# Chuanming-Liu/DAzimSurfTomo

Measured on AMD Instinct MI355X. Metric: FMM traveltime fields/sec (256^2 grid, 16 periods) + LSQR SpMV HBM GB/s, higher is better.
Workload: dtype f32

## Files before the change

dazimsurftomo_amd/csrc/assemble.hip:

```cpp
#include "sparse_internal.h"

#include <rocprim/device/device_scan.hpp>

namespace {

__device__ __forceinline__ bool tikh_face(int cell, int nvx, int nvz, int nzm1, int &i, int &j, int &k) {
  k = cell / (nvx * nvz);
  const int r = cell - k * nvx * nvz;
  j = r / nvx;
  i = r - j * nvx;
  return i == 0 || i == nvx - 1 || j == 0 || j == nvz - 1 || k == 0 || k == nzm1 - 1;
}
__global__ void k_tikh_count(int64_t r0, int64_t nrow, int maxvp, int nvx, int nvz, int nzm1, long *cnt) {
  const int64_t r = (int64_t)blockIdx.x * VB + threadIdx.x;
  if (r > nrow) return;
  int i, j, k;
  cnt[r] = r == nrow ? 0 : (tikh_face((int)((r0 + r) % maxvp), nvx, nvz, nzm1, i, j, k) ? 1 : 7);
}
__global__ void k_tikh_fill(int64_t r0, int64_t nrow, int maxvp, int nvx, int nvz, int nzm1, const long *off, int64_t nnz0,
                            const float *__restrict__ w, int64_t *__restrict__ rowptr, int *__restrict__ col,
                            float *__restrict__ val) {
  const int64_t r = (int64_t)blockIdx.x * VB + threadIdx.x;
  if (r > nrow) return;
  rowptr[r] = nnz0 + off[r];
  if (r == nrow) return;
  const int blk = (int)((r0 + r) / maxvp), cell = (int)((r0 + r) - (int64_t)blk * maxvp);
  int i, j, k;
  const bool face = tikh_face(cell, nvx, nvz, nzm1, i, j, k);
  const float wt = w[blk];
  const int c = blk * maxvp + cell;
  const int64_t p = nnz0 + off[r];
  if (face) {
    col[p] = c;
    val[p] = 2.0f * wt;
  } else {
    const int d[7] = {-nvz * nvx, -nvx, -1, 0, 1, nvx, nvz * nvx};
#pragma unroll
    for (int q = 0; q < 7; q++) {
      col[p + q] = c + d[q];
      val[p + q] = q == 3 ? 6.0f * wt : -1.0f * wt;
    }
  }
}
__device__ __forceinline__ bool lap2d_edge(int cell, int nvx, int nvz) {
  const int j = cell / nvx, i = cell - j * nvx;
  return i == 0 || i == nvx - 1 || j == 0 || j == nvz - 1;
}
__global__ void k_lap2d_count(int64_t nrow, int ncell, int nvx, int nvz, long *cnt) {
  const int64_t r = (int64_t)blockIdx.x * VB + threadIdx.x;
  if (r > nrow) return;
  cnt[r] = r == nrow ? 0 : (lap2d_edge((int)(r % ncell), nvx, nvz) ? 1 : 5);
}
__global__ void k_lap2d_fill(int64_t nrow, int ncell, int nvx, int nvz, const long *off, int64_t nnz0, const float *__restrict__ w,
                             int64_t *__restrict__ rowptr, int *__restrict__ col, float *__restrict__ val) {
  const int64_t r = (int64_t)blockIdx.x * VB + threadIdx.x;
  if (r > nrow) return;
  rowptr[r] = nnz0 + off[r];
  if (r == nrow) return;
  const int b = (int)(r / ncell), cell = (int)(r - (int64_t)b * ncell);
  const float wt = w[b];
  const int c = b * ncell + cell;
  const int64_t p = nnz0 + off[r];
  if (lap2d_edge(cell, nvx, nvz)) {
    col[p] = c;
    val[p] = 2.0f * wt;
  } else {
    const int d[5] = {-nvx, -1, 0, 1, nvx};
#pragma unroll
    for (int q = 0; q < 5; q++) {
      col[p + q] = c + d[q];
      val[p + q] = q == 2 ? 4.0f * wt : -1.0f * wt;
    }
  }
}
__global__ void k_residual(int64_t n, const float *obst, const float *dsyn, float *res, float *rel) {
  for (int64_t i = (int64_t)blockIdx.x * VB + threadIdx.x; i < n; i += (int64_t)gridDim.x * VB) {
    const float r = obst[i] - dsyn[i];
    res[i] = r;
    rel[i] = fabsf(r / obst[i]);
  }
}
__global__ void k_sigma_stats(int64_t n, const float *rel, float *out) {
  constexpr int CH = 8192;
  __shared__ float s_c[CH];
  __shared__ float s_mean;
  float acc = 0.0f;
  for (int pass = 0; pass < 2; pass++) {
    acc = 0.0f;
    const float mean = pass ? s_mean : 0.0f;
    for (int64_t base = 0; base < n; base += CH) {
      const int len = (int)((n - base) < CH ? (n - base) : CH);
      __syncthreads();
      for (int i = threadIdx.x; i < len; i += blockDim.x) s_c[i] = rel[base + i];
      __syncthreads();
      if (threadIdx.x == 0) {
        if (pass == 0)
          for (int i = 0; i < len; i++) acc = acc + s_c[i];
        else
          for (int i = 0; i < len; i++) acc = acc + (s_c[i] - mean) * (s_c[i] - mean);
      }
    }
    if (threadIdx.x == 0) {
      if (pass == 0) {
        s_mean = acc / (float)n;
        out[0] = s_mean;
      } else {
        out[1] = sqrtf(acc / (float)n);
      }
    }
    __syncthreads();
  }
}
__global__ void k_sigma_weights(int64_t n, const float *obst, const float *res, const float *rel, const float *ms, float *wgt,
                                float *rhs) {
  const float sd = ms[1];
  for (int64_t i = (int64_t)blockIdx.x * VB + threadIdx.x; i < n; i += (int64_t)gridDim.x * VB) {
    const float ratio = fabsf(rel[i] / (1.5f * sd));
    float sigma = sd * obst[i];
    if (ratio > 1.0f) sigma = sigma * (float)exp((double)(ratio - 1.0f));
    const float wt = 1.0f / sigma;
    wgt[i] = wt;
    rhs[i] = res[i] * wt;
  }
}
__global__ void k_weight_sums(int64_t n, const float *res, const float *wgt, const float *rhs, double *part) {
  double a[5] = {0, 0, 0, 0, 0};
  for (int64_t i = (int64_t)blockIdx.x * VB + threadIdx.x; i < n; i += (int64_t)gridDim.x * VB) {
    const double r = res[i];
    a[0] += r; a[1] += fabs(r); a[2] += r * r; a[3] += wgt[i]; a[4] += fabsf(rhs[i]);
  }
  __shared__ double s[5][VB / 64];
#pragma unroll
  for (int q = 0; q < 5; q++) {
    const double t = wave_sum(a[q]);
    if ((threadIdx.x & 63) == 0) s[q][threadIdx.x >> 6] = t;
  }
  __syncthreads();
  if (threadIdx.x < 5) {
    double t = 0.0;
    for (int i = 0; i < VB / 64; i++) t += s[threadIdx.x][i];
    part[blockIdx.x * 5 + threadIdx.x] = t;
  }
}
__global__ void k_model_update(int nx, int ny, int nzm1, int joint, float *vs, float *dv, float minvel, float maxvel, float *gc,
                               float *gs) {
  const int nvx = nx - 2, nvz = ny - 2, maxvp = nvx * nvz * nzm1;
  const int ii = blockIdx.x * VB + threadIdx.x;
  if (ii >= maxvp) return;
  const int k = ii / (nvx * nvz), r = ii - k * nvx * nvz, j = r / nvx, i = r - j * nvx;
  float p = dv[ii];
  if (p >= 0.500f) p = 0.500f;
  if (p <= -0.500f) p = -0.500f;
  if (fabsf(p) < 1e-5f) p = 0.0f;
  dv[ii] = p;
  const size_t iv = ((size_t)k * ny + (j + 1)) * nx + (i + 1);
  float v = vs[iv] + p;
  if (v < minvel) v = minvel;
  if (v > maxvel) v = maxvel;
  vs[iv] = v;
  if (joint) {
    if (gc) gc[ii] = dv[maxvp + ii];
    if (gs) gs[ii] = dv[2 * maxvp + ii];
  }
}
__global__ void k_map_update(int nx, int ny, int kmax, int azim, double *pv, float *dm, float minc, float maxc, float *a1, float *a2) {
  const int nvx = nx - 2, nvz = ny - 2, nmap = nvx * nvz * kmax;
  const int ii = blockIdx.x * VB + threadIdx.x;
  if (ii >= nmap) return;
  const int k = ii / (nvx * nvz), r = ii - k * nvx * nvz, j = r / nvx, i = r - j * nvx;
  float p = dm[ii];
  if (p >= 0.500f) p = 0.500f;
  if (p <= -0.500f) p = -0.500f;
  if (fabsf(p) < 1e-5f) p = 0.0f;
  dm[ii] = p;
  const size_t iv = ((size_t)k * ny + (j + 1)) * nx + (i + 1);
  float v = (float)pv[iv] + p;
  if (v < minc) v = minc;
  if (v > maxc) v = maxc;
  pv[iv] = (double)v;
  if (azim) {
    if (a1) a1[ii] = dm[nmap + ii];
    if (a2) a2[ii] = dm[2 * nmap + ii];
  }
}
__global__ void k_update_stats(int ncell, const float *dv, float *out) {
  const float *x = dv + (size_t)blockIdx.x * ncell;
  float mn = INFINITY, mx = -INFINITY;
  double sa = 0.0;
  for (int i = threadIdx.x; i < ncell; i += VB) {
    const float v = x[i];
    mn = fminf(mn, v);
    mx = fmaxf(mx, v);
    sa += fabsf(v);
  }
#pragma unroll
  for (int o = 32; o > 0; o >>= 1) {
    mn = fminf(mn, __shfl_xor(mn, o));
    mx = fmaxf(mx, __shfl_xor(mx, o));
  }
  sa = wave_sum(sa);
  __shared__ float s_mn[VB / 64], s_mx[VB / 64];
  __shared__ double s_sa[VB / 64];
  if ((threadIdx.x & 63) == 0) { s_mn[threadIdx.x >> 6] = mn; s_mx[threadIdx.x >> 6] = mx; s_sa[threadIdx.x >> 6] = sa; }
  __syncthreads();
  if (threadIdx.x == 0) {
    for (int i = 1; i < VB / 64; i++) { mn = fminf(mn, s_mn[i]); mx = fmaxf(mx, s_mx[i]); sa += s_sa[i]; }
    out[blockIdx.x * 3 + 0] = mn; out[blockIdx.x * 3 + 1] = mx; out[blockIdx.x * 3 + 2] = (float)sa;
  }
}

}

extern "C" {

static int append_stencil_rows(dazim_ctx *ctx, dazim_csr *A, bool lap2d, int nvx, int nvz, int nzm1, int64_t maxvp, int64_t row_lo,
                               int64_t nrow, int nblock, const float *w_host, float *dw, long *cnt, long *off);

int dazim_csr_append_tikhonov(dazim_ctx *ctx, dazim_csr *A, int nx, int ny, int nz, int nblock, const float *w_host) {
  if (nblock < 1 || nx < 3 || ny < 3 || nz < 2) return dz_fail(ctx, DAZIM_E_BAD_ARG, "bad arguments to dazim_csr_append_tikhonov");
  return dazim_csr_append_tikhonov_rows(ctx, A, nx, ny, nz, nblock, w_host, 0, (int64_t)(nx - 2) * (ny - 2) * (nz - 1) * nblock);
}
int dazim_csr_append_tikhonov_rows(dazim_ctx *ctx, dazim_csr *A, int nx, int ny, int nz, int nblock, const float *w_host,
                                   int64_t row_lo, int64_t row_hi) {
  if (!ctx || !A || !w_host || nblock < 1 || nx < 3 || ny < 3 || nz < 2) return dz_fail(ctx, DAZIM_E_BAD_ARG, "bad arguments to dazim_csr_append_tikhonov");
  const int nvx = nx - 2, nvz = ny - 2, nzm1 = nz - 1;
  const int64_t maxvp = (int64_t)nvx * nvz * nzm1, nrow = row_hi - row_lo;
  if (row_lo < 0 || row_hi < row_lo || row_hi > maxvp * nblock) return dz_fail(ctx, DAZIM_E_BAD_ARG, "bad row range of the regularisation block");
  if (maxvp * nblock > A->n || maxvp > 0x7ffffff0) return dz_fail(ctx, DAZIM_E_BAD_ARG, "regularisation blocks do not fit the %lld columns", (long long)A->n);
  DZ_HIP(hipSetDevice(ctx->device));
  int rc;
  long *cnt, *off;
  float *dw;
  if ((rc = dz_scratch(ctx, "tikh.cnt", (size_t)(nrow + 1), &cnt)) || (rc = dz_scratch(ctx, "tikh.off", (size_t)(nrow + 1), &off)) ||
      (rc = dz_scratch(ctx, "tikh.w", 64, &dw)))
    return rc;
  if (nblock > 64) return dz_fail(ctx, DAZIM_E_BAD_ARG, "too many regularisation blocks");
  return append_stencil_rows(ctx, A, false, nvx, nvz, nzm1, maxvp, row_lo, nrow, nblock, w_host, dw, cnt, off);
}

static int append_stencil_rows(dazim_ctx *ctx, dazim_csr *A, bool lap2d, int nvx, int nvz, int nzm1, int64_t maxvp, int64_t row_lo,
                               int64_t nrow, int nblock, const float *w_host, float *dw, long *cnt, long *off) {
  int rc;
  void *p;
  DZ_HIP(hipMemcpyAsync(dw, w_host, (size_t)nblock * 4, hipMemcpyHostToDevice, ctx->stream));
  const unsigned nb = (unsigned)((nrow + 1 + VB - 1) / VB);
  if (lap2d)
    hipLaunchKernelGGL(k_lap2d_count, dim3(nb), dim3(VB), 0, ctx->stream, nrow, (int)maxvp, nvx, nvz, cnt);
  else
    hipLaunchKernelGGL(k_tikh_count, dim3(nb), dim3(VB), 0, ctx->stream, row_lo, nrow, (int)maxvp, nvx, nvz, nzm1, cnt);
  auto fill = [&](int64_t *rowptr, int *col, float *val) {
    if (lap2d)
      hipLaunchKernelGGL(k_lap2d_fill, dim3(nb), dim3(VB), 0, ctx->stream, nrow, (int)maxvp, nvx, nvz, off, A->nnz, dw, rowptr, col, val);
    else
      hipLaunchKernelGGL(k_tikh_fill, dim3(nb), dim3(VB), 0, ctx->stream, row_lo, nrow, (int)maxvp, nvx, nvz, nzm1, off, A->nnz, dw,
                         rowptr, col, val);
  };
  size_t tb = 0;
  DZ_HIP(rocprim::exclusive_scan(nullptr, tb, cnt, off, 0l, (size_t)(nrow + 1), rocprim::plus<long>(), ctx->stream));
  if ((rc = dz_scratch(ctx, "tikh.scan", tb + 256, &p))) return rc;
  DZ_HIP(rocprim::exclusive_scan(p, tb, cnt, off, 0l, (size_t)(nrow + 1), rocprim::plus<long>(), ctx->stream));
  long nnz2 = 0;
  DZ_HIP(hipMemcpyAsync(&nnz2, off + nrow, 8, hipMemcpyDeviceToHost, ctx->stream));
  DZ_HIP(hipStreamSynchronize(ctx->stream));
  const int64_t m2 = A->m + nrow, nz2 = A->nnz + nnz2;
  if (nz2 > 0xfffffff0ll) return dz_fail(ctx, DAZIM_E_NNZ_OVERFLOW, "too many stored entries");
  if (A->cap_m >= m2 && A->cap_nnz >= nz2) {
    const int64_t nnz1 = A->nnz;
    fill(A->rowptr + A->m, A->col, A->val);
    DZ_HIP(hipGetLastError());
    A->m = m2;
    A->nnz = nz2;
    if ((rc = dz_build_colblocks(ctx, A, nnz1 > 0 ? nnz1 : 0))) return rc;
    if ((rc = dz_invalidate_transpose(A))) return rc;
    DZ_HIP(hipStreamSynchronize(ctx->stream));
    return 0;
  }
  int64_t *rowptr;
  int *col;
  float *val;
  if ((rc = dz_big_get(ctx, (size_t)(m2 + 1), &rowptr)) || (rc = dz_big_get(ctx, (size_t)(nz2 > 0 ? nz2 : 1), &col)) ||
      (rc = dz_big_get(ctx, (size_t)(nz2 > 0 ? nz2 : 1), &val)))
    return rc;
  DZ_HIP(hipMemcpyAsync(rowptr, A->rowptr, (size_t)A->m * 8, hipMemcpyDeviceToDevice, ctx->stream));
  DZ_HIP(hipMemcpyAsync(col, A->col, (size_t)A->nnz * 4, hipMemcpyDeviceToDevice, ctx->stream));
  DZ_HIP(hipMemcpyAsync(val, A->val, (size_t)A->nnz * 4, hipMemcpyDeviceToDevice, ctx->stream));
  fill(rowptr + A->m, col, val);
  DZ_HIP(hipGetLastError());
  DZ_HIP(hipStreamSynchronize(ctx->stream));
  dz_big_put(ctx, A->rowptr);
  dz_big_put(ctx, A->col);
  dz_big_put(ctx, A->val);
  A->rowptr = rowptr; A->col = col; A->val = val;
  A->m = m2; A->nnz = nz2;
  A->cap_m = A->cap_nnz = 0;
  if ((rc = dz_build_colblocks(ctx, A))) return rc;
  if ((rc = dz_invalidate_transpose(A))) return rc;
  DZ_HIP(hipStreamSynchronize(ctx->stream));
  return 0;
}

int dazim_csr_append_laplacian2d(dazim_ctx *ctx, dazim_csr *A, int nx, int ny, int nmap, const float *w_host) {
  if (!ctx || !A || !w_host || nmap < 1 || nx < 3 || ny < 3) return dz_fail(ctx, DAZIM_E_BAD_ARG, "bad arguments to dazim_csr_append_laplacian2d");
  const int nvx = nx - 2, nvz = ny - 2;
  const int64_t ncell = (int64_t)nvx * nvz, nrow = ncell * nmap;
  if (nrow > A->n || nrow > 0x7ffffff0) return dz_fail(ctx, DAZIM_E_BAD_ARG, "regularisation maps do not fit the %lld columns", (long long)A->n);
  DZ_HIP(hipSetDevice(ctx->device));
  int rc;
  long *cnt, *off;
  float *dw;
  if ((rc = dz_scratch(ctx, "tikh.cnt", (size_t)(nrow + 1), &cnt)) || (rc = dz_scratch(ctx, "tikh.off", (size_t)(nrow + 1), &off)) ||
      (rc = dz_scratch(ctx, "lap2d.w", (size_t)nmap, &dw)))
    return rc;
  return append_stencil_rows(ctx, A, true, nvx, nvz, 1, ncell, 0, nrow, nmap, w_host, dw, cnt, off);
}

int dazim_weight_data(dazim_ctx *ctx, dazim_csr *G, int64_t dall, const float *obst_u, const float *dsyn_u, float *res_u,
                      float *wgt_u, float *rhs_u, float *stats) {
  return dazim_weight_data_sharded(ctx, G, dall, 0, dall, obst_u, dsyn_u, res_u, wgt_u, rhs_u, stats);
}
int dazim_weight_data_sharded(dazim_ctx *ctx, dazim_csr *G, int64_t dall, int64_t row0, int64_t dall_glob, const float *obst_u,
                              const float *dsyn_u, float *res_u, float *wgt_u, float *rhs_u, float *stats) {
  if (!ctx || dall < 1 || !obst_u || !dsyn_u || !res_u || !wgt_u || !rhs_u || (G && G->m < dall) || row0 < 0 || row0 + dall > dall_glob)
    return dz_fail(ctx, DAZIM_E_BAD_ARG, "bad arguments to dazim_weight_data");
  const bool sharded = ctx->comm && dall_glob > dall;
  DZ_HIP(hipSetDevice(ctx->device));
  DzBuf<float> obst, dsyn, res, wgt, rhs;
  int rc;
  if ((rc = obst.init(ctx, obst_u, dall, true, false)) || (rc = dsyn.init(ctx, dsyn_u, dall, true, false)) ||
      (rc = res.init(ctx, res_u, dall, false, true)) || (rc = wgt.init(ctx, wgt_u, dall, false, true)) ||
      (rc = rhs.init(ctx, rhs_u, dall, false, true)))
    return rc;
  float *rel, *ms;
  double *part;
  if ((rc = dz_scratch(ctx, "wd.rel", (size_t)dall, &rel)) || (rc = dz_scratch(ctx, "wd.ms", 16, &ms)) ||
      (rc = dz_scratch(ctx, "wd.part", (size_t)NPART * 5, &part)))
    return rc;
  const int nb = nblk(dall, NPART);
  hipLaunchKernelGGL(k_residual, dim3(nb), dim3(VB), 0, ctx->stream, dall, obst.dev, dsyn.dev, res.dev, rel);
  if (sharded) {
    float *relg;
    if ((rc = dz_scratch(ctx, "wd.relg", (size_t)dall_glob, &relg))) return rc;
    DZ_HIP(hipMemsetAsync(relg, 0, (size_t)dall_glob * 4, ctx->stream));
    DZ_HIP(hipMemcpyAsync(relg + row0, rel, (size_t)dall * 4, hipMemcpyDeviceToDevice, ctx->stream));
    if ((rc = dz_allreduce(ctx, (DzComm *)ctx->comm, relg, (size_t)dall_glob, DZ_F32, DZ_SUM))) return rc;
    hipLaunchKernelGGL(k_sigma_stats, dim3(1), dim3(VB), 0, ctx->stream, dall_glob, relg, ms);
  } else {
    hipLaunchKernelGGL(k_sigma_stats, dim3(1), dim3(VB), 0, ctx->stream, dall, rel, ms);
  }
  hipLaunchKernelGGL(k_sigma_weights, dim3(nb), dim3(VB), 0, ctx->stream, dall, obst.dev, res.dev, rel, ms, wgt.dev, rhs.dev);
  hipLaunchKernelGGL(k_weight_sums, dim3(nb), dim3(VB), 0, ctx->stream, dall, res.dev, wgt.dev, rhs.dev, part);
  DZ_HIP(hipGetLastError());
  std::vector<double> hp((size_t)nb * 5);
  float hms[2];
  DZ_HIP(hipMemcpyAsync(hp.data(), part, hp.size() * 8, hipMemcpyDeviceToHost, ctx->stream));
  DZ_HIP(hipMemcpyAsync(hms, ms, 8, hipMemcpyDeviceToHost, ctx->stream));
  if (G && (rc = dz_scale_rows(ctx, G, dall, wgt.dev))) return rc;
  DZ_HIP(hipStreamSynchronize(ctx->stream));
  if (stats) {
    double a[5] = {0, 0, 0, 0, 0};
    for (int b = 0; b < nb; b++)
      for (int q = 0; q < 5; q++) a[q] += hp[(size_t)b * 5 + q];
    if (sharded && (rc = dazim_comm_allreduce(ctx, a, 5, DZ_F64, DZ_SUM))) return rc;
    const double n = (double)dall_glob, mean = a[0] / n;
    stats[0] = (float)mean;
    stats[1] = (float)sqrt(fmax(a[2] / n - mean * mean, 0.0));
    stats[2] = (float)(a[1] / n);
    stats[3] = (float)sqrt(a[2] / n);
    stats[4] = hms[0];
    stats[5] = hms[1];
    stats[6] = (float)(a[3] / n);
    stats[7] = (float)(a[4] / n);
  }
  if ((rc = res.finish()) || (rc = wgt.finish()) || (rc = rhs.finish())) return rc;
  DZ_HIP(hipStreamSynchronize(ctx->stream));
  return 0;
}

int dazim_model_update(dazim_ctx *ctx, int nx, int ny, int nz, int joint, float *vs_u, float *dv_u, float minvel, float maxvel,
                       float *gc_u, float *gs_u, float *stats) {
  if (!ctx || !vs_u || !dv_u || nx < 3 || ny < 3 || nz < 2) return dz_fail(ctx, DAZIM_E_BAD_ARG, "bad arguments to dazim_model_update");
  DZ_HIP(hipSetDevice(ctx->device));
  const int nzm1 = nz - 1, ncell = (nx - 2) * (ny - 2), maxvp = ncell * nzm1, nblock = joint ? 3 : 1;
  DzBuf<float> vs, dv, gc, gs;
  int rc;
  if ((rc = vs.init(ctx, vs_u, (size_t)nx * ny * nz, true, true)) || (rc = dv.init(ctx, dv_u, (size_t)maxvp * nblock, true, true)) ||
      (rc = gc.init(ctx, gc_u, joint ? maxvp : 0, false, true)) || (rc = gs.init(ctx, gs_u, joint ? maxvp : 0, false, true)))
    return rc;
  hipLaunchKernelGGL(k_model_update, dim3((maxvp + VB - 1) / VB), dim3(VB), 0, ctx->stream, nx, ny, nzm1, joint, vs.dev, dv.dev,
                     minvel, maxvel, joint ? gc.dev : nullptr, joint ? gs.dev : nullptr);
  DZ_HIP(hipGetLastError());
  if (stats) {
    float *p;
    if ((rc = dz_scratch(ctx, "mu.stats", (size_t)nblock * nzm1 * 3, &p))) return rc;
    hipLaunchKernelGGL(k_update_stats, dim3(nblock * nzm1), dim3(VB), 0, ctx->stream, ncell, dv.dev, p);
    DZ_HIP(hipGetLastError());
    DZ_HIP(hipMemcpyAsync(stats, p, (size_t)nblock * nzm1 * 3 * 4, hipMemcpyDeviceToHost, ctx->stream));
  }
  if ((rc = vs.finish()) || (rc = dv.finish()) || (rc = gc.finish()) || (rc = gs.finish())) return rc;
  DZ_HIP(hipStreamSynchronize(ctx->stream));
  return 0;
}

int dazim_phase_map_update(dazim_ctx *ctx, int nx, int ny, int kmax, int azim, double *pv_u, float *dm_u, float minc, float maxc,
                           float *a1_u, float *a2_u, float *stats) {
  if (!ctx || !pv_u || !dm_u || nx < 3 || ny < 3 || kmax < 1) return dz_fail(ctx, DAZIM_E_BAD_ARG, "bad arguments to dazim_phase_map_update");
  DZ_HIP(hipSetDevice(ctx->device));
  const int ncell = (nx - 2) * (ny - 2), nmap = ncell * kmax, nblock = azim ? 3 : 1;
  DzBuf<double> pv;
  DzBuf<float> dm, a1, a2;
  int rc;
  if ((rc = pv.init(ctx, pv_u, (size_t)nx * ny * kmax, true, true)) || (rc = dm.init(ctx, dm_u, (size_t)nmap * nblock, true, true)) ||
      (rc = a1.init(ctx, a1_u, azim ? nmap : 0, false, true)) || (rc = a2.init(ctx, a2_u, azim ? nmap : 0, false, true)))
    return rc;
  hipLaunchKernelGGL(k_map_update, dim3((nmap + VB - 1) / VB), dim3(VB), 0, ctx->stream, nx, ny, kmax, azim ? 1 : 0, pv.dev, dm.dev,
                     minc, maxc, azim ? a1.dev : nullptr, azim ? a2.dev : nullptr);
  DZ_HIP(hipGetLastError());
  if (stats) {
    float *p;
    if ((rc = dz_scratch(ctx, "mu.stats", (size_t)nblock * kmax * 3, &p))) return rc;
    hipLaunchKernelGGL(k_update_stats, dim3(nblock * kmax), dim3(VB), 0, ctx->stream, ncell, dm.dev, p);
    DZ_HIP(hipGetLastError());
    DZ_HIP(hipMemcpyAsync(stats, p, (size_t)nblock * kmax * 3 * 4, hipMemcpyDeviceToHost, ctx->stream));
  }
  if ((rc = pv.finish()) || (rc = dm.finish()) || (rc = a1.finish()) || (rc = a2.finish())) return rc;
  DZ_HIP(hipStreamSynchronize(ctx->stream));
  return 0;
}

}
```

dazimsurftomo_amd/csrc/rays.hip:

```cpp
#include <cmath>
#include <chrono>
#include <unistd.h>

#include "dazim_internal.h"

#include <rocprim/device/device_scan.hpp>
#include <rocprim/device/device_radix_sort.hpp>

namespace {

#ifdef DZ_RAYS_MARK
#define RAYS_MARK(i) asm volatile("; MARK " #i ::: "memory")
#else
#define RAYS_MARK(i)
#endif

constexpr int GDX = 5, GDZ = 5;
constexpr int RM = DAZIM_RMAX;
constexpr float EARTH = 6371.0f;
constexpr float FTOL = 1e-4f;

struct RayArgs {
  dazim_geom g;
  int nx, ny, nz, kmax;
  long nray;
  const int *field;
  const float *rcx, *rcz;
  const float *scx, *scz;
  const int *period;
  const int *kidx;
  const float *veln;
  const float *ttn;
  const int *tslot;
  int tsh;
  long fstride;
  const int *fdone;
  int *defer_mark;
  int max_quads;
  int sweeps;
  const float *ttnr;
  const int *nstsr;
  const dazim_refbox *boxes;
  const float *vels;
  const double *svs, *svp, *srho;
  unsigned nvx_magic;
  const double *skern;
  const float *lsen;
  double r_dnx, r_dnz, r_dnxr, r_dnzr, r_dvx, r_dvz, r_e2dnx, r_e2dnxr;
  float dplh;
  float *dsurf;
  int *status;
  int *rbflag;
  long *count;
  int *nlist;
  unsigned short *lcell;
  float *lval;
  float *fdm_scratch;
  int LK;
  int lcap;
  const unsigned *perm;
  unsigned *qcount;
  float2 *pts;
  int *npts;
  int pcap;
  int dense;
  long *countd;
  int plain_step;
  int keep_small;
  const long *rowptr;
  float *val;
  int *col;
};

__device__ __forceinline__ float dz_sinf(float x) {
  if (!(x > 0.0f && x < 3.1415927f)) return (float)sin((double)x);
  const double y = (double)x - 1.5707963267948966192;
  const double y2 = y * y;
  double p = -1.5619206968586226e-16;
  p = fma(p, y2, 4.7794773323873853e-14);
  p = fma(p, y2, -1.1470745597729725e-11);
  p = fma(p, y2, 2.0876756987868099e-09);
  p = fma(p, y2, -2.7557319223985891e-07);
  p = fma(p, y2, 2.4801587301587302e-05);
  p = fma(p, y2, -1.3888888888888889e-03);
  p = fma(p, y2, 4.1666666666666664e-02);
  p = fma(p, y2, -0.5);
  p = fma(p, y2, 1.0);
  return (float)p;
}

__device__ __forceinline__ void step_azimuth(float x0, float z0, float x1, float z1, float &c2psi, float &s2psi) {
  const float PI_F = 3.1415926535898f;
  const float evtlat = (PI_F / 2 - x0) * 180.0f / PI_F, evtlon = z0 * 180.0f / PI_F;
  const float stalat = (PI_F / 2 - x1) * 180.0f / PI_F, stalon = z1 * 180.0f / PI_F;
  const double pi = (double)3.1415926535898f;
  const float piby2 = (float)(pi / (double)2.f);
  const double rad = (double)2.f * pi / (double)360.f;
  const double sph = (double)(1.0f / 298.257f);
  const double scolat = (double)piby2 - atan((1. - sph) * (1. - sph) * tan((double)stalat * rad));
  const double ecolat = (double)piby2 - atan((1. - sph) * (1. - sph) * tan((double)evtlat * rad));
  const double slon = (double)stalon * rad, elon = (double)evtlon * rad;
  const double a = sin(scolat) * cos(slon), b = sin(scolat) * sin(slon), c = cos(scolat);
  const double dd = sin(elon), ee = -cos(elon), cc = cos(ecolat);
  const double gg = -cc * ee, hh = cc * dd, kk = -sin(ecolat);
  const double rhs1 = (a - dd) * (a - dd) + (b - ee) * (b - ee) + c * c - (double)2.f;
  const double rhs2 = (a - gg) * (a - gg) + (b - hh) * (b - hh) + (c - kk) * (c - kk) - (double)2.f;
  double daz = atan2(rhs1, rhs2);
  if (daz < 0.0) daz = daz + 2 * pi;
  float az = (float)(daz / rad);
  if (fabsf(az - 360.f) < .00001f) az = 0.0f;
  const float rgpsi = az / 180 * PI_F;
  c2psi = (float)cos((double)(2.0f * rgpsi));
  s2psi = (float)sin((double)(2.0f * rgpsi));
}

__device__ __forceinline__ float divr(float x, double rd) { return (float)((double)x * rd); }

__device__ __forceinline__ void basis(float v, float b[4]) {
  const float om = 1.0f - v;
  b[0] = om * om * om / 6.0f;
  b[1] = (4.0f - 6.0f * (v * v) + 3.0f * (v * v * v)) / 6.0f;
  b[2] = (1.0f + 3.0f * v + 3.0f * (v * v) - 3.0f * (v * v * v)) / 6.0f;
  b[3] = v * v * v / 6.0f;
}

__device__ __forceinline__ float div6(float x) { return divr(x, 1.0 / 6.0); }
__device__ __forceinline__ float basis1(float v, int i) {
  const float w = i == 0 ? 1.0f - v : v;
  const float t2 = w * w, t3 = t2 * w;
  const float p = i == 1 ? 4.0f : 1.0f + 3.0f * v;
  const float c = i == 1 ? -6.0f : 3.0f, d = i == 1 ? 3.0f : -3.0f;
  const float n = (p + c * t2) + d * t3;
  return div6((i == 0 || i == 3) ? t3 : n);
}

__device__ __forceinline__ float vel_at(const dazim_geom &g, const float *veln, int ipx, int ipz, float drx, float drz,
                                        double rdnx, double rdnz) {
  float vel = 0.0f;
#pragma unroll
  for (int l = 1; l <= 2; l++)
#pragma unroll
    for (int m = 1; m <= 2; m++) {
      float produ = (1.0f - fabsf(divr((float)(m - 1) * g.dnz - drz, rdnz)));
      produ = produ * (1.0f - fabsf(divr((float)(l - 1) * g.dnx - drx, rdnx)));
      if (ipz - 1 + m <= g.nnz && ipx - 1 + l <= g.nnx && ipz - 1 + m >= 1 && ipx - 1 + l >= 1)
        vel = vel + veln[(size_t)(ipx - 2 + l) * g.nnz + (ipz - 2 + m)] * produ;
    }
  return vel;
}
__device__ __forceinline__ float vel_at_interior(const dazim_geom &g, const float *veln, int ipx, int ipz, float drx, float drz,
                                                 double rdnx, double rdnz) {
  float vel = 0.0f;
#pragma unroll
  for (int l = 1; l <= 2; l++)
#pragma unroll
    for (int m = 1; m <= 2; m++) {
      float produ = (1.0f - fabsf(divr((float)(m - 1) * g.dnz - drz, rdnz)));
      produ = produ * (1.0f - fabsf(divr((float)(l - 1) * g.dnx - drx, rdnx)));
      vel = vel + veln[(size_t)(ipx - 2 + l) * g.nnz + (ipz - 2 + m)] * produ;
    }
  return vel;
}

__device__ __forceinline__ float bilin_cell(const dazim_geom &g, const float *veln, int cx, int cz, float px, float pz,
                                            double rdnx, double rdnz) {
  const float drx = (px - g.gox) - (float)(cx - 1) * g.dnx;
  const float drz = (pz - g.goz) - (float)(cz - 1) * g.dnz;
  float biv = 0.0f;
#pragma unroll
  for (int i = 1; i <= 2; i++)
#pragma unroll
    for (int j = 1; j <= 2; j++) {
      const float produ = (1.0f - fabsf(divr((float)(i - 1) * g.dnx - drx, rdnx))) *
                          (1.0f - fabsf(divr((float)(j - 1) * g.dnz - drz, rdnz)));
      biv = biv + veln[(size_t)(cx - 2 + i) * g.nnz + (cz - 2 + j)] * produ;
    }
  return biv;
}

__global__ void k_row_kernels(long n, int kmax, long ncol, const float *__restrict__ vels, const double *__restrict__ svs,
                              const double *__restrict__ svp, const double *__restrict__ srho, double *__restrict__ out) {
  const long i = (long)blockIdx.x * blockDim.x + threadIdx.x;
  if (i >= n) return;
  const long k = i / (kmax * ncol), c = i % ncol;
  out[i] = dz_row_kernel(vels[k * ncol + c], svs[i], svp[i], srho[i]);
}

__global__ void k_ray_keys(long nray, const int *__restrict__ field, const float *__restrict__ scx, const float *__restrict__ scz,
                           const float *__restrict__ rcx, const float *__restrict__ rcz, float inv_dmax, int dbits,
                           unsigned *__restrict__ keys, unsigned *__restrict__ iota, const int *__restrict__ order) {
  const long i = (long)blockIdx.x * blockDim.x + threadIdx.x;
  if (i >= nray) return;
  const int f = field[i];
  const float dx = scx[f] - rcx[i], dz = (scz[f] - rcz[i]) * __sinf(rcx[i]);
  const float d = sqrtf(dx * dx + dz * dz) * inv_dmax;
  const unsigned dmaxq = (1u << dbits) - 1u;
  unsigned q = d >= 1.0f ? dmaxq : (unsigned)(d * (float)dmaxq);
  keys[i] = ((unsigned)(order ? order[f] : f) << dbits) | (dmaxq - q);
  iota[i] = (unsigned)i;
}

constexpr int GP_COUNT = 8, GP_EMIT = 16;
constexpr int RAYS_MINW = 4;
constexpr int RPW_MAX = 64 / GP_COUNT;
__device__ __forceinline__ void cbar() { asm volatile("" ::: "memory"); }

template <bool EMIT, bool AZIM, bool TILED, bool MAP>
__global__ __launch_bounds__(64, AZIM ? 2 : RAYS_MINW) void rays_kernel(RayArgs A_) {
  using ArgP = const __attribute__((address_space(4))) RayArgs *;
  auto launder = [](ArgP p) {
    int z;
    asm volatile("v_mov_b32 %0, 0" : "=v"(z));
    return (ArgP)((const __attribute__((address_space(4))) char *)p + __builtin_amdgcn_readfirstlane(z));
  };
  ArgP Ap = launder((ArgP)__builtin_amdgcn_kernarg_segment_ptr());
#define A (*Ap)
#define RAYS_ARGS_FRESH Ap = launder(Ap)
  constexpr int GP = EMIT ? GP_EMIT : GP_COUNT;
  constexpr int RPW = 64 / GP;
  constexpr int LPR = 16 / GP;
  constexpr int LSTEP = 4 / LPR;
  constexpr unsigned GMASK = (1u << GP) - 1u;
  extern __shared__ __attribute__((aligned(16))) unsigned short s_lists[];
  dazim_geom g;
  g.nvx = A.g.nvx; g.nvz = A.g.nvz; g.nnx = A.g.nnx; g.nnz = A.g.nnz;
  g.gox = A.g.gox; g.goz = A.g.goz; g.dnx = A.g.dnx; g.dnz = A.g.dnz; g.dvx = A.g.dvx; g.dvz = A.g.dvz;
  const int lane = threadIdx.x, grp = lane / GP, gl = lane & (GP - 1);
  const int lm = gl & 3, l0 = gl >> 2;
  const int nnx = g.nnx, nnz = g.nnz, nvx = g.nvx, nvz = g.nvz;
  const int ldf = nvx + 2, nf = ldf * (nvz + 2);
  constexpr int NG = AZIM ? 3 : 1;
  const unsigned nvx_magic = A.nvx_magic;
  const int LC = A.lcap;
  unsigned short *s_list = s_lists + (size_t)grp * LC;
  float *gfdm = A.fdm_scratch + ((size_t)blockIdx.x * RPW + grp) * nf * NG;
  float *gfdmc = gfdm + nf, *gfdms = gfdm + 2 * nf;
  __shared__ int s_rngs[RPW][4];
  int *s_rng = s_rngs[grp];
  constexpr int RC = 8;
  const float gox = g.gox, goz = g.goz, dnx = g.dnx, dnz = g.dnz, dvx = g.dvx, dvz = g.dvz;
  const double rdnx = A.r_dnx, rdnz = A.r_dnz, rdnxr = A.r_dnxr, rdnzr = A.r_dnzr, rdvx = A.r_dvx, rdvz = A.r_dvz;
  const unsigned gmask_shift = grp * GP;
  const long nquad = (A.nray + RPW - 1) / RPW;
  const int nxcd = (gridDim.x % 8 == 0) ? 8 : 1;
  unsigned *qcnt = A.qcount + (EMIT ? 8 : 0);
  int chunk = (int)(blockIdx.x % nxcd);
  int traced = 0;
  for (;;) {
    RAYS_ARGS_FRESH;
    long quad = -1;
    if (lane == 0) {
      for (int tried = 0; tried < nxcd; tried++) {
        const long lo = nquad * chunk / nxcd, hi = nquad * (chunk + 1) / nxcd;
        const long b = lo < hi ? (long)atomicAdd(&qcnt[chunk], 1u) : hi;
        if (lo + b < hi) {
          quad = lo + b;
          break;
        }
        if (!EMIT && A.sweeps > 1 && lo < hi && b < (hi - lo) * A.sweeps) {
          quad = lo + b % (hi - lo);
          break;
        }
        chunk = (chunk + 1) % nxcd;
      }
    }
    quad = ((long)__shfl((int)(quad >> 32), 0) << 32) | (unsigned)__shfl((int)quad, 0);
    chunk = __shfl(chunk, 0);
    if (quad < 0) break;
    const long slot = quad * RPW + grp;
    if (!EMIT && A.defer_mark) {
      if (!A.defer_mark[quad]) continue;
      if (A.fdone) {
        const int fq = slot < A.nray ? A.field[A.perm ? (long)A.perm[slot] : slot] : -1;
        const int st = fq >= 0 ? __hip_atomic_load(A.fdone + fq, __ATOMIC_ACQUIRE, __HIP_MEMORY_SCOPE_AGENT) : 1;
        if (__ballot(st != 1) != 0) continue;
        __builtin_amdgcn_fence(__ATOMIC_ACQUIRE, "agent");
      }
      if (A.max_quads > 0 && traced >= A.max_quads) break;
      int mine = 0;
      if (lane == 0) mine = __hip_atomic_exchange(A.defer_mark + quad, 0, __ATOMIC_RELAXED, __HIP_MEMORY_SCOPE_AGENT);
      mine = __shfl(mine, 0);
      if (!mine) continue;
      traced++;
      if (lane == 0) atomicAdd(&A.qcount[18], 1u);
    }
    if (slot >= A.nray) continue;
    const long ray = A.perm ? (long)A.perm[slot] : slot;
    const int f = A.field[ray];
    const float scx = A.scx[f], scz = A.scz[f], rcx = A.rcx[ray], rcz = A.rcz[ray];
    const float *veln = A.veln + (size_t)(A.period[f] - 1) * nnx * nnz;
    const float *ttn = TILED ? A.ttn + (size_t)(A.tslot ? A.tslot[f] : f) * A.fstride : A.ttn + (size_t)f * nnx * nnz;
    const int tsh = TILED ? A.tsh : 0;
    auto tnode = [&](int x0, int z0) -> float {
      return TILED ? ttn[dz_tile_x(x0, tsh) + dz_tile_z(z0)] : ttn[(size_t)x0 * nnz + z0];
    };
    const float *ttnr = A.ttnr + (size_t)f * RM * RM;
    const int *nstsr = A.nstsr + (size_t)f * RM * RM;
    const dazim_refbox bx = A.boxes[f];
    const int saved = EMIT ? A.nlist[ray] : -1;
    if (saved < 0 && gl < 4) s_rng[gl] = gl < 2 ? 0x7fffffff : -1;
    cbar();
    int status = 0, rb = 0;
    if (!EMIT) {
      int irx = (int)divr(rcx - gox, rdnx) + 1, irz = (int)divr(rcz - goz, rdnz) + 1;
      if (irx < 1 || irx > nnx || irz < 1 || irz > nnz) status = DAZIM_E_RECEIVER_OUTSIDE;
      if (!status) {
        if (irx == nnx) irx--;
        if (irz == nnz) irz--;
        const int isx = (int)divr(scx - gox, rdnx) + 1, isz = (int)divr(scz - goz, rdnz) + 1;
        float sred = ((scx - rcx) * EARTH) * ((scx - rcx) * EARTH);
        const float e2 = (scz - rcz) * EARTH * dz_sinf(rcx);
        sred = sqrtf(sred + e2 * e2);
        bool sw = sred < A.dplh;
        if (isx == irx && isz == irz) sw = true;
        float trr;
        if (sw) {
          const float vs = bilin_cell(g, veln, isx, isz, scx, scz, rdnx, rdnz);
          const float vr = bilin_cell(g, veln, irx, irz, rcx, rcz, rdnx, rdnz);
          trr = 2.0f * sred / (vs + vr);
        } else {
          const float drx = (rcx - gox) - (float)(irx - 1) * dnx;
          const float drz = (rcz - goz) - (float)(irz - 1) * dnz;
          trr = 0.0f;
#pragma unroll
          for (int k = 1; k <= 2; k++)
#pragma unroll
            for (int l = 1; l <= 2; l++) {
              const float produ = (1.0f - fabsf(divr((float)(l - 1) * dnz - drz, rdnz))) *
                                  (1.0f - fabsf(divr((float)(k - 1) * dnx - drx, rdnx)));
              trr = trr + tnode(irx - 2 + k, irz - 2 + l) * produ;
            }
        }
        if (gl == 0) A.dsurf[ray] = trr;
      }
    }
    const float goxr = bx.goxr, gozr = bx.gozr, dnxr = bx.dnxr, dnzr = bx.dnzr;
    const int nnxr = bx.nnxr, nnzr = bx.nnzr;
    const int isx = (int)divr(scx - goxr, rdnxr) + 1, isz = (int)divr(scz - gozr, rdnzr) + 1;
    const float dpl = 0.5f * A.dplh;
    int ipx = (int)divr(rcx - gox, rdnx) + 1, ipz = (int)divr(rcz - goz, rdnz) + 1;
    if (ipx < 1 || ipx >= nnx || ipz < 1 || ipz >= nnz) status = DAZIM_E_RECEIVER_OUTSIDE;
    if (!status && saved < 0) {
      float x0 = rcx, z0 = rcz;
      float sinx0 = dz_sinf(x0);
      int sw = 0;
      float sred = ((scx - x0) * EARTH) * ((scx - x0) * EARTH);
      float e2 = (scz - z0) * EARTH * sinx0;
      sred = sqrtf(sred + e2 * e2);
      if (sred < 2.0f * dpl) sw = 1;
      int ipxr = (int)divr(rcx - goxr, rdnxr) + 1, ipzr = (int)divr(rcz - gozr, rdnzr) + 1;
      auto in_refined = [&](int px, int pz) -> int {
        if (px < 1 || px >= nnxr || pz < 1 || pz >= nnzr) return 0;
        const int *sp = nstsr + (size_t)(px - 1) * RM + (pz - 1);
        if (sp[0] != 0 || sp[1] != 0) return 0;
        if (sp[RM] != 0 || sp[RM + 1] != 0) return 0;
        return 1;
      };
      int igref = in_refined(ipxr, ipzr);
      if (sw == 0 && igref == 1 && ipxr == isx && ipzr == isz) sw = 1;
      const bool keep_pts = !EMIT && A.pts != nullptr && gl == 0;
      float2 *rp = A.pts ? A.pts + (size_t)ray * A.pcap : nullptr;
      int np = 1;
      if (keep_pts) {
        rp[0] = make_float2(rcx, rcz);
        if (sw == 1) { if (A.pcap > 1) rp[1] = make_float2(scx, scz); np = 2; }
      }
      int cbx = -100, cbz = -100;
      float acc[LPR], accc[LPR], accs[LPR];
#pragma unroll
      for (int q = 0; q < LPR; q++) acc[q] = accc[q] = accs[q] = 0.0f;
      auto flush = [&]() {
        if (cbx > -100) {
#pragma unroll
          for (int q = 0; q < LPR; q++) {
            const int fi = (cbz + l0 + q * LSTEP) * ldf + (cbx + lm);
            gfdm[fi] = acc[q];
            if (AZIM) { gfdmc[fi] = accc[q]; gfdms[fi] = accs[q]; }
          }
        }
      };
      float tc00, tc01, tc10, tc11, tr00 = 0.0f, tr01 = 0.0f, tr10 = 0.0f, tr11 = 0.0f;
      auto load_corner_times = [&]() {
        if (TILED) {
          const int x0 = dz_tile_x(ipx - 1, tsh), x1 = dz_tile_x(ipx, tsh), z0 = dz_tile_z(ipz - 1), z1 = dz_tile_z(ipz);
          tc00 = ttn[x0 + z0]; tc01 = ttn[x0 + z1]; tc10 = ttn[x1 + z0]; tc11 = ttn[x1 + z1];
        } else {
          const float *t = ttn + (size_t)(ipx - 1) * nnz + (ipz - 1);
          tc00 = t[0]; tc01 = t[1]; tc10 = t[nnz]; tc11 = t[nnz + 1];
        }
      };
      auto load_refined_corner_times = [&]() {
        if (ipxr >= 1 && ipxr < nnxr && ipzr >= 1 && ipzr < nnzr) {
          const float *u = ttnr + (size_t)(ipxr - 1) * RM + (ipzr - 1);
          tr00 = u[0]; tr01 = u[1]; tr10 = u[RM]; tr11 = u[RM + 1];
        }
      };
      load_corner_times();
      load_refined_corner_times();
      bool carry = false;
      float rdc[LPR];
#pragma unroll
      for (int q = 0; q < LPR; q++) rdc[q] = 0.0f;
      float fart = __builtin_inff();
      int nnx_in = 0, nnz_in = 0;
      const long maxrp = (long)nnx * nnz;
      for (long j = 1; j <= maxrp; j++) {
        if (sw == 1) break;
        RAYS_MARK(0);
        float dtx, dtz;
        if (igref == 1) {
          dtx = tr10 - tr00;
          dtx = dtx + tr11 - tr01;
          dtx = divr(dtx, A.r_e2dnxr);
          dtz = tr01 - tr00;
          dtz = dtz + tr11 - tr10;
          dtz = dtz / (2.0f * EARTH * sinx0 * dnzr);
        } else {
          dtx = tc10 - tc00;
          dtx = dtx + tc11 - tc01;
          dtx = divr(dtx, A.r_e2dnx);
          dtz = tc01 - tc00;
          dtz = dtz + tc11 - tc10;
          dtz = dtz / (2.0f * EARTH * sinx0 * dnz);
        }
        const float rd1 = sqrtf(dtx * dtx + dtz * dtz);
        float x1 = x0 - dpl * dtx / (EARTH * rd1);
        float z1 = z0 - dpl * dtz / (EARTH * sinx0 * rd1);
        RAYS_MARK(1);
        const int ipxo = ipx, ipzo = ipz;
        const float sdx = scx - x1, sdz = scz - z1;
        bool srcell = false;
        if (__ballot(!(fabsf(sdx) > fart || fabsf(sdz) > fart)) != 0) {
          ipxr = (int)divr(x1 - goxr, rdnxr) + 1;
          ipzr = (int)divr(z1 - gozr, rdnzr) + 1;
          igref = in_refined(ipxr, ipzr);
          srcell = igref == 1 && ipxr == isx && ipzr == isz;
          load_refined_corner_times();
        } else {
          igref = 0;
        }
        ipx = (int)divr(x1 - gox, rdnx) + 1;
        ipz = (int)divr(z1 - goz, rdnz) + 1;
        RAYS_MARK(2);
        float sinx1 = dz_sinf(x1);
        sred = (sdx * EARTH) * (sdx * EARTH);
        e2 = sdz * EARTH * sinx1;
        sred = sqrtf(sred + e2 * e2);
        sw = 0;
        if (sred < 2.0f * dpl) sw = 1;
        if (srcell) sw = 1;
        RAYS_MARK(3);
        bool clipx = false;
        if (ipx < 1) { x1 = gox; ipx = 1; rb = 1; clipx = true; }
        if (ipx >= nnx) { x1 = gox + (float)(nnx - 1) * dnx; ipx = nnx - 1; rb = 1; clipx = true; }
        if (ipz < 1) { z1 = goz; ipz = 1; rb = 1; }
        if (ipz >= nnz) { z1 = goz + (float)(nnz - 1) * dnz; ipz = nnz - 1; rb = 1; }
        RAYS_MARK(4);
        load_corner_times();
        if (keep_pts) {
          if (np < A.pcap) rp[np] = make_float2(x1, z1);
          np++;
          if (sw == 1) {
            if (np < A.pcap) rp[np] = make_float2(scx, scz);
            np++;
          }
        }
        if (clipx) sinx1 = dz_sinf(x1);
        float c2psi = 0.0f, s2psi = 0.0f;
        if (AZIM) step_azimuth(x0, z0, x1, z1, c2psi, s2psi);
        RAYS_MARK(5);
        const int ivx = (ipx - 1) / GDX + 1, ivz = (ipz - 1) / GDZ + 1;
        const int ivxo = (ipxo - 1) / GDX + 1, ivzo = (ipzo - 1) / GDZ + 1;
        int nhp = 0, chp0 = 0, chp1 = 0;
        float vr0 = 1.0f, vr1 = 1.0f, vr2 = 1.0f;
        if (ivx != ivxo) {
          nhp = 1;
          const float xi = (ivx > ivxo) ? gox + (float)(ivx - 1) * dvx : gox + (float)ivx * dvx;
          vr0 = (xi - x0) / (x1 - x0);
          chp0 = 1;
        }
        if (ivz != ivzo) {
          const float zi = (ivz > ivzo) ? goz + (float)(ivz - 1) * dvz : goz + (float)ivz * dvz;
          const float r = (zi - z0) / (z1 - z0);
          if (nhp == 0) {
            vr0 = r;
            chp0 = 2;
          } else if (r >= vr0) {
            vr1 = r;
            chp1 = 2;
          } else {
            vr1 = vr0;
            chp1 = chp0;
            vr0 = r;
            chp0 = 2;
          }
          nhp++;
        }
        nhp++;
        if (nhp == 1) vr0 = 1.0f;
        if (nhp == 2) vr1 = 1.0f;
        RAYS_MARK(6);
        float drx, drz;
        if (__builtin_expect(__ballot(!carry) != 0, 0)) {
          drx = (x0 - gox) - (float)(ipxo - 1) * dnx;
          drz = (z0 - goz) - (float)(ipzo - 1) * dnz;
          const float vel = vel_at(g, veln, ipxo, ipzo, drx, drz, rdnx, rdnz);
          drx = (x0 - gox) - (float)(ivxo - 1) * dvx;
          drz = (z0 - goz) - (float)(ivzo - 1) * dvz;
          const float vi = basis1(divr(drx, rdvx), lm);
#pragma unroll
          for (int q = 0; q < LPR; q++) rdc[q] = vi * basis1(divr(drz, rdvz), l0 + q * LSTEP) / (vel * vel);
          if (A.plain_step == 0) {
            fart = (float)((RM - 1) / 8 + 1) * fmaxf(dnx, dnz);
            nnx_in = nnx;
            nnz_in = nnz;
          }
        }
        RAYS_MARK(7);
        int ivxt = ivxo, ivzt = ivzo;
        bool endsame = false;
        for (int k = 1; k <= nhp; k++) {
          if (k > 1) {
            const int cp = (k == 2) ? chp0 : chp1;
            if (cp == 1) ivxt = ivx;
            else if (cp == 2) ivzt = ivz;
          }
          const float vrk = (k == 1) ? vr0 : (k == 2 ? vr1 : vr2);
          const float vrp = (k == 2) ? vr0 : vr1;
          const float rigz = z0 + vrk * (z1 - z0);
          const float rigx = x0 + vrk * (x1 - x0);
          const int ipxt = (int)divr(rigx - gox, rdnx) + 1, ipzt = (int)divr(rigz - goz, rdnz) + 1;
          endsame = rigx == x1 && rigz == z1 && ipxt == ipx && ipzt == ipz && ivxt == ivx && ivzt == ivz;
          drx = (rigx - gox) - (float)(ipxt - 1) * dnx;
          drz = (rigz - goz) - (float)(ipzt - 1) * dnz;
          const bool inner = ipxt >= 1 && ipxt < nnx_in && ipzt >= 1 && ipzt < nnz_in;
          endsame = endsame && inner;
          float vel;
          if (__builtin_expect(__ballot(!inner) == 0, 1)) vel = vel_at_interior(g, veln, ipxt, ipzt, drx, drz, rdnx, rdnz);
          else vel = vel_at(g, veln, ipxt, ipzt, drx, drz, rdnx, rdnz);
          drx = (rigx - gox) - (float)(ivxt - 1) * dvx;
          drz = (rigz - goz) - (float)(ivzt - 1) * dvz;
          const float vi = basis1(divr(drx, rdvx), lm);
          float wi[LPR];
#pragma unroll
          for (int q = 0; q < LPR; q++) wi[q] = basis1(divr(drz, rdvz), l0 + q * LSTEP);
          const float dinc = (k == 1) ? vrk * dpl : (vrk - vrp) * dpl;
          const int nbx = ivxt - 1, nbz = ivzt - 1;
          RAYS_MARK(8);
          if (nbx != cbx || nbz != cbz) {
            flush();
            cbar();
            cbx = nbx;
            cbz = nbz;
            __hip_atomic_fetch_min(s_rng + 0, nbx, __ATOMIC_RELAXED, __HIP_MEMORY_SCOPE_WORKGROUP);
            __hip_atomic_fetch_min(s_rng + 1, nbz, __ATOMIC_RELAXED, __HIP_MEMORY_SCOPE_WORKGROUP);
            __hip_atomic_fetch_max(s_rng + 2, nbx, __ATOMIC_RELAXED, __HIP_MEMORY_SCOPE_WORKGROUP);
            __hip_atomic_fetch_max(s_rng + 3, nbz, __ATOMIC_RELAXED, __HIP_MEMORY_SCOPE_WORKGROUP);
#pragma unroll
            for (int q = 0; q < LPR; q++) {
              const int fi = (cbz + l0 + q * LSTEP) * ldf + (cbx + lm);
              acc[q] = gfdm[fi];
              if (AZIM) { accc[q] = gfdmc[fi]; accs[q] = gfdms[fi]; }
            }
          }
          RAYS_MARK(9);
#pragma unroll
          for (int q = 0; q < LPR; q++) {
            const float rdc1 = vi * wi[q] / (vel * vel);
            const float rdc2 = rdc[q];
            rdc[q] = rdc1;
            float r1 = -(rdc1 + rdc2) * dinc / 2.0f;
            acc[q] = r1 + acc[q];
            if (AZIM) {
              r1 = -(rdc1 * c2psi + rdc2 * c2psi) * dinc / 2.0f;
              accc[q] = r1 + accc[q];
              r1 = -(rdc1 * s2psi + rdc2 * s2psi) * dinc / 2.0f;
              accs[q] = r1 + accs[q];
            }
          }
        }
        RAYS_MARK(10);
        carry = endsame;
        x0 = x1;
        z0 = z1;
        sinx0 = sinx1;
      RAYS_MARK(11);
      }
      flush();
      if (keep_pts) A.npts[ray] = np <= A.pcap ? np : -1;
    }
    cbar();
    if (!EMIT && gl == 0) {
      if (A.pts && status) A.npts[ray] = 0;
      A.status[ray] = status;
      A.rbflag[ray] = rb;
    }
    auto usual = [&](int n) { return n <= LC && n <= RC * GP && (MAP || A.skern != nullptr) && !A.dense; };
    int nlist = 0;
    if (saved >= 0) {
      nlist = saved;
      const size_t o = (size_t)ray * A.LK, ov = o * NG;
      const bool viaslot = !usual(saved);
      for (int i = gl; i < nlist; i += GP) {
        const int c = A.lcell[o + i];
        s_list[i] = (unsigned short)c;
        if (viaslot) {
          const int jj = (int)__umulhi((unsigned)c, nvx_magic) + 1, kk = c - (jj - 1) * nvx + 1;
          gfdm[jj * ldf + kk] = A.lval[ov + i];
          if (AZIM) {
            gfdmc[jj * ldf + kk] = A.lval[ov + A.LK + i];
            gfdms[jj * ldf + kk] = A.lval[ov + 2 * A.LK + i];
          }
        }
      }
    } else if (!status) {
      const int kk0 = max(s_rng[0], 1), kk1 = min(s_rng[2] + 3, nvx), jj0 = max(s_rng[1], 1), jj1 = min(s_rng[3] + 3, nvz);
      for (int jj = jj0; jj <= jj1; jj++)
        for (int kb = kk0; kb <= kk1; kb += GP) {
          const int kk = kb + gl;
          const bool keep = kk <= kk1 && fabsf(gfdm[jj * ldf + kk]) >= FTOL;
          const unsigned m = (unsigned)((__ballot(keep) >> gmask_shift) & GMASK);
          const int pos = nlist + __popc(m & ((1u << gl) - 1u));
          if (keep && pos < LC) s_list[pos] = (unsigned short)((jj - 1) * nvx + kk - 1);
          nlist += __popc(m);
        }
    }
    cbar();
    if (!EMIT) {
      const size_t o = (size_t)ray * A.LK, ov = o * NG;
      if (nlist <= A.LK)
        for (int i = gl; i < nlist; i += GP) {
          const int c = s_list[i];
          const int jj = (int)__umulhi((unsigned)c, nvx_magic) + 1, kk = c - (jj - 1) * nvx + 1;
          A.lcell[o + i] = (unsigned short)c;
          A.lval[ov + i] = gfdm[jj * ldf + kk];
          if (AZIM) {
            A.lval[ov + A.LK + i] = gfdmc[jj * ldf + kk];
            A.lval[ov + 2 * A.LK + i] = gfdms[jj * ldf + kk];
          }
        }
      if (gl == 0) A.nlist[ray] = (status || nlist <= A.LK) ? (status ? 0 : nlist) : -1;
    }
    const size_t ncol = (size_t)A.nx * A.ny;
    const int kslot = A.kidx[f] - 1;
    long cnt = 0;
    const long rstart = EMIT ? A.rowptr[ray] : 0;
    const int nparpi = nvx * nvz * (A.nz - 1);
    const int nlay = MAP ? 1 : A.nz - 1;
    const int bstride = MAP ? A.kmax * nvx * nvz : nparpi;
    const int poff = MAP ? (A.period[f] - 1) * nvx * nvz : 0;
    const bool lovf = nlist > LC;
    const int ntot = lovf ? nvz * nvx : nlist;
    long cntd = 0;
    int jjL = 1, kkL = 1;
    if (A.dense) {
      int clast = -1;
      if (!lovf) {
        if (nlist > 0) clast = s_list[nlist - 1];
      } else {
        for (int base = ((nvz * nvx - 1) / GP) * GP; base >= 0 && clast < 0; base -= GP) {
          const int c = base + gl;
          bool k2 = false;
          if (c < nvz * nvx) {
            const int jj = (int)__umulhi((unsigned)c, nvx_magic) + 1, kk = c - (jj - 1) * nvx + 1;
            k2 = fabsf(gfdm[jj * ldf + kk]) >= FTOL;
          }
          const unsigned m2 = (unsigned)((__ballot(k2) >> gmask_shift) & GMASK);
          if (m2) clast = base + (31 - __clz(m2));
        }
      }
      if (clast >= 0) { jjL = (int)__umulhi((unsigned)clast, nvx_magic) + 1; kkL = clast - (jjL - 1) * nvx + 1; }
    }
    const bool rowcache = usual(nlist);
    if (rowcache) {
      int sidx[RC], cbase[RC], fidx[RC];
#pragma unroll
      for (int i = 0; i < RC; i++) {
        const int li = i * GP + gl;
        const int c = li < ntot ? (int)s_list[li] : 0;
        const int jj = (int)__umulhi((unsigned)c, nvx_magic) + 1, kk = c - (jj - 1) * nvx + 1;
        sidx[i] = jj * (nvx + 2) + kk;
        cbase[i] = (jj - 1) * nvx + kk;
        fidx[i] = jj * ldf + kk;
      }
      for (int blk = 0; blk < NG; blk++) {
        float fdv[RC];
        const float *fsrc = blk == 0 ? gfdm : (blk == 1 ? gfdmc : gfdms);
        const float *lsrc = A.lval + ((size_t)ray * NG + blk) * A.LK;
#pragma unroll
        for (int i = 0; i < RC; i++) fdv[i] = (i * GP + gl < ntot) ? (saved >= 0 ? lsrc[i * GP + gl] : fsrc[fidx[i]]) : 0.0f;
        for (int k = 1; k <= nlay; k++) {
          const size_t sk = ((size_t)(k - 1) * A.kmax + kslot) * ncol;
          const int nk = blk * bstride + poff + (k - 1) * nvz * nvx;
#pragma unroll
          for (int i = 0; i < RC; i++) {
            if (i * GP >= ntot) break;
            const bool cell = i * GP + gl < ntot;
            float rowv = 0.0f;
            bool keep = false;
            if (cell) {
              if (MAP) rowv = fdv[i];
              else if (blk == 0) rowv = (float)(A.skern[sk + sidx[i]] * (double)fdv[i]);
              else rowv = A.lsen[sk + sidx[i]] * fdv[i];
              keep = A.keep_small ? (rowv != 0.0f) : (fabsf(rowv) > FTOL);
            }
            const unsigned m = (unsigned)((__ballot(keep) >> gmask_shift) & GMASK);
            if (EMIT && keep) {
              const long pos = rstart + cnt + __popc(m & ((1u << gl) - 1u));
              A.val[pos] = rowv;
              A.col[pos] = nk + cbase[i] - 1;
            }
            cnt += __popc(m);
          }
        }
      }
    } else
    for (int blk = 0; blk < NG; blk++)
      for (int k = 1; k <= nlay; k++) {
        for (int base = 0; base < ntot; base += GP) {
          const int li = base + gl;
          bool keep = false, keepd = false;
          float rowv = 0.0f;
          int nn = 0;
          bool cell = li < ntot;
          int c = 0;
          if (cell) c = lovf ? li : s_list[li];
          const int jj = (int)__umulhi((unsigned)c, nvx_magic) + 1, kk = c - (jj - 1) * nvx + 1;
          if (cell && lovf) cell = fabsf(gfdm[jj * ldf + kk]) >= FTOL;
          if (cell && MAP) {
            rowv = (blk == 0 ? gfdm : (blk == 1 ? gfdmc : gfdms))[jj * ldf + kk];
            keep = A.keep_small ? (rowv != 0.0f) : (fabsf(rowv) > FTOL);
            nn = blk * bstride + poff + (jj - 1) * nvx + kk;
          } else if (cell) {
            const size_t si = ((size_t)(k - 1) * A.kmax + kslot) * ncol + (size_t)jj * (nvx + 2) + kk;
            if (blk == 0) {
              const float fd = gfdm[jj * ldf + kk];
              double r;
              if (A.skern) {
                r = A.skern[si] * (double)fd;
              } else {
                const float v = A.vels[((size_t)(k - 1) * A.ny + jj) * A.nx + kk];
                const float coe_a = (2.0947f - 0.8206f * 2 * v + 0.2683f * 3 * (v * v) - 0.0251f * 4 * (v * v * v));
                const float vpft = 0.9409f + 2.0947f * v - 0.8206f * (v * v) + 0.2683f * (v * v * v) - 0.0251f * (v * v * v * v);
                const float coe_rho = coe_a * (1.6612f - 0.4721f * 2 * vpft + 0.0671f * 3 * (vpft * vpft) -
                                               0.0043f * 4 * (vpft * vpft * vpft) + 0.000106f * 5 * (vpft * vpft * vpft * vpft));
                r = (A.svp[si] * (double)coe_a + A.srho[si] * (double)coe_rho + A.svs[si]) * (double)fd;
              }
              rowv = (float)r;
              if (A.dense) {
                const float vL = A.vels[((size_t)(k - 1) * A.ny + jjL) * A.nx + kkL];
                const float caL = (2.0947f - 0.8206f * 2 * vL + 0.2683f * 3 * (vL * vL) - 0.0251f * 4 * (vL * vL * vL));
                const float vpL = 0.9409f + 2.0947f * vL - 0.8206f * (vL * vL) + 0.2683f * (vL * vL * vL) - 0.0251f * (vL * vL * vL * vL);
                const float crL = caL * (1.6612f - 0.4721f * 2 * vpL + 0.0671f * 3 * (vpL * vpL) -
                                         0.0043f * 4 * (vpL * vpL * vpL) + 0.000106f * 5 * (vpL * vpL * vpL * vpL));
                const double rd = (A.svp[si] * (double)caL + A.srho[si] * (double)crL + A.svs[si]) * (double)fd;
                keepd = (float)rd != 0.0f;
                if (EMIT && A.dense == 1) rowv = (float)rd;
              }
            } else {
              rowv = A.lsen[si] * (blk == 1 ? gfdmc : gfdms)[jj * ldf + kk];
              keepd = rowv != 0.0f;
            }
            keep = A.keep_small ? (rowv != 0.0f) : (fabsf(rowv) > FTOL);
            if (EMIT && A.dense == 1) keep = keepd;
            nn = blk * bstride + (k - 1) * nvz * nvx + (jj - 1) * nvx + kk;
          }
          if (!EMIT && A.dense == 2) cntd += __popc((unsigned)((__ballot(keepd) >> gmask_shift) & GMASK));
          const unsigned m = (unsigned)((__ballot(keep) >> gmask_shift) & GMASK);
          if (EMIT && keep) {
            const long pos = rstart + cnt + __popc(m & ((1u << gl) - 1u));
            A.val[pos] = rowv;
            A.col[pos] = nn - 1;
          }
          cnt += __popc(m);
        }
      }
    cbar();
    if (saved < 0) {
      const int x0 = max(s_rng[0], 0), x1 = min(s_rng[2] + 3, nvx + 1), z0 = max(s_rng[1], 0), z1 = min(s_rng[3] + 3, nvz + 1);
      for (int z = z0; z <= z1; z++)
        for (int x = x0 + gl; x <= x1; x += GP) {
          gfdm[z * ldf + x] = 0.0f;
          if (AZIM) { gfdmc[z * ldf + x] = 0.0f; gfdms[z * ldf + x] = 0.0f; }
        }
    } else if (!rowcache) {
      for (int i = gl; i < nlist; i += GP) {
        const int c = s_list[i];
        const int jj = (int)__umulhi((unsigned)c, nvx_magic) + 1, kk = c - (jj - 1) * nvx + 1;
        gfdm[jj * ldf + kk] = 0.0f;
        if (AZIM) { gfdmc[jj * ldf + kk] = 0.0f; gfdms[jj * ldf + kk] = 0.0f; }
      }
    }
    cbar();
    if (!EMIT && gl == 0) {
      A.count[ray] = cnt;
      if (A.dense == 2) A.countd[ray] = cntd;
      if (lovf) atomicAdd(&A.qcount[16], 1u);
      if (!status && nlist > A.LK) atomicAdd(&A.qcount[17], 1u);
    }
  }
}
#undef A
#undef RAYS_ARGS_FRESH

struct RayBuild {
  dazim_ctx *ctx;
  int nx = 0, ny = 0, nz = 0, kmax = 0, nfield = 0;
  float goxd = 0, gozd = 0, dvxd = 0, dvzd = 0;
  const float *vels = nullptr, *scx = nullptr, *scz = nullptr, *veln = nullptr, *ttn = nullptr, *ttnr = nullptr, *rcx = nullptr, *rcz = nullptr;
  const float *lsen = nullptr;
  const int *period = nullptr, *kidx = nullptr, *nstsr = nullptr, *field = nullptr;
  const dazim_refbox *boxes = nullptr;
  const double *svs = nullptr, *svp = nullptr, *srho = nullptr;
  int64_t nray = 0;
  float *dsurf = nullptr;
  dazim_csr **G = nullptr;
  int64_t *nnz_out = nullptr;
  int *n_boundary = nullptr;
  bool map = false, azim = false;
  struct StreamSwap {
    dazim_ctx *c; hipStream_t main; bool on = false;
    void restore() { if (on) { c->stream = main; on = false; } }
    ~StreamSwap() {
      if (on) (void)hipStreamSynchronize(c->stream);
      restore();
    }
  } swap;
  struct {
    DzBuf<float> vels, scx, scz, veln, ttn, ttnr, rcx, rcz, dsurf, lsen;
    DzBuf<int> period, kidx, nstsr, field;
    DzBuf<dazim_refbox> boxes;
    DzBuf<double> svs, svp, srho;
  } d;
  struct Arrays {
    dazim_ctx *c; int64_t *rp = nullptr; float *v = nullptr; int *cl = nullptr; int64_t nnz = 0, cap_nnz = 0; bool keep = false;
    ~Arrays() { if (!keep) { dz_big_put(c, rp); dz_big_put(c, v); dz_big_put(c, cl); } }
  } arrays, arrays_d;
  dazim_geom g;
  bool joint = false, tiled = false, overlap = false, twin = false;
  size_t nn = 0, nr = 0, ncol = 0, nk = 0, nr1 = 0, lds = 0;
  int64_t res_rows = 0, res_nnz = 0;
  long nwg = 0;
  double overlap_tail_s = 0.0;
  RayArgs A;
  explicit RayBuild(dazim_ctx *c) : ctx(c), swap{c, c ? c->stream : nullptr}, arrays{c}, arrays_d{c} {}
  int check() {
    if (!ctx || !G) return DAZIM_E_BAD_ARG;
    joint = map ? azim : lsen != nullptr;
    if (map) nz = 2;
    if (map && dz_opt(ctx, "rays.dense_twin", 0) != 0)
      return dz_fail(ctx, DAZIM_E_BAD_ARG, "dazim_rays_build_G_maps: option rays.dense_twin serves the 3-D program's diagnostics only");
    if (dazim_geometry(nx, ny, goxd, gozd, dvxd, dvzd, &g)) return dz_fail(ctx, DAZIM_E_BAD_ARG, "bad grid");
    if (nray < 0 || nfield < 1 || nz < 2 || kmax < 1 || (size_t)g.nvx * g.nvz > 65535u) return dz_fail(ctx, DAZIM_E_BAD_ARG, "bad arguments to dazim_rays_build_G");
    tiled = ttn == nullptr;
    if (tiled && (!ctx->fields.tiled || ctx->fields.nfield != nfield || ctx->fields.nnx != g.nnx || ctx->fields.nnz != g.nnz))
      return dz_fail(ctx, DAZIM_E_BAD_ARG, "dazim_rays_build_G: ttn is NULL and the last dazim_fmm_batch call did not keep %d fields of this grid inside the library (call it with ttn = NULL)", nfield);
    if (!scx || !scz || !period || !veln || !ttnr || !nstsr || !boxes || !dsurf ||
        (!map && (!vels || !svs || !svp || !srho)) || (nray > 0 && (!field || !rcx || !rcz)))
      return dz_fail(ctx, DAZIM_E_BAD_ARG, "dazim_rays_build_G: NULL array (the refined fields ttnr, nstsr and boxes of dazim_fmm_batch are required)");
    DZ_HIP(hipSetDevice(ctx->device));
    return 0;
  }
  int decide_overlap() {
    overlap = (bool)ctx->fmm_finish && tiled && ctx->fields.fdone && nray > 0;
    if (overlap && ctx->aux_epilogue && ctx->comm && ((DzComm *)ctx->comm)->nccl) overlap = false;
    if (overlap)
      for (const void *q : {(const void *)vels, (const void *)scx, (const void *)scz, (const void *)period, (const void *)veln,
                            (const void *)ttnr, (const void *)nstsr, (const void *)boxes, (const void *)field, (const void *)rcx,
                            (const void *)rcz, (const void *)svs, (const void *)svp, (const void *)srho, (const void *)dsurf,
                            (const void *)kidx, (const void *)lsen})
        if (q && !dz_is_device_ptr(q)) overlap = false;
    if (!overlap) { const int rcf = dz_fmm_finish(ctx); if (rcf) return rcf; }
    if (overlap) {
      DZ_HIP(hipStreamWaitEvent(ctx->stream3, ctx->ev_pre, 0));
      ctx->stream = ctx->stream3;
      swap.on = true;
    }
    return dz_join_aux(ctx);
  }
  int stage_inputs() {
    nn = (size_t)g.nnx * g.nnz; nr = (size_t)RM * RM; ncol = (size_t)nx * ny;
    int rc;
    if (!map && (rc = d.vels.init(ctx, vels, (size_t)nz * ncol, true, false))) return rc;
    if ((rc = d.scx.init(ctx, scx, nfield, true, false)) || (rc = d.scz.init(ctx, scz, nfield, true, false)) ||
        (rc = d.period.init(ctx, period, nfield, true, false)) || (rc = d.kidx.init(ctx, kidx ? kidx : period, nfield, true, false)) ||
        (rc = d.veln.init(ctx, veln, nn * kmax, true, false)) || (!tiled && (rc = d.ttn.init(ctx, ttn, nn * nfield, true, false))) ||
        (rc = d.ttnr.init(ctx, ttnr, nr * nfield, true, false)) || (rc = d.nstsr.init(ctx, nstsr, nr * nfield, true, false)) ||
        (rc = d.boxes.init(ctx, boxes, nfield, true, false)) || (rc = d.field.init(ctx, field, nray, true, false)) ||
        (rc = d.rcx.init(ctx, rcx, nray, true, false)) || (rc = d.rcz.init(ctx, rcz, nray, true, false)))
      return rc;
    nk = (size_t)nz * kmax * ncol;
    if (!map && ((rc = d.svs.init(ctx, svs, nk, true, false)) || (rc = d.svp.init(ctx, svp, nk, true, false)) ||
                  (rc = d.srho.init(ctx, srho, nk, true, false))))
      return rc;
    if ((rc = d.dsurf.init(ctx, dsurf, nray, false, true))) return rc;
    if (joint && !map && (rc = d.lsen.init(ctx, lsen, (size_t)(nz - 1) * kmax * ncol, true, false))) return rc;
    if ((rc = dz_check_range(ctx, d.period.dev, nfield, 1, kmax, "period_idx"))) return rc;
    if ((rc = dz_check_range(ctx, d.kidx.dev, nfield, 1, kmax, "kernel_idx"))) return rc;
    return dz_check_range(ctx, d.field.dev, nray, 0, nfield - 1, "field_of_ray");
  }
  int kernel_constants() {
    int rc;
    A.g = g;
    A.nx = nx; A.ny = ny; A.nz = nz; A.kmax = kmax;
    A.nray = nray;
    A.field = d.field.dev; A.rcx = d.rcx.dev; A.rcz = d.rcz.dev; A.scx = d.scx.dev; A.scz = d.scz.dev;
    A.period = d.period.dev; A.kidx = d.kidx.dev; A.veln = d.veln.dev; A.ttn = d.ttn.dev; A.ttnr = d.ttnr.dev;
    A.tslot = nullptr; A.tsh = 0; A.fstride = (long)nn;
    if (tiled) {
      A.ttn = reinterpret_cast<const float *>(ctx->fields.tiled);
      A.tslot = ctx->fields.tslot; A.tsh = ctx->fields.tsh; A.fstride = ctx->fields.stride;
    }
    ctx->ksec["rays.tiled_fields"] = tiled ? 1.0 : 0.0;
    ctx->ksec["rays.map"] = map ? 1.0 : 0.0;
    ctx->ksec["rays.overlap"] = overlap ? 1.0 : 0.0;
    A.fdone = overlap ? ctx->fields.fdone : nullptr;
    A.defer_mark = nullptr; A.max_quads = 0; A.sweeps = 1;
    A.nstsr = d.nstsr.dev; A.boxes = d.boxes.dev; A.vels = d.vels.dev; A.svs = d.svs.dev; A.svp = d.svp.dev; A.srho = d.srho.dev;
    A.lsen = joint && !map ? d.lsen.dev : nullptr;
    A.skern = nullptr;
    {
      const unsigned dv = (unsigned)g.nvx;
      A.nvx_magic = (unsigned)((0x100000000ull + dv - 1) / dv);
      for (unsigned c = 0; c < 65536u; c++)
        if ((unsigned)(((unsigned long long)c * A.nvx_magic) >> 32) != c / dv) return dz_fail(ctx, DAZIM_E_BAD_ARG, "internal: reciprocal of nvx");
    }
    if (!map && dz_opt(ctx, "rays.skern", 1) != 0) {
      double *pk;
      if ((rc = dz_scratch(ctx, "rays.skern", nk, &pk))) return rc;
      hipLaunchKernelGGL(k_row_kernels, dim3((unsigned)((nk + 255) / 256)), dim3(256), 0, ctx->stream, (long)nk, kmax, (long)ncol,
                         d.vels.dev, d.svs.dev, d.svp.dev, d.srho.dev, pk);
      DZ_HIP(hipGetLastError());
      A.skern = pk;
    }
    {
      float dpl = g.dnx * EARTH;
      float rd1 = g.dnz * EARTH * sinf(g.gox);
      if (rd1 < dpl) dpl = rd1;
      rd1 = g.dnz * EARTH * sinf(g.gox + (float)(g.nnx - 1) * g.dnx);
      if (rd1 < dpl) dpl = rd1;
      A.dplh = dpl;
    }
    {
      const float dnxr = g.dvx / (float)(GDX * 8), dnzr = g.dvz / (float)(GDZ * 8);
      const float e2dnx = 2.0f * EARTH * g.dnx, e2dnxr = 2.0f * EARTH * dnxr;
      A.r_dnx = 1.0 / (double)g.dnx;   A.r_dnz = 1.0 / (double)g.dnz;
      A.r_dnxr = 1.0 / (double)dnxr;   A.r_dnzr = 1.0 / (double)dnzr;
      A.r_dvx = 1.0 / (double)g.dvx;   A.r_dvz = 1.0 / (double)g.dvz;
      A.r_e2dnx = 1.0 / (double)e2dnx; A.r_e2dnxr = 1.0 / (double)e2dnxr;
    }
    return 0;
  }
  int scratch() {
    int rc;
    nr1 = (size_t)(nray > 0 ? nray : 1);
    if ((rc = dz_scratch(ctx, "rays.status", nr1, &A.status))) return rc;
    if ((rc = dz_scratch(ctx, "rays.rb", nr1, &A.rbflag))) return rc;
    if ((rc = dz_scratch(ctx, "rays.count", (size_t)(nray + 1), &A.count))) return rc;
    A.lcap = g.nvx * g.nvz <= 4096 ? 512 : 1024;
    if (dz_opt(ctx, "rays.lcap", 0) >= 16 && dz_opt(ctx, "rays.lcap", 0) <= 8192) A.lcap = dz_opt(ctx, "rays.lcap", 0);
    if (A.lcap > g.nvx * g.nvz) A.lcap = g.nvx * g.nvz;
    A.LK = A.lcap;
    A.keep_small = dz_opt(ctx, "rays.keep_small", 0) != 0 ? 1 : 0;
    A.plain_step = dz_opt(ctx, "rays.plain_step", 0) != 0 ? 1 : 0;
    A.pts = nullptr; A.npts = nullptr; A.pcap = 0;
    if (dz_opt(ctx, "rays.keep_paths", 0) != 0) {
      A.pcap = 4 * (g.nnx + g.nnz) + 16;
      if ((rc = dz_scratch(ctx, "rays.pts", nr1 * (size_t)A.pcap, &A.pts))) return rc;
      if ((rc = dz_scratch(ctx, "rays.npts", nr1, &A.npts))) return rc;
      DZ_HIP(hipMemsetAsync(A.npts, 0, nr1 * 4, ctx->stream));
    }
    ctx->ksec["rays.path_cap"] = A.pcap;
    ctx->ksec["rays.path_rays"] = A.pts ? (double)nray : 0.0;
    twin = dz_opt(ctx, "rays.dense_twin", 0) != 0 && !A.keep_small;
    A.dense = twin ? 2 : 0;
    A.countd = nullptr;
    if (twin) {
      if ((rc = dz_scratch(ctx, "rays.countd", (size_t)(nray + 1), &A.countd))) return rc;
      DZ_HIP(hipMemsetAsync(A.countd, 0, (size_t)(nray + 1) * 8, ctx->stream));
    }
    if ((rc = dz_scratch(ctx, "rays.nlist", nr1, &A.nlist))) return rc;
    if ((rc = dz_scratch(ctx, "rays.lcell", nr1 * A.LK, &A.lcell))) return rc;
    if ((rc = dz_scratch(ctx, "rays.lval", nr1 * A.LK * (joint ? 3 : 1), &A.lval))) return rc;
    res_rows = (int64_t)g.nvx * g.nvz * (map ? kmax : nz - 1) * (joint ? 3 : 1);
    res_nnz = (map ? 5 : 7) * res_rows;
    if (dz_opt(ctx, "csr.reserve_rows", 0) > res_rows) res_rows = dz_opt(ctx, "csr.reserve_rows", 0);
    if (dz_opt(ctx, "csr.reserve_nnz", 0) > res_nnz) res_nnz = dz_opt(ctx, "csr.reserve_nnz", 0);
    if ((rc = dz_big_get(ctx, (size_t)(nray + res_rows + 1), &arrays.rp))) return rc;
    A.dsurf = d.dsurf.dev;
    A.rowptr = (const long *)arrays.rp; A.val = nullptr; A.col = nullptr;
    return 0;
  }
  template <int I> static const void *kernel_no() { return (const void *)rays_kernel<(I & 8) != 0, (I & 4) != 0, (I & 2) != 0, (I & 1) != 0>; }
  const void *kern(bool emit) const {
    static const void *const tab[16] = {kernel_no<0>(),  kernel_no<1>(),  kernel_no<2>(),  kernel_no<3>(), kernel_no<4>(),  kernel_no<5>(),
                                        kernel_no<6>(),  kernel_no<7>(),  kernel_no<8>(),  kernel_no<9>(), kernel_no<10>(), kernel_no<11>(),
                                        kernel_no<12>(), kernel_no<13>(), kernel_no<14>(), kernel_no<15>()};
    return tab[(emit ? 8 : 0) + (joint ? 4 : 0) + (tiled ? 2 : 0) + (map ? 1 : 0)];
  }
  int launch(bool emit, const RayArgs &R, long nwg_) {
    RayArgs args = R;
    void *params[] = {&args};
    DZ_HIP(hipLaunchKernel(kern(emit), dim3((unsigned)nwg_), dim3(64), params, lds, ctx->stream));
    return 0;
  }
  int launch_shape() {
    lds = (size_t)A.lcap * 2 * RPW_MAX + 16;
    DZ_HIP(hipFuncSetAttribute(kern(false), hipFuncAttributeMaxDynamicSharedMemorySize, (int)lds));
    DZ_HIP(hipFuncSetAttribute(kern(true), hipFuncAttributeMaxDynamicSharedMemorySize, (int)lds));
    int per_cu = (int)(160 * 1024 / (lds + 256));
    {
      int occ = 0;
      const void *kf = kern(false);
      if (hipOccupancyMaxActiveBlocksPerMultiprocessor(&occ, kf, 64, lds) == hipSuccess && occ > 0 && occ < per_cu) per_cu = occ;
    }
    if (per_cu > 16) per_cu = 16;
    if (per_cu < 1) return dz_fail(ctx, DAZIM_E_BAD_ARG, "inversion grid too large for the LDS cell lists");
    if (dz_opt(ctx, "rays.wg_per_cu", 0) > 0 && dz_opt(ctx, "rays.wg_per_cu", 0) < per_cu) per_cu = dz_opt(ctx, "rays.wg_per_cu", 0);
    nwg = (long)ctx->num_cu * per_cu;
    if (nwg > (nray + RPW_MAX - 1) / RPW_MAX) nwg = (nray + RPW_MAX - 1) / RPW_MAX;
    if (dz_opt(ctx, "rays.nwg", 0) > 0 && dz_opt(ctx, "rays.nwg", 0) < nwg) nwg = dz_opt(ctx, "rays.nwg", 0);
    if (nwg >= 8) nwg -= nwg % 8;
    if (nwg < 1) nwg = 1;
    const size_t nslot = (size_t)nwg * RPW_MAX * (g.nvx + 2) * (g.nvz + 2) * (joint ? 3 : 1);
    int rc;
    if ((rc = dz_scratch(ctx, "rays.fdm", nslot, &A.fdm_scratch))) return rc;
    DZ_HIP(hipMemsetAsync(A.fdm_scratch, 0, nslot * sizeof(float), ctx->stream));
    ctx->ksec["rays.nwg"] = (double)nwg;
    return 0;
  }
  int sort_rays() {
    int rc;
    A.perm = nullptr;
    if (nray >= 64 && nray < (1ll << 32) && dz_opt(ctx, "rays.sort", 1) != 0) {
      int fbits = 1;
      while ((1ll << fbits) < nfield) fbits++;
      const int dbits = 32 - fbits > 12 ? 12 : 32 - fbits;
      if (dbits >= 4) {
        unsigned *k0, *k1, *v0, *v1;
        if ((rc = dz_scratch(ctx, "rays.sortbuf", (size_t)nray * 4 + 16, &k0))) return rc;
        k1 = k0 + nray; v0 = k1 + nray; v1 = v0 + nray;
        const float ex = (float)g.nnx * g.dnx, ez = (float)g.nnz * g.dnz;
        const float inv_dmax = 1.0f / sqrtf(ex * ex + ez * ez);
        hipLaunchKernelGGL(k_ray_keys, dim3((unsigned)((nray + 255) / 256)), dim3(256), 0, ctx->stream, (long)nray, d.field.dev, d.scx.dev,
                           d.scz.dev, d.rcx.dev, d.rcz.dev, inv_dmax, dbits, k0, v0, overlap ? A.tslot : (const int *)nullptr);
        size_t tb = 0;
        DZ_HIP(rocprim::radix_sort_pairs(nullptr, tb, k0, k1, v0, v1, (size_t)nray, 0, fbits + dbits, ctx->stream));
        void *tmp;
        if ((rc = dz_scratch(ctx, "rays.sorttmp", tb + 256, &tmp))) return rc;
        DZ_HIP(rocprim::radix_sort_pairs(tmp, tb, k0, k1, v0, v1, (size_t)nray, 0, fbits + dbits, ctx->stream));
        A.perm = v1;
      }
    }
    if ((rc = dz_scratch(ctx, "rays.qcount", 32, &A.qcount))) return rc;
    DZ_HIP(hipMemsetAsync(A.qcount, 0, 128, ctx->stream));
    if (overlap) {
      const size_t nq = (size_t)((nray + RPW_MAX - 1) / RPW_MAX) + 8;
      if ((rc = dz_scratch(ctx, "rays.defer", nq, &A.defer_mark))) return rc;
      DZ_HIP(hipMemsetAsync(A.defer_mark, 0, nq * 4, ctx->stream));
    }
    return 0;
  }
  int count_pass() { return nray > 0 ? launch(false, A, nwg) : 0; }
  int count_passes_beside_eikonal() {
    int rc;
    const auto t_poll0 = std::chrono::steady_clock::now();
    auto fmm_over = [&]() {
      const bool over = hipEventQuery(ctx->ev_f1) == hipSuccess;
      if (!over) (void)hipGetLastError();
      return over;
    };
    if (ctx->fields.hprog && ctx->fields.total_tasks > 0) {
      const unsigned slack = ctx->fields.nwg / 4 + 8 * 16;
      const unsigned total = ctx->fields.total_tasks;
      const unsigned want = total > slack ? total - slack : 0;
      for (;;) {
        unsigned have = 0;
        for (int c = 0; c < 8; c++) have += ctx->fields.hprog[c];
        if (have >= want || fmm_over()) break;
        if (std::chrono::steady_clock::now() - t_poll0 > std::chrono::seconds(120)) break;
        usleep(50);
      }
    }
    const unsigned nquad_all = (unsigned)((nray + RPW_MAX - 1) / RPW_MAX);
    unsigned pending = nquad_all, *h_traced = nullptr;
    { void *hp; if ((rc = dz_pinned(ctx, "rays.host_pending", 64, &hp))) return rc; h_traced = (unsigned *)hp; }
    DZ_HIP(hipMemsetAsync(A.defer_mark, 1, (size_t)nquad_all * 4, ctx->stream));
    int npass = 0;
    bool collected = false, ev0_set = false;
    unsigned left_by_first = 0;
    int rcf = 0;
    while (pending > 0) {
      const bool last = fmm_over();
      if (last && !collected) {
        swap.restore();
        DZ_HIP(hipStreamSynchronize(ctx->stream3));
        rcf = dz_fmm_finish(ctx);
        collected = true;
        if (rcf) break;
        if (npass == 0) (void)hipEventRecord(ctx->ev_r1, ctx->stream);
        (void)hipEventRecord(ctx->ev0, ctx->stream);
        ev0_set = true;
      }
      long nwg_pass = nwg;
      A.max_quads = 0;
      A.sweeps = collected ? 1 : 3;
      if (collected) A.fdone = nullptr;
      DZ_HIP(hipMemsetAsync(A.qcount, 0, 32, ctx->stream));
      if ((rc = launch(false, A, nwg_pass))) return rc;
      if (!collected) DZ_HIP(hipEventRecord(ctx->ev_r1, ctx->stream));
      DZ_HIP(hipMemcpyAsync(h_traced, A.qcount + 18, 4, hipMemcpyDeviceToHost, ctx->stream));
      DZ_HIP(hipStreamSynchronize(ctx->stream));
      const unsigned before = pending;
      pending = collected ? 0u : nquad_all - *h_traced;
      if (npass == 0) left_by_first = pending;
      npass++;
      if (pending > 0 && pending == before) usleep(100);
    }
    swap.restore();
    if (!collected) rcf = dz_fmm_finish(ctx);
    DZ_HIP(hipStreamSynchronize(ctx->stream3));
    if (rcf) return rcf;
    ctx->ksec["rays.passes"] = npass;
    ctx->ksec["rays.deferred_quads"] = left_by_first;
    A.fdone = nullptr; A.defer_mark = nullptr; A.max_quads = 0; A.sweeps = 1;
    float ms_tail = 0;
    if (hipEventElapsedTime(&ms_tail, ctx->ev_f1, ctx->ev_r1) == hipSuccess && ms_tail > 0) overlap_tail_s = ms_tail * 1e-3;
    if (!ev0_set) (void)hipEventRecord(ctx->ev0, ctx->stream);
    return 0;
  }
  int scan_and_emit(Arrays &M, long *count, int64_t slack, bool dense_twin) {
    int rc; void *p; size_t tb = 0;
    DZ_HIP(rocprim::exclusive_scan(nullptr, tb, count, (long *)M.rp, 0l, (size_t)(nray + 1), rocprim::plus<long>(), ctx->stream));
    if ((rc = dz_scratch(ctx, "rays.scan", tb + 256, &p))) return rc;
    DZ_HIP(rocprim::exclusive_scan(p, tb, count, (long *)M.rp, 0l, (size_t)(nray + 1), rocprim::plus<long>(), ctx->stream));
    DZ_HIP(hipMemcpyAsync(&M.nnz, M.rp + nray, 8, hipMemcpyDeviceToHost, ctx->stream));
    DZ_HIP(hipStreamSynchronize(ctx->stream));
    M.cap_nnz = M.nnz + slack;
    const size_t cap = (size_t)(M.cap_nnz > 0 ? M.cap_nnz : 1);
    if ((rc = dz_big_get(ctx, cap, &M.v)) || (rc = dz_big_get(ctx, cap, &M.cl))) return rc;
    RayArgs R = A;
    R.rowptr = (const long *)M.rp; R.val = M.v; R.col = M.cl;
    if (dense_twin) {
      R.dense = 1;
      DZ_HIP(hipMemsetAsync(A.qcount + 8, 0, 32, ctx->stream));
    }
    return nray > 0 ? launch(true, R, nwg) : 0;
  }
  int statuses() {
    int rc;
    std::vector<int> hs(nr1), hb(nr1);
    unsigned hq[2] = {0, 0};
    if (nray > 0) {
      DZ_HIP(hipMemcpyAsync(hq, A.qcount + 16, 8, hipMemcpyDeviceToHost, ctx->stream));
      DZ_HIP(hipMemcpyAsync(hs.data(), A.status, nray * 4, hipMemcpyDeviceToHost, ctx->stream));
      DZ_HIP(hipMemcpyAsync(hb.data(), A.rbflag, nray * 4, hipMemcpyDeviceToHost, ctx->stream));
      DZ_HIP(hipStreamSynchronize(ctx->stream));
    }
    int nb = 0, err = 0;
    for (int64_t i = 0; i < nray; i++) {
      nb += hb[i];
      if (hs[i] && !err) err = dz_fail(ctx, hs[i], "ray %ld: receiver lies outside model", (long)i);
    }
    if (n_boundary) *n_boundary = nb;
    if (nnz_out) *nnz_out = arrays.nnz;
    ctx->ksec["rays.list_sweeps"] = hq[0];
    ctx->ksec["rays.list_retraced"] = hq[1];
    ctx->ksec["rays.lcap"] = A.lcap;
    if ((rc = d.dsurf.finish())) return rc;
    DZ_HIP(hipStreamSynchronize(ctx->stream));
    return err;
  }
  int adopt() {
    int rc;
    const int64_t n = (int64_t)g.nvx * g.nvz * (map ? kmax : nz - 1) * (joint ? 3 : 1);
    arrays.keep = true;
    if ((rc = dz_csr_adopt_cap(ctx, nray, n, arrays.nnz, arrays.rp, arrays.cl, arrays.v, nray + res_rows, arrays.cap_nnz, G))) return rc;
    if (twin) {
      dazim_csr *Gd = nullptr;
      arrays_d.keep = true;
      if ((rc = dz_csr_adopt_cap(ctx, nray, n, arrays_d.nnz, arrays_d.rp, arrays_d.cl, arrays_d.v, 0, 0, &Gd)) || (rc = dz_csr_set_twin(ctx, *G, Gd))) {
        dazim_csr_free(ctx, *G);
        *G = nullptr;
        return rc;
      }
    }
    return 0;
  }
  int run() {
    int rc;
    if ((rc = check()) || (rc = decide_overlap()) || (rc = stage_inputs()) || (rc = kernel_constants()) || (rc = scratch()) ||
        (rc = launch_shape()) || (rc = sort_rays()))
      return rc;
    DzTimer t(ctx, "rays");
    DZ_HIP(hipMemsetAsync(A.count, 0, (size_t)(nray + 1) * 8, ctx->stream));
    if ((rc = overlap ? count_passes_beside_eikonal() : count_pass())) return rc;
    if ((rc = scan_and_emit(arrays, A.count, res_nnz, false))) return rc;
    if (twin && ((rc = dz_big_get(ctx, (size_t)(nray + 1), &arrays_d.rp)) || (rc = scan_and_emit(arrays_d, A.countd, 0, true)))) return rc;
    t.stop();
    if (overlap) {
      ctx->ksec["rays.after_fmm_count"] = overlap_tail_s;
      ctx->ksec["rays"] += overlap_tail_s;
    }
    return (rc = statuses()) ? rc : adopt();
  }
};

}

extern "C" int dazim_rays_build_G(dazim_ctx *ctx, int nx, int ny, int nz, float goxd, float gozd, float dvxd,
                                  float dvzd, int kmax, const float *vels, int nfield, const float *scx,
                                  const float *scz, const int *period, const int *kidx, const float *veln,
                                  const float *ttn, const float *ttnr, const int *nstsr, const dazim_refbox *boxes,
                                  int64_t nray, const int *field, const float *rcx, const float *rcz,
                                  const double *svs, const double *svp, const double *srho, float *dsurf,
                                  dazim_csr **G, int64_t *nnz_out, int *n_boundary) {
  RayBuild b(ctx);
  b.nx = nx; b.ny = ny; b.nz = nz; b.goxd = goxd; b.gozd = gozd; b.dvxd = dvxd; b.dvzd = dvzd;
  b.kmax = kmax; b.vels = vels; b.svs = svs; b.svp = svp; b.srho = srho;
  b.nfield = nfield; b.scx = scx; b.scz = scz; b.period = period; b.kidx = kidx;
  b.veln = veln; b.ttn = ttn; b.ttnr = ttnr; b.nstsr = nstsr; b.boxes = boxes;
  b.nray = nray; b.field = field; b.rcx = rcx; b.rcz = rcz;
  b.dsurf = dsurf; b.G = G; b.nnz_out = nnz_out; b.n_boundary = n_boundary;
  return b.run();
}
extern "C" int dazim_rays_build_G_joint(dazim_ctx *ctx, int nx, int ny, int nz, float goxd, float gozd, float dvxd,
                                        float dvzd, int kmax, const float *vels, int nfield, const float *scx,
                                        const float *scz, const int *period, const int *kidx, const float *veln,
                                        const float *ttn, const float *ttnr, const int *nstsr,
                                        const dazim_refbox *boxes, int64_t nray, const int *field, const float *rcx,
                                        const float *rcz, const double *svs, const double *svp, const double *srho,
                                        const float *lsen, float *dsurf, dazim_csr **G, int64_t *nnz_out,
                                        int *n_boundary) {
  if (!lsen) return dz_fail(ctx, DAZIM_E_BAD_ARG, "joint mode needs Lsen_Gsc");
  RayBuild b(ctx);
  b.nx = nx; b.ny = ny; b.nz = nz; b.goxd = goxd; b.gozd = gozd; b.dvxd = dvxd; b.dvzd = dvzd;
  b.kmax = kmax; b.vels = vels; b.svs = svs; b.svp = svp; b.srho = srho; b.lsen = lsen;
  b.nfield = nfield; b.scx = scx; b.scz = scz; b.period = period; b.kidx = kidx;
  b.veln = veln; b.ttn = ttn; b.ttnr = ttnr; b.nstsr = nstsr; b.boxes = boxes;
  b.nray = nray; b.field = field; b.rcx = rcx; b.rcz = rcz;
  b.dsurf = dsurf; b.G = G; b.nnz_out = nnz_out; b.n_boundary = n_boundary;
  return b.run();
}

extern "C" int dazim_rays_build_G_maps(dazim_ctx *ctx, int nx, int ny, float goxd, float gozd, float dvxd, float dvzd, int kmax,
                                       int azim, int nfield, const float *scx, const float *scz, const int *period,
                                       const float *veln, const float *ttn, const float *ttnr, const int *nstsr,
                                       const dazim_refbox *boxes, int64_t nray, const int *field, const float *rcx,
                                       const float *rcz, float *dsurf, dazim_csr **G, int64_t *nnz_out, int *n_boundary) {
  RayBuild b(ctx);
  b.map = true; b.azim = azim != 0;
  b.nx = nx; b.ny = ny; b.nz = 2; b.goxd = goxd; b.gozd = gozd; b.dvxd = dvxd; b.dvzd = dvzd;
  b.kmax = kmax; b.nfield = nfield; b.scx = scx; b.scz = scz; b.period = period;
  b.veln = veln; b.ttn = ttn; b.ttnr = ttnr; b.nstsr = nstsr; b.boxes = boxes;
  b.nray = nray; b.field = field; b.rcx = rcx; b.rcz = rcz;
  b.dsurf = dsurf; b.G = G; b.nnz_out = nnz_out; b.n_boundary = n_boundary;
  return b.run();
}

extern "C" int dazim_ray_paths_dims(dazim_ctx *ctx, int64_t *nray, int *cap) {
  if (!ctx || !nray || !cap) return DAZIM_E_BAD_ARG;
  *nray = (int64_t)dazim_last_kernel_seconds(ctx, "rays.path_rays");
  *cap = (int)dazim_last_kernel_seconds(ctx, "rays.path_cap");
  if (*nray < 0) *nray = 0;
  if (*cap < 0) *cap = 0;
  return 0;
}
extern "C" int dazim_ray_paths_copy(dazim_ctx *ctx, float *xz, int *nrp) {
  int64_t nray;
  int cap;
  if (!ctx || !xz || !nrp || dazim_ray_paths_dims(ctx, &nray, &cap)) return DAZIM_E_BAD_ARG;
  if (nray == 0 || cap == 0) return dz_fail(ctx, DAZIM_E_BAD_ARG, "no ray paths were kept (option rays.keep_paths)");
  auto a = ctx->scratch.find("rays.pts"), b = ctx->scratch.find("rays.npts");
  if (a == ctx->scratch.end() || b == ctx->scratch.end()) return dz_fail(ctx, DAZIM_E_BAD_ARG, "no ray paths were kept");
  DZ_HIP(hipMemcpyAsync(xz, a->second.first, (size_t)nray * cap * 8, hipMemcpyDefault, ctx->stream));
  DZ_HIP(hipMemcpyAsync(nrp, b->second.first, (size_t)nray * 4, hipMemcpyDefault, ctx->stream));
  DZ_HIP(hipStreamSynchronize(ctx->stream));
  return 0;
}
```

dazimsurftomo_amd/csrc/sparse.hip:

```cpp
#include "sparse_internal.h"

#include <type_traits>

#include <rocprim/device/device_radix_sort.hpp>
#include <rocprim/device/device_scan.hpp>

namespace {

__global__ __launch_bounds__(64 * WPB) void spmv_rows(int64_t nrows, const int64_t *__restrict__ ptr,
                                                        const int *__restrict__ idx,
                                                        const float *__restrict__ val,
                                                        const float *__restrict__ x, float *__restrict__ out,
                                                        const float *__restrict__ beta_p, float beta_sign,
                                                        double *__restrict__ sumsq, const int *__restrict__ guard) {
  if (guard && *guard) return;
  const int lane = threadIdx.x & 63, w = threadIdx.x >> 6;
  const float beta = beta_p ? beta_sign * beta_p[0] : beta_sign;
  double sq = 0.0;
  for (int64_t r = (int64_t)blockIdx.x * WPB + w; r < nrows; r += (int64_t)gridDim.x * WPB) {
    const int64_t s = ptr[r], e = ptr[r + 1];
    float acc = 0.0f;
    int64_t s4 = (s + 3) & ~(int64_t)3;
    if (s4 > e) s4 = e;
    for (int64_t i = s + lane; i < s4; i += 64) acc += val[i] * x[idx[i]];
    const int64_t e4 = s4 + ((e - s4) & ~(int64_t)3);
    for (int64_t i = s4 + 4 * lane; i < e4; i += 256) {
      const float4 v = *reinterpret_cast<const float4 *>(val + i);
      const int4 c = *reinterpret_cast<const int4 *>(idx + i);
      acc += v.x * x[c.x];
      acc += v.y * x[c.y];
      acc += v.z * x[c.z];
      acc += v.w * x[c.w];
    }
    for (int64_t i = e4 + lane; i < e; i += 64) acc += val[i] * x[idx[i]];
    acc = wave_sum(acc);
    if (lane == 0) {
      const float o = beta * out[r] + acc;
      out[r] = o;
      sq += (double)o * (double)o;
    }
  }
  if (sumsq) {
    __shared__ double s_sq[WPB];
    if (lane == 0) s_sq[w] = sq;
    __syncthreads();
    if (threadIdx.x == 0) {
      double t = 0.0;
      for (int i = 0; i < WPB; i++) t += s_sq[i];
      sumsq[blockIdx.x] = t;
    }
  }
}

constexpr int LWPB = 16;
template <class IT> struct Idx4;
template <> struct Idx4<int> { using type = int4; };
template <> struct Idx4<unsigned short> { using type = ushort4; };
template <class IT>
__global__ __launch_bounds__(64 * LWPB) void spmv_rows_ldsx(int64_t nrows, int64_t nx, const int64_t *__restrict__ ptr,
                                                           const IT *__restrict__ idx, const float *__restrict__ val,
                                                           const float *__restrict__ x, float *__restrict__ out,
                                                           const float *__restrict__ beta_p, float beta_sign,
                                                           double *__restrict__ sumsq, const int *__restrict__ guard) {
  extern __shared__ __attribute__((aligned(16))) float xs[];
  if (guard && *guard) return;
  for (int64_t i = threadIdx.x * 4; i < nx; i += 64 * LWPB * 4) {
    if (i + 3 < nx)
      *reinterpret_cast<float4 *>(xs + i) = *reinterpret_cast<const float4 *>(x + i);
    else
      for (int64_t j = i; j < nx; j++) xs[j] = x[j];
  }
  __syncthreads();
  const int lane = threadIdx.x & 63, w = threadIdx.x >> 6;
  const float beta = beta_p ? beta_sign * beta_p[0] : beta_sign;
  double sq = 0.0;
  for (int64_t r = (int64_t)blockIdx.x * LWPB + w; r < nrows; r += (int64_t)gridDim.x * LWPB) {
    const int64_t s = ptr[r], e = ptr[r + 1];
    float acc = 0.0f;
    int64_t s4 = (s + 3) & ~(int64_t)3;
    if (s4 > e) s4 = e;
    for (int64_t i = s + lane; i < s4; i += 64) acc += val[i] * xs[idx[i]];
    const int64_t e4 = s4 + ((e - s4) & ~(int64_t)3);
    int64_t i = s4 + 4 * lane;
    for (; i + 768 < e4; i += 1024) {
      using I4 = typename Idx4<IT>::type;
      float4 v[4];
      I4 c[4];
#pragma unroll
      for (int g = 0; g < 4; g++) {
        v[g] = *reinterpret_cast<const float4 *>(val + i + 256 * g);
        c[g] = *reinterpret_cast<const I4 *>(idx + i + 256 * g);
      }
#pragma unroll
      for (int g = 0; g < 4; g++) {
        acc += v[g].x * xs[c[g].x];
        acc += v[g].y * xs[c[g].y];
        acc += v[g].z * xs[c[g].z];
        acc += v[g].w * xs[c[g].w];
      }
    }
    for (; i + 256 < e4; i += 512) {
      using I4 = typename Idx4<IT>::type;
      const float4 v0 = *reinterpret_cast<const float4 *>(val + i);
      const I4 c0 = *reinterpret_cast<const I4 *>(idx + i);
      const float4 v1 = *reinterpret_cast<const float4 *>(val + i + 256);
      const I4 c1 = *reinterpret_cast<const I4 *>(idx + i + 256);
      acc += v0.x * xs[c0.x];
      acc += v0.y * xs[c0.y];
      acc += v0.z * xs[c0.z];
      acc += v0.w * xs[c0.w];
      acc += v1.x * xs[c1.x];
      acc += v1.y * xs[c1.y];
      acc += v1.z * xs[c1.z];
      acc += v1.w * xs[c1.w];
    }
    for (; i < e4; i += 256) {
      using I4 = typename Idx4<IT>::type;
      const float4 v = *reinterpret_cast<const float4 *>(val + i);
      const I4 c = *reinterpret_cast<const I4 *>(idx + i);
      acc += v.x * xs[c.x];
      acc += v.y * xs[c.y];
      acc += v.z * xs[c.z];
      acc += v.w * xs[c.w];
    }
    for (int64_t k = e4 + lane; k < e; k += 64) acc += val[k] * xs[idx[k]];
    acc = wave_sum(acc);
    if (lane == 0) {
      const float o = beta * out[r] + acc;
      out[r] = o;
      sq += (double)o * (double)o;
    }
  }
  if (sumsq) {
    __shared__ double s_sq[LWPB];
    if (lane == 0) s_sq[w] = sq;
    __syncthreads();
    if (threadIdx.x == 0) {
      double t = 0.0;
      for (int k = 0; k < LWPB; k++) t += s_sq[k];
      sumsq[blockIdx.x] = t;
    }
  }
}
__global__ void k_scale_rows(int64_t nrows, const int64_t *ptr, float *val, const float *w) {
  const int lane = threadIdx.x & 63, wv = threadIdx.x >> 6;
  for (int64_t r = (int64_t)blockIdx.x * WPB + wv; r < nrows; r += (int64_t)gridDim.x * WPB) {
    const float a = w[r];
    for (int64_t i = ptr[r] + lane; i < ptr[r + 1]; i += 64) val[i] *= a;
  }
}
__global__ void k_col_abs_sums(int64_t n, const int *col, const float *val, double scale, unsigned long long *acc) {
  for (int64_t i = (int64_t)blockIdx.x * VB + threadIdx.x; i < n; i += (int64_t)gridDim.x * VB)
    atomicAdd(&acc[col[i]], (unsigned long long)__double2ll_rn((double)fabsf(val[i]) * scale));
}
__global__ void k_fixed_to_float(int64_t n, const unsigned long long *acc, double inv_scale, float *out) {
  for (int64_t i = (int64_t)blockIdx.x * VB + threadIdx.x; i < n; i += (int64_t)gridDim.x * VB) out[i] = (float)((double)acc[i] * inv_scale);
}
__global__ void k_gather_f(int64_t n, const unsigned *perm, const float *src, float *dst) {
  for (int64_t i = (int64_t)blockIdx.x * VB + threadIdx.x; i < n; i += (int64_t)gridDim.x * VB) dst[i] = src[perm[i]];
}
__global__ void k_gather_i(int64_t n, const unsigned *perm, const int *src, int *dst, int add) {
  for (int64_t i = (int64_t)blockIdx.x * VB + threadIdx.x; i < n; i += (int64_t)gridDim.x * VB) dst[i] = src[perm ? perm[i] : (unsigned)i] + add;
}
__global__ void k_iota_keys(int64_t n, const int *one_based, unsigned *keys, unsigned *iota) {
  for (int64_t i = (int64_t)blockIdx.x * VB + threadIdx.x; i < n; i += (int64_t)gridDim.x * VB) {
    if (keys) keys[i] = (unsigned)(one_based[i] - 1);
    iota[i] = (unsigned)i;
  }
}
__global__ void k_lower_bound(int64_t nrows, int64_t nnz, const unsigned *keys, int64_t *ptr) {
  for (int64_t r = (int64_t)blockIdx.x * VB + threadIdx.x; r <= nrows; r += (int64_t)gridDim.x * VB) {
    int64_t lo = 0, hi = nnz;
    while (lo < hi) {
      const int64_t mid = (lo + hi) >> 1;
      if ((int64_t)keys[mid] < r) lo = mid + 1; else hi = mid;
    }
    ptr[r] = lo;
  }
}
__global__ void k_check_range(int64_t n, const int *a, int lo, int hi, int *bad) {
  for (int64_t i = (int64_t)blockIdx.x * VB + threadIdx.x; i < n; i += (int64_t)gridDim.x * VB)
    if (a[i] < lo || a[i] > hi) atomicOr(bad, 1);
}

constexpr int SCW = 16;
constexpr int CBW_MAX = 19 * 1024;

__global__ void k_colblock_ptr(int64_t nrows, int ncb, int cbw, const int64_t *__restrict__ ptr,
                               const int *__restrict__ col, int64_t *__restrict__ cbptr) {
  const int64_t t = (int64_t)blockIdx.x * VB + threadIdx.x;
  if (t >= nrows * (ncb + 1)) return;
  const int64_t r = t / (ncb + 1);
  const int b = (int)(t - r * (ncb + 1));
  int64_t lo = ptr[r], hi = ptr[r + 1];
  const int target = b * cbw;
  while (lo < hi) {
    const int64_t mid = (lo + hi) >> 1;
    if (col[mid] < target) lo = mid + 1; else hi = mid;
  }
  cbptr[t] = lo;
}
constexpr int SPLIT_SHORT = 64;
__global__ void k_last_long_row(int64_t nrows, const int64_t *__restrict__ ptr, int thresh, unsigned long long *res) {
  unsigned long long best = 0;
  for (int64_t r = (int64_t)blockIdx.x * VB + threadIdx.x; r < nrows; r += (int64_t)gridDim.x * VB)
    if (ptr[r + 1] - ptr[r] >= thresh) best = (unsigned long long)(r + 1);
#pragma unroll
  for (int o = 32; o > 0; o >>= 1) {
    const unsigned long long b = __shfl_xor(best, o);
    best = b > best ? b : best;
  }
  if ((threadIdx.x & 63) == 0 && best) atomicMax(res, best);
}
__global__ void k_narrow_cols(int64_t n, const int *__restrict__ col, unsigned short *__restrict__ col16, int mod) {
  for (int64_t i = ((int64_t)blockIdx.x * VB + threadIdx.x) * 4; i < n; i += (int64_t)gridDim.x * VB * 4) {
    if (i + 3 < n) {
      int4 c = *reinterpret_cast<const int4 *>(col + i);
      if (mod > 0) { c.x %= mod; c.y %= mod; c.z %= mod; c.w %= mod; }
      *reinterpret_cast<ushort4 *>(col16 + i) = make_ushort4((unsigned short)c.x, (unsigned short)c.y, (unsigned short)c.z, (unsigned short)c.w);
    } else {
      for (int64_t j = i; j < n; j++) col16[j] = (unsigned short)(mod > 0 ? col[j] % mod : col[j]);
    }
  }
}
__device__ __forceinline__ unsigned abs_bits(float x) { return __float_as_uint(x) & 0x7fffffffu; }
__device__ __forceinline__ unsigned umax2(unsigned a, unsigned b) { return a > b ? a : b; }
__global__ void k_absmax(int64_t n, const float *x, float *part) {
  unsigned v = 0u;
  const int64_t n4 = ((reinterpret_cast<uintptr_t>(x) & 15) == 0) ? n / 4 : 0;
  for (int64_t i = (int64_t)blockIdx.x * VB + threadIdx.x; i < n4; i += (int64_t)gridDim.x * VB) {
    const float4 q = reinterpret_cast<const float4 *>(x)[i];
    v = umax2(umax2(v, umax2(abs_bits(q.x), abs_bits(q.y))), umax2(abs_bits(q.z), abs_bits(q.w)));
  }
  for (int64_t i = n4 * 4 + (int64_t)blockIdx.x * VB + threadIdx.x; i < n; i += (int64_t)gridDim.x * VB) v = umax2(v, abs_bits(x[i]));
#pragma unroll
  for (int o = 32; o > 0; o >>= 1) v = umax2(v, (unsigned)__shfl_xor((int)v, o));
  __shared__ unsigned s[VB / 64];
  if ((threadIdx.x & 63) == 0) s[threadIdx.x >> 6] = v;
  __syncthreads();
  if (threadIdx.x == 0) {
    unsigned t = 0u;
    for (int i = 0; i < VB / 64; i++) t = umax2(t, s[i]);
    part[blockIdx.x] = __uint_as_float(t);
  }
}
__global__ void k_absmax_finish(const float *part, int np, float *res) {
  unsigned v = 0u;
  for (int i = threadIdx.x; i < np; i += 64) v = umax2(v, abs_bits(part[i]));
#pragma unroll
  for (int o = 32; o > 0; o >>= 1) v = umax2(v, (unsigned)__shfl_xor((int)v, o));
  if (threadIdx.x == 0) res[0] = __uint_as_float(v);
}

struct RowPtr { int64_t s, e; float aux; };
template <int GL, int NG, class IT, class PtrF, class ElemF, class EndF>
__device__ __forceinline__ void walk_rows(int64_t r_first, int64_t stride, int64_t nrows, int lane, const IT *__restrict__ col,
                                          const float *__restrict__ val, PtrF ptrf, ElemF elemf, EndF endf) {
  using I4 = typename Idx4<IT>::type;
  struct Ent { int64_t r, s4, e4; float aux; float4 v[NG]; I4 k[NG]; float hv, tv; int hk, tk; bool hh, ht; };
  auto load_ptr = [&](int64_t r) {
    RowPtr p = ptrf(r < nrows ? r : 0);
    if (r >= nrows) p.e = p.s;
    return p;
  };
  auto issue = [&](int64_t r, const RowPtr &p) {
    Ent t;
    t.r = r;
    t.aux = p.aux;
    t.s4 = (p.s + 3) & ~(int64_t)3;
    if (t.s4 > p.e) t.s4 = p.e;
    t.e4 = t.s4 + ((p.e - t.s4) & ~(int64_t)3);
#pragma unroll
    for (int g = 0; g < NG; g++) {
      const int64_t i = t.s4 + 4 * lane + (int64_t)g * 4 * GL;
      const int64_t j = i < t.e4 ? i : 0;
      t.v[g] = *reinterpret_cast<const float4 *>(val + j);
      t.k[g] = *reinterpret_cast<const I4 *>(col + j);
    }
    const int64_t ih = p.s + lane, it = t.e4 + lane;
    t.hh = ih < t.s4;
    t.ht = it < p.e;
    t.hv = val[t.hh ? ih : 0];
    t.hk = (int)col[t.hh ? ih : 0];
    t.tv = val[t.ht ? it : 0];
    t.tk = (int)col[t.ht ? it : 0];
    return t;
  };
  auto consume = [&](const Ent &t) {
    if (t.hh) elemf(t.hk, t.hv, t.aux);
#pragma unroll
    for (int g = 0; g < NG; g++) {
      const int64_t i = t.s4 + 4 * lane + (int64_t)g * 4 * GL;
      if (i < t.e4) {
        elemf((int)t.k[g].x, t.v[g].x, t.aux); elemf((int)t.k[g].y, t.v[g].y, t.aux);
        elemf((int)t.k[g].z, t.v[g].z, t.aux); elemf((int)t.k[g].w, t.v[g].w, t.aux);
      }
    }
    for (int64_t i = t.s4 + 4 * lane + (int64_t)NG * 4 * GL; i < t.e4; i += 4 * GL) {
      const float4 v = *reinterpret_cast<const float4 *>(val + i);
      const I4 k = *reinterpret_cast<const I4 *>(col + i);
      elemf((int)k.x, v.x, t.aux); elemf((int)k.y, v.y, t.aux); elemf((int)k.z, v.z, t.aux); elemf((int)k.w, v.w, t.aux);
    }
    if (t.ht) elemf(t.tk, t.tv, t.aux);
    endf(t.r, t.aux);
  };
  int64_t r = r_first;
  Ent eC = issue(r, load_ptr(r));
  RowPtr pB = load_ptr(r + stride);
  for (; r < nrows; r += stride) {
    const RowPtr pA = load_ptr(r + 2 * stride);
    const Ent eB = issue(r + stride, pB);
    consume(eC);
    eC = eB;
    pB = pA;
  }
}

template <int GL, int NG, class IT>
__global__ __launch_bounds__(64 * SCW) void spmvT_scatter(int64_t nsplit, int64_t nrows, int nchunk, int ncb, int cbw, int64_t ncols,
                                                          const int64_t *__restrict__ cbptr, const IT *__restrict__ col,
                                                          const float *__restrict__ val, const float *__restrict__ y,
                                                          double scale, long long *__restrict__ part, const int *__restrict__ guard,
                                                          int pairlocal) {
  extern __shared__ __attribute__((aligned(16))) long long acc[];
  if (guard && *guard) return;
  const int chunk = blockIdx.x / ncb, cb = blockIdx.x - chunk * ncb;
  const int c0 = cb * cbw;
  const int csub = pairlocal ? (cb & 1) * cbw : c0;
  const int width = (int)((ncols - c0) < cbw ? (ncols - c0) : cbw);
  for (int i = threadIdx.x; i < width; i += 64 * SCW) acc[i] = 0;
  __syncthreads();
  constexpr int RPWV = 64 / GL;
  const int lane = (threadIdx.x & 63) % GL, grp = (threadIdx.x & 63) / GL;
  constexpr double MAGIC = 6755399441055744.0;
  auto ptrf = [&](int64_t r) { return RowPtr{cbptr[r * (ncb + 1) + cb], cbptr[r * (ncb + 1) + cb + 1], y[r]}; };
  auto elemf = [&](int c, float v, float yr) {
    atomicAdd((unsigned long long *)&acc[c - csub],
              (unsigned long long)(__double_as_longlong(fma((double)(v * yr), scale, MAGIC)) - __double_as_longlong(MAGIC)));
  };
  walk_rows<GL, NG, IT>(((int64_t)chunk + (int64_t)nchunk * (threadIdx.x >> 6)) * RPWV + grp, (int64_t)nchunk * SCW * RPWV, nsplit, lane,
                        col, val, ptrf, elemf, [](int64_t, float) {});
  if (nsplit < nrows) {
    constexpr int GS = 16, RS = 64 / GS;
    const int lane_s = (threadIdx.x & 63) % GS, grp_s = (threadIdx.x & 63) / GS;
    walk_rows<GS, 1, IT>(nsplit + ((int64_t)chunk + (int64_t)nchunk * (threadIdx.x >> 6)) * RS + grp_s, (int64_t)nchunk * SCW * RS, nrows,
                         lane_s, col, val, ptrf, elemf, [](int64_t, float) {});
  }
  __syncthreads();
  long long *dst = part + (size_t)chunk * ncols + c0;
  for (int i = threadIdx.x; i < width; i += 64 * SCW) dst[i] = acc[i];
}
__global__ void k_scatter_combine(int64_t ncols, int nchunk, const long long *__restrict__ part, double inv_scale,
                                  float *__restrict__ out, const float *__restrict__ beta_p, float beta_sign,
                                  double *__restrict__ sumsq, const int *__restrict__ guard) {
  if (guard && *guard) return;
  const float beta = beta_p ? beta_sign * beta_p[0] : beta_sign;
  double sq = 0.0;
  for (int64_t c = (int64_t)blockIdx.x * VB + threadIdx.x; c < ncols; c += (int64_t)gridDim.x * VB) {
    long long t8[8] = {0, 0, 0, 0, 0, 0, 0, 0};
    int k = 0;
    for (; k + 8 <= nchunk; k += 8)
#pragma unroll
      for (int j = 0; j < 8; j++) t8[j] += part[(size_t)(k + j) * ncols + c];
    for (; k < nchunk; k++) t8[0] += part[(size_t)k * ncols + c];
    const long long t = ((t8[0] + t8[1]) + (t8[2] + t8[3])) + ((t8[4] + t8[5]) + (t8[6] + t8[7]));
    const float o = beta * out[c] + (float)((double)t * inv_scale);
    out[c] = o;
    sq += (double)o * o;
  }
  if (sumsq) block_partial(sq, sumsq);
}

template <int GL, int NG, class IT>
__global__ __launch_bounds__(64 * SCW) void spmv_rows_blocked(int64_t nsplit, int64_t nrows, int nset, int npair, int ncb, int cbw, int64_t ncols,
                                                              const int64_t *__restrict__ cbptr, const IT *__restrict__ col,
                                                              const float *__restrict__ val, const float *__restrict__ x,
                                                              float *__restrict__ part, const int *__restrict__ guard, int pairlocal) {
  extern __shared__ __attribute__((aligned(16))) float xblk[];
  if (guard && *guard) return;
  const int set = blockIdx.x / npair, pr = blockIdx.x - set * npair;
  const int cb0 = 2 * pr, cb1 = (cb0 + 2 < ncb) ? cb0 + 2 : ncb;
  const int c0 = cb0 * cbw;
  const int csub = pairlocal ? 0 : c0;
  const int width = (int)((ncols - c0) < 2 * (int64_t)cbw ? (ncols - c0) : 2 * (int64_t)cbw);
  for (int i = threadIdx.x; i < width; i += 64 * SCW) xblk[i] = x[c0 + i];
  __syncthreads();
  constexpr int RPWV = 64 / GL;
  const int lane = (threadIdx.x & 63) % GL, grp = (threadIdx.x & 63) / GL;
  float acc = 0.0f;
  float *dst = part + (size_t)pr * nrows;
  auto ptrf = [&](int64_t r) { return RowPtr{cbptr[r * (ncb + 1) + cb0], cbptr[r * (ncb + 1) + cb1], 0.0f}; };
  auto elemf = [&](int c, float v, float) { acc += v * xblk[c - csub]; };
  walk_rows<GL, NG, IT>(((int64_t)set + (int64_t)nset * (threadIdx.x >> 6)) * RPWV + grp, (int64_t)nset * SCW * RPWV, nsplit, lane, col, val,
                        ptrf, elemf, [&](int64_t r, float) {
                          float a = acc;
#pragma unroll
                          for (int o = GL / 2; o > 0; o >>= 1) a += __shfl_xor(a, o);
                          if (lane == 0 && r < nsplit) dst[r] = a;
                          acc = 0.0f;
                        });
  if (nsplit < nrows) {
    constexpr int GS = 16, RS = 64 / GS;
    const int lane_s = (threadIdx.x & 63) % GS, grp_s = (threadIdx.x & 63) / GS;
    acc = 0.0f;
    walk_rows<GS, 1, IT>(nsplit + ((int64_t)set + (int64_t)nset * (threadIdx.x >> 6)) * RS + grp_s, (int64_t)nset * SCW * RS, nrows, lane_s,
                         col, val, ptrf, elemf, [&](int64_t r, float) {
                           float a = acc;
#pragma unroll
                           for (int o = GS / 2; o > 0; o >>= 1) a += __shfl_xor(a, o);
                           if (lane_s == 0 && r < nrows) dst[r] = a;
                           acc = 0.0f;
                         });
  }
}
__global__ void k_rows_combine(int64_t nrows, int npair, const float *__restrict__ part, float *__restrict__ out,
                               const float *__restrict__ beta_p, float beta_sign, double *__restrict__ sumsq,
                               const int *__restrict__ guard) {
  if (guard && *guard) return;
  const float beta = beta_p ? beta_sign * beta_p[0] : beta_sign;
  double sq = 0.0;
  for (int64_t r = (int64_t)blockIdx.x * blockDim.x + threadIdx.x; r < nrows; r += (int64_t)gridDim.x * blockDim.x) {
    float t = part[r];
    for (int k = 1; k < npair; k++) t += part[(size_t)k * nrows + r];
    const float o = beta * out[r] + t;
    out[r] = o;
    sq += (double)o * o;
  }
  if (sumsq) block_partial(sq, sumsq);
}

constexpr int64_t LDSX_MAX = 38 * 1024;
bool use_ldsx(dazim_ctx *ctx, int64_t nrows, int64_t nx) {
  if (dz_opt(ctx, "spmv.ldsx", 1) == 0) return false;
  return nx <= LDSX_MAX && nrows >= (int64_t)ctx->num_cu * LWPB * 4;
}
int launch_spmv(dazim_ctx *ctx, int64_t nrows, int64_t nx, const int64_t *ptr, const int *idx, const float *val,
                const float *x, float *out, const float *beta_p, float beta_sign, double *sumsq,
                int nblocks, const int *guard = nullptr, const unsigned short *idx16 = nullptr) {
  if (use_ldsx(ctx, nrows, nx)) {
    const size_t lds = (size_t)((nx + 3) & ~(int64_t)3) * 4;
    if (idx16) {
      DZ_HIP(hipFuncSetAttribute((const void *)spmv_rows_ldsx<unsigned short>, hipFuncAttributeMaxDynamicSharedMemorySize, (int)lds));
      hipLaunchKernelGGL(spmv_rows_ldsx<unsigned short>, dim3(nblocks), dim3(64 * LWPB), lds, ctx->stream, nrows, nx, ptr, idx16, val,
                         x, out, beta_p, beta_sign, sumsq, guard);
    } else {
      DZ_HIP(hipFuncSetAttribute((const void *)spmv_rows_ldsx<int>, hipFuncAttributeMaxDynamicSharedMemorySize, (int)lds));
      hipLaunchKernelGGL(spmv_rows_ldsx<int>, dim3(nblocks), dim3(64 * LWPB), lds, ctx->stream, nrows, nx, ptr, idx, val, x, out,
                         beta_p, beta_sign, sumsq, guard);
    }
  } else {
    hipLaunchKernelGGL(spmv_rows, dim3(nblocks), dim3(64 * WPB), 0, ctx->stream, nrows, ptr, idx, val, x, out,
                       beta_p, beta_sign, sumsq, guard);
  }
  DZ_HIP(hipGetLastError());
  return 0;
}
__global__ void k_expand_rows(int64_t nrows, const int64_t *ptr, unsigned *rowid) {
  const int lane = threadIdx.x & 63, wv = threadIdx.x >> 6;
  for (int64_t r = (int64_t)blockIdx.x * WPB + wv; r < nrows; r += (int64_t)gridDim.x * WPB)
    for (int64_t i = ptr[r] + lane; i < ptr[r + 1]; i += 64) rowid[i] = (unsigned)r;
}
__global__ void k_offset_ptr(int64_t n, const int64_t *src, int64_t add, int64_t *dst) {
  for (int64_t i = (int64_t)blockIdx.x * VB + threadIdx.x; i < n; i += (int64_t)gridDim.x * VB) dst[i] = src[i] + add;
}
template <bool FILL>
__global__ __launch_bounds__(256) void k_threshold_rows(int64_t m, const int64_t *__restrict__ rowptr, const int *__restrict__ col,
                                                        const float *__restrict__ val, float tol, long *__restrict__ cnt,
                                                        const long *__restrict__ rowptr2, int *__restrict__ col2,
                                                        float *__restrict__ val2) {
  const int lane = threadIdx.x & 63;
  const int64_t r = (int64_t)blockIdx.x * 4 + (threadIdx.x >> 6);
  if (r > m) return;
  if (r == m) {
    if (!FILL && lane == 0) cnt[m] = 0;
    return;
  }
  const int64_t s = rowptr[r], e = rowptr[r + 1];
  long kept = 0;
  const long o = FILL ? rowptr2[r] : 0;
  for (int64_t i = s; i < e; i += 64) {
    const int64_t k = i + lane;
    float v = 0.0f;
    int c = 0;
    if (k < e) { v = val[k]; c = col[k]; }
    const bool keep = k < e && fabsf(v) > tol;
    const unsigned long long b = __ballot(keep);
    if (FILL && keep) {
      const long q = o + kept + __popcll(b & ((1ull << lane) - 1ull));
      val2[q] = v;
      col2[q] = c;
    }
    kept += __popcll(b);
  }
  if (!FILL && lane == 0) cnt[r] = kept;
}

bool use_blocked(dazim_ctx *ctx, const dazim_csr *A) {
  if (dz_opt(ctx, "spmv.blocked", 1) == 0) return false;
  return A->cbptr && A->n > LDSX_MAX && A->nnz >= (1 << 22) && A->m >= (int64_t)ctx->num_cu * SCW;
}
int absmax_to_host(dazim_ctx *ctx, const float *x, int64_t n, float *res) {
  int rc;
  float *pm;
  if ((rc = dz_scratch(ctx, "csr.absmax", (size_t)APART + 4, &pm))) return rc;
  const int nb = nblk((n + 3) / 4, APART);
  hipLaunchKernelGGL(k_absmax, dim3(nb), dim3(VB), 0, ctx->stream, n, x, pm);
  hipLaunchKernelGGL(k_absmax_finish, dim3(1), dim3(64), 0, ctx->stream, pm, nb, pm + APART);
  DZ_HIP(hipMemcpyAsync(res, pm + APART, 4, hipMemcpyDeviceToHost, ctx->stream));
  return 0;
}
double fixed_scale(double pm, int64_t m) {
  int e = 0;
  if (pm > 0) (void)frexp(pm, &e);
  int lgm = 0;
  while (((int64_t)1 << lgm) < m) lgm++;
  const int fb = 62 - lgm < 40 ? 62 - lgm : 40;
  return ldexp(1.0, fb - e);
}
struct RowSplit { int64_t nsplit; bool shortseg; };
RowSplit row_split(dazim_ctx *ctx, const dazim_csr *A, double thresh) {
  const bool split = dz_opt(ctx, "spmv.split", 1) != 0 && A->split_row < A->m;
  return {split ? A->split_row : A->m, (split ? A->long_avg : (double)A->nnz / (double)A->m) < thresh};
}
template <class F>
int dispatch_rows(const dazim_csr *A, bool shortseg, F launch) {
  using GL16 = std::integral_constant<int, 16>; using NG2 = std::integral_constant<int, 2>;
  using GL64 = std::integral_constant<int, 64>; using NG4 = std::integral_constant<int, 4>;
  if (A->col16) return shortseg ? launch(GL16(), NG2(), A->col16) : launch(GL64(), NG4(), A->col16);
  return shortseg ? launch(GL16(), NG2(), A->col) : launch(GL64(), NG4(), A->col);
}

}

int dz_spmv_blocks(dazim_ctx *ctx, int64_t nrows, int64_t nx) {
  if (nx >= 0 && use_ldsx(ctx, nrows, nx)) return ctx->num_cu;
  int64_t b = (nrows + WPB - 1) / WPB;
  const int64_t cap = (int64_t)ctx->num_cu * 8;
  if (b > cap) b = cap;
  if (b < 1) b = 1;
  return (int)b;
}

int dz_invalidate_transpose(dazim_csr *A) {
  for (void **pp : {(void **)&A->colptr, (void **)&A->row, (void **)&A->tval, (void **)&A->tperm})
    if (*pp) { (void)hipFree(*pp); *pp = nullptr; }
  return 0;
}
int dz_build_transpose(dazim_ctx *ctx, dazim_csr *A) {
  const int64_t nnz = A->nnz, n = A->n, m = A->m;
  const size_t nz = (size_t)(nnz > 0 ? nnz : 1);
  (void)dz_invalidate_transpose(A);
  DZ_HIP(dz_malloc_retry(ctx, (void **)&A->colptr, (n + 1) * 8));
  DZ_HIP(dz_malloc_retry(ctx, (void **)&A->row, nz * 4));
  DZ_HIP(dz_malloc_retry(ctx, (void **)&A->tval, nz * 4));
  DZ_HIP(dz_malloc_retry(ctx, (void **)&A->tperm, nz * 4));
  if (nnz == 0) {
    DZ_HIP(hipMemsetAsync(A->colptr, 0, (n + 1) * 8, ctx->stream));
    return 0;
  }
  int rc;
  unsigned *ck, *cks, *iota, *rowid;
  if ((rc = dz_scratch(ctx, "csr.k0", nz, &ck)) || (rc = dz_scratch(ctx, "csr.k1", nz, &cks)) ||
      (rc = dz_scratch(ctx, "csr.v0", nz, &iota)) || (rc = dz_scratch(ctx, "csr.perm", nz, &rowid)))
    return rc;
  const int nb = nblk(nnz);
  int cbits = 1;
  while (((int64_t)1 << cbits) < n) cbits++;
  hipLaunchKernelGGL(k_gather_i, dim3(nb), dim3(VB), 0, ctx->stream, nnz, (const unsigned *)nullptr, A->col, (int *)ck, 0);
  hipLaunchKernelGGL(k_iota_keys, dim3(nb), dim3(VB), 0, ctx->stream, nnz, (const int *)nullptr, (unsigned *)nullptr, iota);
  hipLaunchKernelGGL(k_expand_rows, dim3(dz_spmv_blocks(ctx, m, -1)), dim3(64 * WPB), 0, ctx->stream, m, A->rowptr, rowid);
  size_t tb = 0;
  DZ_HIP(rocprim::radix_sort_pairs(nullptr, tb, ck, cks, iota, A->tperm, (size_t)nnz, 0, cbits, ctx->stream));
  void *tmp;
  if ((rc = dz_scratch(ctx, "csr.tmp", tb + 256, &tmp))) return rc;
  DZ_HIP(rocprim::radix_sort_pairs(tmp, tb, ck, cks, iota, A->tperm, (size_t)nnz, 0, cbits, ctx->stream));
  hipLaunchKernelGGL(k_lower_bound, dim3(nblk(n + 1)), dim3(VB), 0, ctx->stream, n, nnz, cks, A->colptr);
  hipLaunchKernelGGL(k_gather_f, dim3(nb), dim3(VB), 0, ctx->stream, nnz, A->tperm, A->val, A->tval);
  hipLaunchKernelGGL(k_gather_i, dim3(nb), dim3(VB), 0, ctx->stream, nnz, A->tperm, (const int *)rowid, A->row, 0);
  DZ_HIP(hipGetLastError());
  return 0;
}

int dz_build_colblocks(dazim_ctx *ctx, dazim_csr *A, int64_t changed_from) {
  if (A->cbptr) { dz_big_put(ctx, A->cbptr); A->cbptr = nullptr; }
  A->ncb = (int)((A->n + CBW_MAX - 1) / CBW_MAX);
  A->cbw = (int)(((A->n + A->ncb - 1) / A->ncb + 3) & ~3ll);
  const int mod16 = A->n <= 65536 ? 0 : 2 * A->cbw;
  const bool want16 = mod16 <= 65536 && A->nnz > 0 && dz_opt(ctx, "spmv.col16", 1) != 0;
  if (A->col16 && (!want16 || A->col16_cap < A->nnz || changed_from == 0 || A->col16_mod != mod16)) {
    dz_big_put(ctx, A->col16);
    A->col16 = nullptr;
    A->col16_cap = 0;
  }
  if (want16 && (!A->col16 || changed_from >= 0)) {
    int64_t from = 0;
    if (!A->col16) {
      A->col16_cap = ((A->cap_nnz > A->nnz ? A->cap_nnz : A->nnz) + 3) & ~(int64_t)3;
      if (int rcp = dz_big_get(ctx, (size_t)A->col16_cap, &A->col16)) return rcp;
      A->col16_mod = mod16;
    } else {
      from = changed_from & ~(int64_t)3;
    }
    const int64_t cnt = A->nnz - from;
    if (cnt > 0)
      hipLaunchKernelGGL(k_narrow_cols, dim3(nblk((cnt + 3) / 4)), dim3(VB), 0, ctx->stream, cnt, A->col + from, A->col16 + from, mod16);
    DZ_HIP(hipGetLastError());
  }
  const int64_t np = A->m * (A->ncb + 1);
  if (np > 0) {
    if (int rcp = dz_big_get(ctx, (size_t)np, &A->cbptr)) return rcp;
    hipLaunchKernelGGL(k_colblock_ptr, dim3((unsigned)((np + VB - 1) / VB)), dim3(VB), 0, ctx->stream, A->m, A->ncb, A->cbw,
                       A->rowptr, A->col, A->cbptr);
    DZ_HIP(hipGetLastError());
  }
  int rc;
  A->vmax = 0.0f;
  A->split_row = A->m;
  A->long_avg = A->m > 0 ? (double)A->nnz / (double)A->m : 0.0;
  if (A->m > 0 && A->nnz > 0) {
    float *pm;
    if ((rc = dz_scratch(ctx, "csr.absmax", (size_t)APART + 4, &pm))) return rc;
    unsigned long long *d_last = reinterpret_cast<unsigned long long *>(pm + APART + 2), h_last = 0;
    DZ_HIP(hipMemsetAsync(d_last, 0, 8, ctx->stream));
    hipLaunchKernelGGL(k_last_long_row, dim3(nblk(A->m)), dim3(VB), 0, ctx->stream, A->m, A->rowptr, SPLIT_SHORT, d_last);
    DZ_HIP(hipMemcpyAsync(&h_last, d_last, 8, hipMemcpyDeviceToHost, ctx->stream));
    DZ_HIP(hipStreamSynchronize(ctx->stream));
    if ((int64_t)h_last < A->m && (int64_t)h_last > 0) {
      int64_t at = 0;
      DZ_HIP(hipMemcpy(&at, A->rowptr + h_last, 8, hipMemcpyDeviceToHost));
      A->split_row = (int64_t)h_last;
      A->long_avg = (double)at / (double)h_last;
    }
  }
  if (A->nnz > 0 && (rc = absmax_to_host(ctx, A->val, A->nnz, &A->vmax))) return rc;
  DZ_HIP(hipStreamSynchronize(ctx->stream));
  return 0;
}
bool dz_use_scatter(dazim_ctx *ctx, const dazim_csr *A) {
  if (dz_opt(ctx, "spmv.scatter", 1) == 0) return false;
  return A->cbptr && A->nnz >= (1 << 22) && A->m >= (int64_t)ctx->num_cu * SCW;
}
int dz_launch_spmvT(dazim_ctx *ctx, const dazim_csr *A, const float *y, float ymax, float *out, const float *beta_p,
                    float beta_sign, double *sumsq, int *npart, const int *guard) {
  const double pm = (double)A->vmax * (double)ymax;
  ctx->ksec["spmvt.kind"] = (dz_use_scatter(ctx, A) && std::isfinite(pm)) ? 1 : 0;
  ctx->ksec["spmvt.idx_bytes"] = (A->col16 && dz_use_scatter(ctx, A) && std::isfinite(pm)) ? 2 : 4;
  ctx->ksec["spmvt.lanes"] = 0;
  ctx->ksec["spmv.ncb"] = A->ncb;
  ctx->ksec["spmv.cbw"] = A->cbw;
  if (!dz_use_scatter(ctx, A) || !std::isfinite(pm)) {
    if (!A->colptr) {
      int rc0 = dz_build_transpose(ctx, const_cast<dazim_csr *>(A));
      if (rc0) return rc0;
    }
    const int gn = dz_spmv_blocks(ctx, A->n, A->m);
    if (npart) *npart = gn;
    return launch_spmv(ctx, A->n, A->m, A->colptr, A->row, A->tval, y, out, beta_p, beta_sign, sumsq, gn, guard);
  }
  int nchunk = ctx->num_cu / A->ncb;
  if (nchunk < 1) nchunk = 1;
  int rc;
  long long *part;
  if ((rc = dz_scratch(ctx, "spmvt.part", (size_t)nchunk * A->n, &part))) return rc;
  const double scale = fixed_scale(pm, A->m);
  const size_t lds = (size_t)A->cbw * 8;
  const RowSplit rs = row_split(ctx, A, 400.0 * A->ncb);
  ctx->ksec["spmvt.split_row"] = (double)rs.nsplit;
  const dim3 sgrid(nchunk * A->ncb), sblock(64 * SCW);
  rc = dispatch_rows(A, rs.shortseg, [&](auto gl, auto ng, auto *colp) -> int {
    using IT = std::remove_pointer_t<decltype(colp)>;
    const auto kern = spmvT_scatter<decltype(gl)::value, decltype(ng)::value, IT>;
    ctx->ksec["spmvt.lanes"] = decltype(gl)::value;
    DZ_HIP(hipFuncSetAttribute((const void *)kern, hipFuncAttributeMaxDynamicSharedMemorySize, (int)lds));
    hipLaunchKernelGGL(kern, sgrid, sblock, lds, ctx->stream, rs.nsplit, A->m, nchunk, A->ncb, A->cbw, A->n, A->cbptr,
                       (const IT *)colp, A->val, y, scale, part, guard, (sizeof(IT) == 2 && A->col16_mod > 0) ? 1 : 0);
    return 0;
  });
  if (rc) return rc;
  const int nb = nblk(A->n, NPART);
  hipLaunchKernelGGL(k_scatter_combine, dim3(nb), dim3(VB), 0, ctx->stream, A->n, nchunk, part, 1.0 / scale, out, beta_p,
                     beta_sign, sumsq, guard);
  DZ_HIP(hipGetLastError());
  if (npart) *npart = nb;
  return 0;
}

int dz_launch_spmvA(dazim_ctx *ctx, const dazim_csr *A, const float *x, float *out, const float *beta_p, float beta_sign,
                    double *sumsq, int *npart, const int *guard) {
  ctx->ksec["spmv.kind"] = use_blocked(ctx, A) ? 2 : (use_ldsx(ctx, A->m, A->n) ? 1 : 0);
  ctx->ksec["spmv.idx_bytes"] = (A->col16 && (use_blocked(ctx, A) || (use_ldsx(ctx, A->m, A->n) && A->col16_mod == 0))) ? 2 : 4;
  ctx->ksec["spmv.lanes"] = 0;
  ctx->ksec["spmv.ncb"] = A->ncb;
  ctx->ksec["spmv.cbw"] = A->cbw;
  if (!use_blocked(ctx, A)) {
    const int gm = dz_spmv_blocks(ctx, A->m, A->n);
    if (npart) *npart = gm;
    return launch_spmv(ctx, A->m, A->n, A->rowptr, A->col, A->val, x, out, beta_p, beta_sign, sumsq, gm, guard,
                       A->col16_mod == 0 ? A->col16 : nullptr);
  }
  const int npair = (A->ncb + 1) / 2;
  int nset = ctx->num_cu / npair;
  if (nset < 1) nset = 1;
  int rc;
  float *part;
  if ((rc = dz_scratch(ctx, "spmv.part", (size_t)npair * A->m, &part))) return rc;
  const size_t lds = (size_t)A->cbw * 2 * 4;
  const RowSplit rs = row_split(ctx, A, 600.0 * npair);
  ctx->ksec["spmv.split_row"] = (double)rs.nsplit;
  const dim3 bgrid(nset * npair), bblock(64 * SCW);
  rc = dispatch_rows(A, rs.shortseg, [&](auto gl, auto ng, auto *colp) -> int {
    using IT = std::remove_pointer_t<decltype(colp)>;
    const auto kern = spmv_rows_blocked<decltype(gl)::value, decltype(ng)::value, IT>;
    ctx->ksec["spmv.lanes"] = decltype(gl)::value;
    DZ_HIP(hipFuncSetAttribute((const void *)kern, hipFuncAttributeMaxDynamicSharedMemorySize, (int)lds));
    hipLaunchKernelGGL(kern, bgrid, bblock, lds, ctx->stream, rs.nsplit, A->m, nset, npair, A->ncb, A->cbw, A->n, A->cbptr,
                       (const IT *)colp, A->val, x, part, guard, (sizeof(IT) == 2 && A->col16_mod > 0) ? 1 : 0);
    return 0;
  });
  if (rc) return rc;
  const int nb = nblk(A->m, NPART);
  hipLaunchKernelGGL(k_rows_combine, dim3(nb), dim3(VB), 0, ctx->stream, A->m, npair, part, out, beta_p, beta_sign, sumsq, guard);
  DZ_HIP(hipGetLastError());
  if (npart) *npart = nb;
  return 0;
}
int dz_scale_rows(dazim_ctx *ctx, dazim_csr *A, int64_t nrows, const float *w) {
  hipLaunchKernelGGL(k_scale_rows, dim3(dz_spmv_blocks(ctx, nrows, -1)), dim3(64 * WPB), 0, ctx->stream, nrows, A->rowptr, A->val, w);
  if (A->tperm) hipLaunchKernelGGL(k_gather_f, dim3(nblk(A->nnz)), dim3(VB), 0, ctx->stream, A->nnz, A->tperm, A->val, A->tval);
  DZ_HIP(hipGetLastError());
  DZ_HIP(hipStreamSynchronize(ctx->stream));
  return dz_build_colblocks(ctx, A, -1);
}

extern "C" {

int dz_csr_set_twin(dazim_ctx *ctx, dazim_csr *A, dazim_csr *B) {
  if (!A || !B || A->twin) return dz_fail(ctx, DAZIM_E_BAD_ARG, "bad arguments to dz_csr_set_twin");
  A->twin = B;
  return 0;
}
int dazim_csr_take_twin(dazim_ctx *ctx, dazim_csr *A, dazim_csr **twin) {
  if (!A || !twin) return dz_fail(ctx, DAZIM_E_BAD_ARG, "bad arguments to dazim_csr_take_twin");
  *twin = A->twin;
  A->twin = nullptr;
  return 0;
}

int dazim_csr_free(dazim_ctx *ctx, dazim_csr *A) {
  if (!A) return 0;
  if (A->twin) { dazim_csr *t = A->twin; A->twin = nullptr; (void)dazim_csr_free(ctx, t); }
  if (ctx) DZ_HIP(hipStreamSynchronize(ctx->stream));
  else (void)hipDeviceSynchronize();
  void *ps[] = {A->rowptr, A->colptr, A->col, A->row, A->val, A->tval, A->tperm, A->cbptr, A->col16};
  for (void *p : ps)
    if (p) dz_big_put(ctx, p);
  delete A;
  return 0;
}

int dazim_csr_dims(const dazim_csr *A, int64_t *m, int64_t *n, int64_t *nnz) {
  if (!A) return DAZIM_E_BAD_ARG;
  if (m) *m = A->m;
  if (n) *n = A->n;
  if (nnz) *nnz = A->nnz;
  return 0;
}

int dazim_csr_from_coo(dazim_ctx *ctx, int64_t m, int64_t n, int64_t nnz, const int *irow_u,
                       const int *icol_u, const float *rw_u, dazim_csr **out) {
  if (!ctx || !out || m < 1 || n < 1 || nnz < 0 || nnz > 0xfffffff0ll || m > 0x7ffffff0 || n > 0x7ffffff0)
    return dz_fail(ctx, DAZIM_E_BAD_ARG, "bad arguments to dazim_csr_from_coo");
  DZ_HIP(hipSetDevice(ctx->device));
  DzBuf<int> irow, icol;
  DzBuf<float> rw;
  int rc;
  if ((rc = irow.init(ctx, irow_u, nnz, true, false))) return rc;
  if ((rc = icol.init(ctx, icol_u, nnz, true, false))) return rc;
  if ((rc = rw.init(ctx, rw_u, nnz, true, false))) return rc;
  dazim_csr *A = new dazim_csr;
  auto fail = [&](int r) { dazim_csr_free(ctx, A); return r; };
  A->m = m;
  A->n = n;
  A->nnz = nnz;
  const size_t nz = (size_t)(nnz > 0 ? nnz : 1);
  if ((rc = dz_big_get(ctx, (size_t)m + 1, &A->rowptr)) || (rc = dz_big_get(ctx, nz, &A->col)) || (rc = dz_big_get(ctx, nz, &A->val)))
    return fail(rc);
  unsigned *k0, *k1, *v0, *perm;
  int *bad;
  if ((rc = dz_scratch(ctx, "csr.k0", nz, &k0)) || (rc = dz_scratch(ctx, "csr.k1", nz, &k1)) ||
      (rc = dz_scratch(ctx, "csr.v0", nz, &v0)) || (rc = dz_scratch(ctx, "csr.perm", nz, &perm)) ||
      (rc = dz_scratch(ctx, "csr.bad", 4, &bad)))
    return fail(rc);
  DZ_HIP(hipMemsetAsync(bad, 0, 4, ctx->stream));
  const int nb = nblk(nnz);
  if (nnz > 0) {
    hipLaunchKernelGGL(k_check_range, dim3(nb), dim3(VB), 0, ctx->stream, nnz, irow.dev, 1, (int)m, bad);
    hipLaunchKernelGGL(k_check_range, dim3(nb), dim3(VB), 0, ctx->stream, nnz, icol.dev, 1, (int)n, bad);
    int hbad = 0;
    DZ_HIP(hipMemcpyAsync(&hbad, bad, 4, hipMemcpyDeviceToHost, ctx->stream));
    DZ_HIP(hipStreamSynchronize(ctx->stream));
    if (hbad) {
      dazim_csr_free(ctx, A);
      return dz_fail(ctx, DAZIM_E_BAD_ARG, "COO index outside 1..m / 1..n");
    }
    int rbits = 1, cbits = 1;
    while (((int64_t)1 << rbits) < m) rbits++;
    while (((int64_t)1 << cbits) < n) cbits++;
    unsigned *permc;
    if ((rc = dz_scratch(ctx, "csr.permc", nz, &permc))) return fail(rc);
    hipLaunchKernelGGL(k_iota_keys, dim3(nb), dim3(VB), 0, ctx->stream, nnz, icol.dev, k0, v0);
    size_t tb = 0, tb1 = 0;
    DZ_HIP(rocprim::radix_sort_pairs(nullptr, tb, k0, k1, v0, permc, (size_t)nnz, 0, cbits, ctx->stream));
    DZ_HIP(rocprim::radix_sort_pairs(nullptr, tb1, k0, k1, permc, perm, (size_t)nnz, 0, rbits, ctx->stream));
    if (tb1 > tb) tb = tb1;
    void *tmp;
    if ((rc = dz_scratch(ctx, "csr.tmp", tb + 256, &tmp))) return fail(rc);
    DZ_HIP(rocprim::radix_sort_pairs(tmp, tb, k0, k1, v0, permc, (size_t)nnz, 0, cbits, ctx->stream));
    hipLaunchKernelGGL(k_gather_i, dim3(nb), dim3(VB), 0, ctx->stream, nnz, permc, irow.dev, (int *)k0, -1);
    DZ_HIP(rocprim::radix_sort_pairs(tmp, tb, k0, k1, permc, perm, (size_t)nnz, 0, rbits, ctx->stream));
    hipLaunchKernelGGL(k_lower_bound, dim3(nblk(m + 1)), dim3(VB), 0, ctx->stream, m, nnz, k1, A->rowptr);
    hipLaunchKernelGGL(k_gather_f, dim3(nb), dim3(VB), 0, ctx->stream, nnz, perm, rw.dev, A->val);
    hipLaunchKernelGGL(k_gather_i, dim3(nb), dim3(VB), 0, ctx->stream, nnz, perm, icol.dev, A->col, -1);
    DZ_HIP(hipGetLastError());
  } else {
    DZ_HIP(hipMemsetAsync(A->rowptr, 0, (m + 1) * 8, ctx->stream));
  }
  if ((rc = dz_build_colblocks(ctx, A))) return fail(rc);
  if ((rc = dz_invalidate_transpose(A))) return fail(rc);
  DZ_HIP(hipStreamSynchronize(ctx->stream));
  *out = A;
  return 0;
}

int dazim_csr_adopt(dazim_ctx *ctx, int64_t m, int64_t n, int64_t nnz, int64_t *rowptr, int *col, float *val,
                    dazim_csr **out) {
  return dz_csr_adopt_cap(ctx, m, n, nnz, rowptr, col, val, 0, 0, out);
}

int dz_csr_adopt_cap(dazim_ctx *ctx, int64_t m, int64_t n, int64_t nnz, int64_t *rowptr, int *col, float *val,
                     int64_t cap_m, int64_t cap_nnz, dazim_csr **out) {
  if (!ctx || !out || !rowptr) return DAZIM_E_BAD_ARG;
  dazim_csr *A = new dazim_csr;
  A->m = m; A->n = n; A->nnz = nnz;
  A->rowptr = rowptr; A->col = col; A->val = val;
  if (cap_m > m) A->cap_m = cap_m;
  if (cap_nnz > nnz) A->cap_nnz = cap_nnz;
  int rc;
  if ((rc = dz_build_colblocks(ctx, A)) || (rc = dz_invalidate_transpose(A))) {
    dazim_csr_free(ctx, A);
    return rc;
  }
  DZ_HIP(hipStreamSynchronize(ctx->stream));
  *out = A;
  return 0;
}

int dazim_csr_threshold(dazim_ctx *ctx, const dazim_csr *A, float tol, int64_t reserve_rows, int64_t reserve_nnz, dazim_csr **out) {
  if (!ctx || !A || !out || reserve_rows < 0 || reserve_nnz < 0) return dz_fail(ctx, DAZIM_E_BAD_ARG, "bad arguments to dazim_csr_threshold");
  DZ_HIP(hipSetDevice(ctx->device));
  const int64_t m = A->m;
  int rc;
  long *cnt;
  if ((rc = dz_scratch(ctx, "thr.cnt", (size_t)(m + 1), &cnt))) return rc;
  int64_t *rowptr = nullptr;
  float *val = nullptr;
  int *col = nullptr;
  struct Arrays {
    dazim_ctx *c; int64_t *&rp; float *&v; int *&cl; bool keep = false;
    ~Arrays() { if (!keep) { dz_big_put(c, rp); dz_big_put(c, v); dz_big_put(c, cl); } }
  } arrays{ctx, rowptr, val, col};
  if ((rc = dz_big_get(ctx, (size_t)(m + reserve_rows + 1), &rowptr))) return rc;
  const unsigned nb = (unsigned)((m + 1 + 3) / 4);
  hipLaunchKernelGGL((k_threshold_rows<false>), dim3(nb), dim3(256), 0, ctx->stream, m, A->rowptr, A->col, A->val, tol, cnt,
                     (const long *)nullptr, (int *)nullptr, (float *)nullptr);
  size_t tb = 0;
  DZ_HIP(rocprim::exclusive_scan(nullptr, tb, cnt, (long *)rowptr, 0l, (size_t)(m + 1), rocprim::plus<long>(), ctx->stream));
  void *p;
  if ((rc = dz_scratch(ctx, "thr.scan", tb + 256, &p))) return rc;
  DZ_HIP(rocprim::exclusive_scan(p, tb, cnt, (long *)rowptr, 0l, (size_t)(m + 1), rocprim::plus<long>(), ctx->stream));
  long nnz = 0;
  DZ_HIP(hipMemcpyAsync(&nnz, rowptr + m, 8, hipMemcpyDeviceToHost, ctx->stream));
  DZ_HIP(hipStreamSynchronize(ctx->stream));
  const int64_t cap = nnz + reserve_nnz;
  if ((rc = dz_big_get(ctx, (size_t)(cap > 0 ? cap : 1), &val)) || (rc = dz_big_get(ctx, (size_t)(cap > 0 ? cap : 1), &col))) return rc;
  hipLaunchKernelGGL((k_threshold_rows<true>), dim3(nb), dim3(256), 0, ctx->stream, m, A->rowptr, A->col, A->val, tol, cnt,
                     (const long *)rowptr, col, val);
  DZ_HIP(hipGetLastError());
  arrays.keep = true;
  return dz_csr_adopt_cap(ctx, m, A->n, nnz, rowptr, col, val, m + reserve_rows, cap, out);
}

int dazim_csr_append_coo(dazim_ctx *ctx, dazim_csr *A, int64_t extra_m, int64_t nnz2, const int *irow_u,
                         const int *icol_u, const float *rw_u) {
  if (!ctx || !A || extra_m < 0 || nnz2 < 0) return DAZIM_E_BAD_ARG;
  if (extra_m == 0 && nnz2 == 0) return 0;
  DzBuf<int> irow;
  int rc;
  if ((rc = irow.init(ctx, irow_u, nnz2, true, false))) return rc;
  int *shifted;
  if ((rc = dz_scratch(ctx, "csr.shift", (size_t)(nnz2 > 0 ? nnz2 : 1), &shifted))) return rc;
  if (nnz2 > 0) hipLaunchKernelGGL(k_gather_i, dim3(nblk(nnz2)), dim3(VB), 0, ctx->stream, nnz2, (const unsigned *)nullptr, irow.dev, shifted, (int)-A->m);
  dazim_csr *B = nullptr;
  if ((rc = dazim_csr_from_coo(ctx, extra_m > 0 ? extra_m : 1, A->n, nnz2, shifted, icol_u, rw_u, &B))) return rc;
  const int64_t m2 = A->m + extra_m, nz2 = A->nnz + nnz2;
  if (A->cap_m >= m2 && A->cap_nnz >= nz2) {
    const int64_t nnz1 = A->nnz;
    if (extra_m > 0)
      hipLaunchKernelGGL(k_offset_ptr, dim3(nblk(extra_m + 1)), dim3(VB), 0, ctx->stream, extra_m + 1, B->rowptr, A->nnz, A->rowptr + A->m);
    DZ_HIP(hipMemcpyAsync(A->col + nnz1, B->col, (size_t)nnz2 * 4, hipMemcpyDeviceToDevice, ctx->stream));
    DZ_HIP(hipMemcpyAsync(A->val + nnz1, B->val, (size_t)nnz2 * 4, hipMemcpyDeviceToDevice, ctx->stream));
    DZ_HIP(hipStreamSynchronize(ctx->stream));
    dazim_csr_free(ctx, B);
    A->m = m2;
    A->nnz = nz2;
    if ((rc = dz_build_colblocks(ctx, A, nnz1 > 0 ? nnz1 : 0))) return rc;
    if ((rc = dz_invalidate_transpose(A))) return rc;
    DZ_HIP(hipStreamSynchronize(ctx->stream));
    return 0;
  }
  int64_t *rowptr;
  int *col;
  float *val;
  if ((rc = dz_big_get(ctx, (size_t)(m2 + 1), &rowptr)) || (rc = dz_big_get(ctx, (size_t)(nz2 > 0 ? nz2 : 1), &col)) ||
      (rc = dz_big_get(ctx, (size_t)(nz2 > 0 ? nz2 : 1), &val)))
    return rc;
  DZ_HIP(hipMemcpyAsync(rowptr, A->rowptr, (A->m + 1) * 8, hipMemcpyDeviceToDevice, ctx->stream));
  if (extra_m > 0)
    hipLaunchKernelGGL(k_offset_ptr, dim3(nblk(extra_m + 1)), dim3(VB), 0, ctx->stream, extra_m + 1, B->rowptr, A->nnz, rowptr + A->m);
  DZ_HIP(hipMemcpyAsync(col, A->col, (size_t)A->nnz * 4, hipMemcpyDeviceToDevice, ctx->stream));
  DZ_HIP(hipMemcpyAsync(val, A->val, (size_t)A->nnz * 4, hipMemcpyDeviceToDevice, ctx->stream));
  DZ_HIP(hipMemcpyAsync(col + A->nnz, B->col, (size_t)nnz2 * 4, hipMemcpyDeviceToDevice, ctx->stream));
  DZ_HIP(hipMemcpyAsync(val + A->nnz, B->val, (size_t)nnz2 * 4, hipMemcpyDeviceToDevice, ctx->stream));
  DZ_HIP(hipStreamSynchronize(ctx->stream));
  dazim_csr_free(ctx, B);
  dz_big_put(ctx, A->rowptr);
  dz_big_put(ctx, A->col);
  dz_big_put(ctx, A->val);
  A->rowptr = rowptr; A->col = col; A->val = val;
  A->m = m2; A->nnz = nz2;
  A->cap_m = A->cap_nnz = 0;
  if ((rc = dz_build_colblocks(ctx, A))) return rc;
  if ((rc = dz_invalidate_transpose(A))) return rc;
  DZ_HIP(hipStreamSynchronize(ctx->stream));
  return 0;
}

int dazim_csr_to_coo(dazim_ctx *ctx, const dazim_csr *A, int *irow_u, int *icol_u, float *rw_u) {
  if (!ctx || !A) return DAZIM_E_BAD_ARG;
  DzBuf<int> irow, icol;
  DzBuf<float> rw;
  int rc;
  if ((rc = irow.init(ctx, irow_u, A->nnz, false, true))) return rc;
  if ((rc = icol.init(ctx, icol_u, A->nnz, false, true))) return rc;
  if ((rc = rw.init(ctx, rw_u, A->nnz, false, true))) return rc;
  if (A->nnz > 0) {
    unsigned *rowid;
    if ((rc = dz_scratch(ctx, "csr.perm", (size_t)A->nnz, &rowid))) return rc;
    hipLaunchKernelGGL(k_expand_rows, dim3(dz_spmv_blocks(ctx, A->m, -1)), dim3(64 * WPB), 0, ctx->stream, A->m, A->rowptr, rowid);
    const int nb = nblk(A->nnz);
    if (irow.dev) hipLaunchKernelGGL(k_gather_i, dim3(nb), dim3(VB), 0, ctx->stream, A->nnz, (const unsigned *)nullptr, (const int *)rowid, irow.dev, 1);
    if (icol.dev) hipLaunchKernelGGL(k_gather_i, dim3(nb), dim3(VB), 0, ctx->stream, A->nnz, (const unsigned *)nullptr, A->col, icol.dev, 1);
    if (rw.dev) DZ_HIP(hipMemcpyAsync(rw.dev, A->val, (size_t)A->nnz * 4, hipMemcpyDeviceToDevice, ctx->stream));
    DZ_HIP(hipGetLastError());
  }
  if ((rc = irow.finish()) || (rc = icol.finish()) || (rc = rw.finish())) return rc;
  DZ_HIP(hipStreamSynchronize(ctx->stream));
  return 0;
}

int dazim_csr_scale_rows(dazim_ctx *ctx, dazim_csr *A, const float *w_u) {
  if (!ctx || !A || !w_u) return DAZIM_E_BAD_ARG;
  DzBuf<float> w;
  int rc;
  if ((rc = w.init(ctx, w_u, A->m, true, false))) return rc;
  return dz_scale_rows(ctx, A, A->m, w.dev);
}

int dazim_csr_col_abs_sums(dazim_ctx *ctx, const dazim_csr *A, float *out_u) {
  if (!ctx || !A || !out_u) return DAZIM_E_BAD_ARG;
  DzBuf<float> out;
  int rc;
  if ((rc = out.init(ctx, out_u, A->n, false, true))) return rc;
  unsigned long long *acc;
  if ((rc = dz_scratch(ctx, "csr.colacc", (size_t)A->n, &acc))) return rc;
  DZ_HIP(hipMemsetAsync(acc, 0, (size_t)A->n * 8, ctx->stream));
  const double scale = fixed_scale((double)A->vmax, A->m);
  if (A->nnz) hipLaunchKernelGGL(k_col_abs_sums, dim3(nblk(A->nnz)), dim3(VB), 0, ctx->stream, A->nnz, A->col, A->val, scale, acc);
  hipLaunchKernelGGL(k_fixed_to_float, dim3(nblk(A->n)), dim3(VB), 0, ctx->stream, A->n, acc, 1.0 / scale, out.dev);
  DZ_HIP(hipGetLastError());
  if ((rc = out.finish())) return rc;
  DZ_HIP(hipStreamSynchronize(ctx->stream));
  return 0;
}

int dazim_aprod(dazim_ctx *ctx, int mode, const dazim_csr *A, float *x_u, float *y_u) {
  if (!ctx || !A || !x_u || !y_u || (mode != 1 && mode != 2)) return dz_fail(ctx, DAZIM_E_BAD_ARG, "bad arguments to dazim_aprod");
  DZ_HIP(hipSetDevice(ctx->device));
  DzBuf<float> x, y;
  int rc;
  if ((rc = x.init(ctx, x_u, A->n, true, mode == 2))) return rc;
  if ((rc = y.init(ctx, y_u, A->m, true, mode == 1))) return rc;
  if (mode == 1) {
    DzTimer t(ctx, "spmv");
    if ((rc = dz_launch_spmvA(ctx, A, x.dev, y.dev, nullptr, 1.0f, nullptr, nullptr))) return rc;
    t.stop();
  } else {
    float ymax = 1.0f;
    if (dz_use_scatter(ctx, A)) {
      if ((rc = absmax_to_host(ctx, y.dev, A->m, &ymax))) return rc;
      DZ_HIP(hipStreamSynchronize(ctx->stream));
    }
    DzTimer t(ctx, "spmvt");
    if ((rc = dz_launch_spmvT(ctx, A, y.dev, ymax, x.dev, nullptr, 1.0f, nullptr, nullptr))) return rc;
    t.stop();
  }
  if ((rc = x.finish()) || (rc = y.finish())) return rc;
  DZ_HIP(hipStreamSynchronize(ctx->stream));
  return 0;
}

}
```

dazimsurftomo_amd/csrc/sparse_internal.h:

```cpp
#pragma once
#include "dazim_internal.h"

struct dazim_csr {
  int64_t m = 0, n = 0, nnz = 0;
  int64_t *rowptr = nullptr, *colptr = nullptr;
  int *col = nullptr, *row = nullptr;
  float *val = nullptr, *tval = nullptr;
  unsigned *tperm = nullptr;
  int ncb = 0, cbw = 0;
  int64_t *cbptr = nullptr;
  float vmax = 0.0f;
  int64_t split_row = 0;
  double long_avg = 0.0;
  unsigned short *col16 = nullptr;
  int64_t col16_cap = 0;
  int col16_mod = 0;
  int64_t cap_m = 0, cap_nnz = 0;
  dazim_csr *twin = nullptr;
};

constexpr int WPB = 4;
constexpr int VB = 256;
constexpr int NPART = 256;
constexpr int APART = 2048;

__device__ __forceinline__ float wave_sum(float v) {
#pragma unroll
  for (int o = 32; o > 0; o >>= 1) v += __shfl_xor(v, o);
  return v;
}
__device__ __forceinline__ double wave_sum(double v) {
#pragma unroll
  for (int o = 32; o > 0; o >>= 1) v += __shfl_xor(v, o);
  return v;
}
__device__ __forceinline__ void block_partial(double v, double *part) {
  __shared__ double s[VB / 64];
  v = wave_sum(v);
  if ((threadIdx.x & 63) == 0) s[threadIdx.x >> 6] = v;
  __syncthreads();
  if (threadIdx.x == 0) {
    double t = 0.0;
    for (int i = 0; i < VB / 64; i++) t += s[i];
    part[blockIdx.x] = t;
  }
}
inline int nblk(int64_t n, int cap = 2048) {
  int64_t b = (n + VB - 1) / VB;
  if (b < 1) b = 1;
  return (int)(b > cap ? cap : b);
}

#pragma GCC visibility push(hidden)
int dz_spmv_blocks(dazim_ctx *ctx, int64_t nrows, int64_t nx = -1);
bool dz_use_scatter(dazim_ctx *ctx, const dazim_csr *A);
int dz_launch_spmvA(dazim_ctx *ctx, const dazim_csr *A, const float *x, float *out, const float *beta_p, float beta_sign,
                    double *sumsq, int *npart, const int *guard = nullptr);
int dz_launch_spmvT(dazim_ctx *ctx, const dazim_csr *A, const float *y, float ymax, float *out, const float *beta_p,
                    float beta_sign, double *sumsq, int *npart, const int *guard = nullptr);
int dz_build_transpose(dazim_ctx *ctx, dazim_csr *A);
int dz_invalidate_transpose(dazim_csr *A);
int dz_build_colblocks(dazim_ctx *ctx, dazim_csr *A, int64_t changed_from = 0);
int dz_scale_rows(dazim_ctx *ctx, dazim_csr *A, int64_t nrows, const float *w);
#pragma GCC visibility pop
```

Baseline: 56920.

## Emit col16 and vmax during ray emission and make CSR derived-data build incremental

The ray emit kernel now writes the 16-bit column copy directly and tracks the absolute maximum value with an atomic, so adopting the CSR can skip the separate col16 and absmax passes. Column-block pointers and long-row detection are recomputed only for appended rows, and several host round trips are merged into one pinned readback. Ray status checks move from copying whole arrays to the host to a small device reduction. An optional, off-by-default LDS-staged vectorised emit path is added. The changes add kernel complexity and extra global writes during emission in exchange for fewer separate passes and synchronisations.

New measurement: 57210 (median of 6 runs). Within noise of the previous version (+0.5%).

```diff
diff --git a/dazimsurftomo_amd/csrc/assemble.hip b/dazimsurftomo_amd/csrc/assemble.hip
--- a/dazimsurftomo_amd/csrc/assemble.hip
+++ b/dazimsurftomo_amd/csrc/assemble.hip
@@ -265,12 +265,12 @@
   const int64_t m2 = A->m + nrow, nz2 = A->nnz + nnz2;
   if (nz2 > 0xfffffff0ll) return dz_fail(ctx, DAZIM_E_NNZ_OVERFLOW, "too many stored entries");
   if (A->cap_m >= m2 && A->cap_nnz >= nz2) {
-    const int64_t nnz1 = A->nnz;
+    const int64_t nnz1 = A->nnz, m1 = A->m;
     fill(A->rowptr + A->m, A->col, A->val);
     DZ_HIP(hipGetLastError());
     A->m = m2;
     A->nnz = nz2;
-    if ((rc = dz_build_colblocks(ctx, A, nnz1 > 0 ? nnz1 : 0))) return rc;
+    if ((rc = dz_build_colblocks(ctx, A, nnz1 > 0 ? nnz1 : 0, m1))) return rc;
     if ((rc = dz_invalidate_transpose(A))) return rc;
     DZ_HIP(hipStreamSynchronize(ctx->stream));
     return 0;
diff --git a/dazimsurftomo_amd/csrc/emit_pieces.h b/dazimsurftomo_amd/csrc/emit_pieces.h
--- /dev/null
+++ b/dazimsurftomo_amd/csrc/emit_pieces.h
@@ -0,0 +1,19 @@
+#pragma once
+#if defined(__HIPCC__)
+#define DZ_EMIT_HD __host__ __device__ static inline
+#else
+#define DZ_EMIT_HD static inline
+#endif
+
+typedef struct { int head, body, tail; } dz_emit_run;
+
+DZ_EMIT_HD dz_emit_run dz_emit_pieces(long first, int len) {
+  dz_emit_run r;
+  r.head = (int)((4 - (first & 3)) & 3);
+  if (r.head > len) r.head = len;
+  r.body = (len - r.head) / 4;
+  r.tail = len - r.head - 4 * r.body;
+  return r;
+}
+DZ_EMIT_HD int dz_emit_cap_min(int gp) { return gp + 4; }
+DZ_EMIT_HD int dz_emit_full(long first, long next, int gp, int cap) { return (next - (first & ~3l)) + gp > cap; }
diff --git a/dazimsurftomo_amd/csrc/rays.hip b/dazimsurftomo_amd/csrc/rays.hip
--- a/dazimsurftomo_amd/csrc/rays.hip
+++ b/dazimsurftomo_amd/csrc/rays.hip
@@ -2,7 +2,8 @@
 #include <chrono>
 #include <unistd.h>
 
-#include "dazim_internal.h"
+#include "sparse_internal.h"
+#include "emit_pieces.h"
 
 #include <rocprim/device/device_scan.hpp>
 #include <rocprim/device/device_radix_sort.hpp>
@@ -70,6 +71,10 @@
   const long *rowptr;
   float *val;
   int *col;
+  unsigned short *col16;
+  int mod16;
+  unsigned *vmax_out;
+  int stage_cap;
 };
 
 __device__ __forceinline__ float dz_sinf(float x) {
@@ -233,6 +238,10 @@
   const unsigned nvx_magic = A.nvx_magic;
   const int LC = A.lcap;
   unsigned short *s_list = s_lists + (size_t)grp * LC;
+  const int SC = EMIT ? A.stage_cap : 0;
+  float *s_val = reinterpret_cast<float *>(reinterpret_cast<char *>(s_lists) + (((size_t)RPW * LC * 2 + 15) & ~(size_t)15)) + (size_t)grp * SC * 2;
+  int *s_col = reinterpret_cast<int *>(s_val + SC);
+  unsigned vmx = 0u;
   float *gfdm = A.fdm_scratch + ((size_t)blockIdx.x * RPW + grp) * nf * NG;
   float *gfdmc = gfdm + nf, *gfdms = gfdm + 2 * nf;
   __shared__ int s_rngs[RPW][4];
@@ -683,6 +692,39 @@
         cbase[i] = (jj - 1) * nvx + kk;
         fidx[i] = jj * ldf + kk;
       }
+      const bool staged = EMIT && SC > 0;
+      long sfirst = rstart;
+      auto put16 = [&](int c) { return (unsigned short)(A.mod16 > 0 ? c % A.mod16 : c); };
+      auto flush_run = [&](long next) {
+        cbar();
+        const dz_emit_run run = dz_emit_pieces(sfirst, (int)(next - sfirst));
+        const long gbase = sfirst & ~3l;
+        if (gl < run.head) {
+          const long p = sfirst + gl;
+          const int c = s_col[p - gbase];
+          A.val[p] = s_val[p - gbase];
+          A.col[p] = c;
+          if (A.col16) A.col16[p] = put16(c);
+        }
+        const long b0 = sfirst + run.head;
+        for (int pc = gl; pc < run.body; pc += GP) {
+          const long p = b0 + 4 * pc;
+          const float4 v = *reinterpret_cast<const float4 *>(s_val + (p - gbase));
+          const int4 c = *reinterpret_cast<const int4 *>(s_col + (p - gbase));
+          *reinterpret_cast<float4 *>(A.val + p) = v;
+          *reinterpret_cast<int4 *>(A.col + p) = c;
+          if (A.col16) *reinterpret_cast<ushort4 *>(A.col16 + p) = make_ushort4(put16(c.x), put16(c.y), put16(c.z), put16(c.w));
+        }
+        if (gl < run.tail) {
+          const long p = b0 + 4 * run.body + gl;
+          const int c = s_col[p - gbase];
+          A.val[p] = s_val[p - gbase];
+          A.col[p] = c;
+          if (A.col16) A.col16[p] = put16(c);
+        }
+        cbar();
+        sfirst = next;
+      };
       for (int blk = 0; blk < NG; blk++) {
         float fdv[RC];
         const float *fsrc = blk == 0 ? gfdm : (blk == 1 ? gfdmc : gfdms);
@@ -705,15 +747,25 @@
               keep = A.keep_small ? (rowv != 0.0f) : (fabsf(rowv) > FTOL);
             }
             const unsigned m = (unsigned)((__ballot(keep) >> gmask_shift) & GMASK);
+            if (staged && dz_emit_full(sfirst, rstart + cnt, GP, SC)) flush_run(rstart + cnt);
             if (EMIT && keep) {
               const long pos = rstart + cnt + __popc(m & ((1u << gl) - 1u));
-              A.val[pos] = rowv;
-              A.col[pos] = nk + cbase[i] - 1;
+              const int c = nk + cbase[i] - 1;
+              vmx = max(vmx, __float_as_uint(rowv) & 0x7fffffffu);
+              if (staged) {
+                s_val[pos - (sfirst & ~3l)] = rowv;
+                s_col[pos - (sfirst & ~3l)] = c;
+              } else {
+                A.val[pos] = rowv;
+                A.col[pos] = c;
+                if (A.col16) A.col16[pos] = put16(c);
+              }
             }
             cnt += __popc(m);
           }
         }
       }
+      if (staged) flush_run(rstart + cnt);
     } else
     for (int blk = 0; blk < NG; blk++)
       for (int k = 1; k <= nlay; k++) {
@@ -769,8 +821,10 @@
           const unsigned m = (unsigned)((__ballot(keep) >> gmask_shift) & GMASK);
           if (EMIT && keep) {
             const long pos = rstart + cnt + __popc(m & ((1u << gl) - 1u));
+            vmx = max(vmx, __float_as_uint(rowv) & 0x7fffffffu);
             A.val[pos] = rowv;
             A.col[pos] = nn - 1;
+            if (A.col16) A.col16[pos] = (unsigned short)(A.mod16 > 0 ? (nn - 1) % A.mod16 : nn - 1);
           }
           cnt += __popc(m);
         }
@@ -799,9 +853,38 @@
       if (!status && nlist > A.LK) atomicAdd(&A.qcount[17], 1u);
     }
   }
+  if (EMIT) {
+    RAYS_ARGS_FRESH;
+#pragma unroll
+    for (int o = 32; o > 0; o >>= 1) vmx = max(vmx, (unsigned)__shfl_xor((int)vmx, o));
+    if (lane == 0 && vmx && A.vmax_out) atomicMax(A.vmax_out, vmx);
+  }
 }
 #undef A
 #undef RAYS_ARGS_FRESH
+
+struct RayStatusOut { unsigned long long first; int code, nb; };
+__global__ void k_ray_status(long nray, const int *__restrict__ status, const int *__restrict__ rbflag, RayStatusOut *out) {
+  unsigned long long first = ~0ull;
+  int nb = 0;
+  for (long i = (long)blockIdx.x * blockDim.x + threadIdx.x; i < nray; i += (long)gridDim.x * blockDim.x) {
+    nb += rbflag[i];
+    if (status[i] && first == ~0ull) first = (unsigned long long)i;
+  }
+#pragma unroll
+  for (int o = 32; o > 0; o >>= 1) {
+    nb += __shfl_xor(nb, o);
+    const unsigned long long f = __shfl_xor(first, o);
+    first = f < first ? f : first;
+  }
+  if ((threadIdx.x & 63) == 0) {
+    if (nb) atomicAdd(&out->nb, nb);
+    if (first != ~0ull) atomicMin(&out->first, first);
+  }
+}
+__global__ void k_ray_status_code(long nray, const int *__restrict__ status, RayStatusOut *out) {
+  out->code = out->first < (unsigned long long)nray ? status[out->first] : 0;
+}
 
 struct RayBuild {
   dazim_ctx *ctx;
@@ -834,11 +917,16 @@
   } d;
   struct Arrays {
     dazim_ctx *c; int64_t *rp = nullptr; float *v = nullptr; int *cl = nullptr; int64_t nnz = 0, cap_nnz = 0; bool keep = false;
-    ~Arrays() { if (!keep) { dz_big_put(c, rp); dz_big_put(c, v); dz_big_put(c, cl); } }
+    unsigned short *c16 = nullptr; int64_t c16_cap = 0;
+    ~Arrays() {
+      if (!keep) { dz_big_put(c, rp); dz_big_put(c, v); dz_big_put(c, cl); }
+      if (c16) dz_big_put(c, c16);
+    }
   } arrays, arrays_d;
   dazim_geom g;
   bool joint = false, tiled = false, overlap = false, twin = false;
-  size_t nn = 0, nr = 0, ncol = 0, nk = 0, nr1 = 0, lds = 0;
+  size_t nn = 0, nr = 0, ncol = 0, nk = 0, nr1 = 0, lds = 0, lds_emit = 0;
+  bool hand_over = false, hand_over_G = false;
   int64_t res_rows = 0, res_nnz = 0;
   long nwg = 0;
   double overlap_tail_s = 0.0;
@@ -989,6 +1077,7 @@
     if ((rc = dz_big_get(ctx, (size_t)(nray + res_rows + 1), &arrays.rp))) return rc;
     A.dsurf = d.dsurf.dev;
     A.rowptr = (const long *)arrays.rp; A.val = nullptr; A.col = nullptr;
+    A.col16 = nullptr; A.mod16 = 0; A.vmax_out = nullptr; A.stage_cap = 0;
     return 0;
   }
   template <int I> static const void *kernel_no() { return (const void *)rays_kernel<(I & 8) != 0, (I & 4) != 0, (I & 2) != 0, (I & 1) != 0>; }
@@ -1001,13 +1090,21 @@
   int launch(bool emit, const RayArgs &R, long nwg_) {
     RayArgs args = R;
     void *params[] = {&args};
-    DZ_HIP(hipLaunchKernel(kern(emit), dim3((unsigned)nwg_), dim3(64), params, lds, ctx->stream));
+    DZ_HIP(hipLaunchKernel(kern(emit), dim3((unsigned)nwg_), dim3(64), params, emit ? lds_emit : lds, ctx->stream));
     return 0;
   }
   int launch_shape() {
     lds = (size_t)A.lcap * 2 * RPW_MAX + 16;
+    A.stage_cap = 0;
+    if (dz_opt(ctx, "rays.emit_staged", 0) != 0) {
+      A.stage_cap = dz_opt(ctx, "rays.stage_cap", 128);
+      if (A.stage_cap < dz_emit_cap_min(GP_EMIT) || A.stage_cap > 2048 || A.stage_cap % 4)
+        return dz_fail(ctx, DAZIM_E_BAD_ARG, "option rays.stage_cap: a multiple of 4 in %d..2048", dz_emit_cap_min(GP_EMIT));
+    }
+    ctx->ksec["rays.stage_cap"] = A.stage_cap;
+    lds_emit = (((size_t)A.lcap * 2 * (64 / GP_EMIT) + 15) & ~(size_t)15) + (size_t)A.stage_cap * 8 * (64 / GP_EMIT) + 16;
     DZ_HIP(hipFuncSetAttribute(kern(false), hipFuncAttributeMaxDynamicSharedMemorySize, (int)lds));
-    DZ_HIP(hipFuncSetAttribute(kern(true), hipFuncAttributeMaxDynamicSharedMemorySize, (int)lds));
+    DZ_HIP(hipFuncSetAttribute(kern(true), hipFuncAttributeMaxDynamicSharedMemorySize, (int)lds_emit));
     int per_cu = (int)(160 * 1024 / (lds + 256));
     {
       int occ = 0;
@@ -1141,6 +1238,19 @@
     if ((rc = dz_big_get(ctx, cap, &M.v)) || (rc = dz_big_get(ctx, cap, &M.cl))) return rc;
     RayArgs R = A;
     R.rowptr = (const long *)M.rp; R.val = M.v; R.col = M.cl;
+    R.col16 = nullptr; R.mod16 = 0; R.vmax_out = nullptr;
+    hand_over = !dense_twin && nray > 0 && dz_opt(ctx, "csr.rebuild", 0) == 0;
+    if (hand_over) {
+      const int64_t n = ncols();
+      if (dz_want_col16(ctx, n, M.nnz)) {
+        M.c16_cap = dz_col16_cap(M.nnz, M.cap_nnz);
+        if ((rc = dz_big_get(ctx, (size_t)M.c16_cap, &M.c16))) return rc;
+        R.col16 = M.c16;
+        R.mod16 = dz_col_shape(n).mod16;
+      }
+      R.vmax_out = A.qcount + 24;
+    }
+    if (((uintptr_t)M.v | (uintptr_t)M.cl | (uintptr_t)M.c16) & 15) R.stage_cap = 0;
     if (dense_twin) {
       R.dense = 1;
       DZ_HIP(hipMemsetAsync(A.qcount + 8, 0, 32, ctx->stream));
@@ -1149,18 +1259,36 @@
   }
   int statuses() {
     int rc;
-    std::vector<int> hs(nr1), hb(nr1);
     unsigned hq[2] = {0, 0};
-    if (nray > 0) {
+    int nb = 0, err = 0;
+    if (nray > 0 && dz_opt(ctx, "rays.status_host", 0) != 0) {
+      std::vector<int> hs(nr1), hb(nr1);
       DZ_HIP(hipMemcpyAsync(hq, A.qcount + 16, 8, hipMemcpyDeviceToHost, ctx->stream));
       DZ_HIP(hipMemcpyAsync(hs.data(), A.status, nray * 4, hipMemcpyDeviceToHost, ctx->stream));
       DZ_HIP(hipMemcpyAsync(hb.data(), A.rbflag, nray * 4, hipMemcpyDeviceToHost, ctx->stream));
       DZ_HIP(hipStreamSynchronize(ctx->stream));
-    }
-    int nb = 0, err = 0;
-    for (int64_t i = 0; i < nray; i++) {
-      nb += hb[i];
-      if (hs[i] && !err) err = dz_fail(ctx, hs[i], "ray %ld: receiver lies outside model", (long)i);
+      for (int64_t i = 0; i < nray; i++) {
+        nb += hb[i];
+        if (hs[i] && !err) err = dz_fail(ctx, hs[i], "ray %ld: receiver lies outside model", (long)i);
+      }
+    } else if (nray > 0) {
+      RayStatusOut *dst, *hst;
+      void *hp;
+      if ((rc = dz_scratch(ctx, "rays.status_out", 1, &dst)) || (rc = dz_pinned(ctx, "rays.host_status", 64, &hp))) return rc;
+      hst = (RayStatusOut *)hp;
+      hst->first = ~0ull; hst->code = 0; hst->nb = 0;
+      DZ_HIP(hipMemcpyAsync(dst, hst, sizeof(RayStatusOut), hipMemcpyHostToDevice, ctx->stream));
+      const unsigned nbk = (unsigned)((nray + 255) / 256 < 1024 ? (nray + 255) / 256 : 1024);
+      hipLaunchKernelGGL(k_ray_status, dim3(nbk), dim3(256), 0, ctx->stream, (long)nray, (const int *)A.status, (const int *)A.rbflag, dst);
+      hipLaunchKernelGGL(k_ray_status_code, dim3(1), dim3(1), 0, ctx->stream, (long)nray, (const int *)A.status, dst);
+      DZ_HIP(hipGetLastError());
+      DZ_HIP(hipMemcpyAsync(hst, dst, sizeof(RayStatusOut), hipMemcpyDeviceToHost, ctx->stream));
+      DZ_HIP(hipMemcpyAsync(hst + 1, A.qcount + 16, 8, hipMemcpyDeviceToHost, ctx->stream));
+      DZ_HIP(hipStreamSynchronize(ctx->stream));
+      memcpy(hq, hst + 1, 8);
+      nb = hst->nb;
+      if (hst->first < (unsigned long long)nray && hst->code)
+        err = dz_fail(ctx, hst->code, "ray %ld: receiver lies outside model", (long)hst->first);
     }
     if (n_boundary) *n_boundary = nb;
     if (nnz_out) *nnz_out = arrays.nnz;
@@ -1171,11 +1299,18 @@
     DZ_HIP(hipStreamSynchronize(ctx->stream));
     return err;
   }
+  int64_t ncols() const { return (int64_t)g.nvx * g.nvz * (map ? kmax : nz - 1) * (joint ? 3 : 1); }
   int adopt() {
     int rc;
-    const int64_t n = (int64_t)g.nvx * g.nvz * (map ? kmax : nz - 1) * (joint ? 3 : 1);
+    const int64_t n = ncols();
     arrays.keep = true;
-    if ((rc = dz_csr_adopt_cap(ctx, nray, n, arrays.nnz, arrays.rp, arrays.cl, arrays.v, nray + res_rows, arrays.cap_nnz, G))) return rc;
+    CsrReady ready;
+    ready.col16 = arrays.c16; ready.col16_cap = arrays.c16_cap; ready.col16_mod = dz_col_shape(n).mod16;
+    ready.vmax_bits = A.qcount + 24;
+    arrays.c16 = nullptr;
+    if ((rc = dz_csr_adopt_ready(ctx, nray, n, arrays.nnz, arrays.rp, arrays.cl, arrays.v, nray + res_rows, arrays.cap_nnz,
+                                 hand_over_G ? &ready : nullptr, G)))
+      return rc;
     if (twin) {
       dazim_csr *Gd = nullptr;
       arrays_d.keep = true;
@@ -1196,6 +1331,7 @@
     DZ_HIP(hipMemsetAsync(A.count, 0, (size_t)(nray + 1) * 8, ctx->stream));
     if ((rc = overlap ? count_passes_beside_eikonal() : count_pass())) return rc;
     if ((rc = scan_and_emit(arrays, A.count, res_nnz, false))) return rc;
+    hand_over_G = hand_over;
     if (twin && ((rc = dz_big_get(ctx, (size_t)(nray + 1), &arrays_d.rp)) || (rc = scan_and_emit(arrays_d, A.countd, 0, true)))) return rc;
     t.stop();
     if (overlap) {
diff --git a/dazimsurftomo_amd/csrc/sparse.hip b/dazimsurftomo_amd/csrc/sparse.hip
--- a/dazimsurftomo_amd/csrc/sparse.hip
+++ b/dazimsurftomo_amd/csrc/sparse.hip
@@ -184,15 +184,19 @@
 }
 
 constexpr int SCW = 16;
-constexpr int CBW_MAX = 19 * 1024;
-
-__global__ void k_colblock_ptr(int64_t nrows, int ncb, int cbw, const int64_t *__restrict__ ptr,
+
+__global__ void k_colblock_ptr(int64_t r0, int64_t nrows, int ncb, int cbw, const int64_t *__restrict__ ptr,
                                const int *__restrict__ col, int64_t *__restrict__ cbptr) {
-  const int64_t t = (int64_t)blockIdx.x * VB + threadIdx.x;
-  if (t >= nrows * (ncb + 1)) return;
+  int64_t t = (int64_t)blockIdx.x * VB + threadIdx.x;
+  if (t >= (nrows - r0) * (ncb + 1)) return;
+  t += r0 * (ncb + 1);
   const int64_t r = t / (ncb + 1);
   const int b = (int)(t - r * (ncb + 1));
   int64_t lo = ptr[r], hi = ptr[r + 1];
+  if (ncb == 1) {
+    cbptr[t] = b == 0 ? lo : hi;
+    return;
+  }
   const int target = b * cbw;
   while (lo < hi) {
     const int64_t mid = (lo + hi) >> 1;
@@ -201,9 +205,9 @@
   cbptr[t] = lo;
 }
 constexpr int SPLIT_SHORT = 64;
-__global__ void k_last_long_row(int64_t nrows, const int64_t *__restrict__ ptr, int thresh, unsigned long long *res) {
+__global__ void k_last_long_row(int64_t r0, int64_t nrows, const int64_t *__restrict__ ptr, int thresh, unsigned long long *res) {
   unsigned long long best = 0;
-  for (int64_t r = (int64_t)blockIdx.x * VB + threadIdx.x; r < nrows; r += (int64_t)gridDim.x * VB)
+  for (int64_t r = r0 + (int64_t)blockIdx.x * VB + threadIdx.x; r < nrows; r += (int64_t)gridDim.x * VB)
     if (ptr[r + 1] - ptr[r] >= thresh) best = (unsigned long long)(r + 1);
 #pragma unroll
   for (int o = 32; o > 0; o >>= 1) {
@@ -244,12 +248,26 @@
     part[blockIdx.x] = __uint_as_float(t);
   }
 }
-__global__ void k_absmax_finish(const float *part, int np, float *res) {
-  unsigned v = 0u;
+__global__ void k_absmax_finish(const float *part, int np, float *res, unsigned seed) {
+  unsigned v = seed;
   for (int i = threadIdx.x; i < np; i += 64) v = umax2(v, abs_bits(part[i]));
 #pragma unroll
   for (int o = 32; o > 0; o >>= 1) v = umax2(v, (unsigned)__shfl_xor((int)v, o));
   if (threadIdx.x == 0) res[0] = __uint_as_float(v);
+}
+__global__ void k_pack_derived(const unsigned long long *last, const int64_t *__restrict__ ptr, int64_t nrows, const unsigned *vmax_bits,
+                               unsigned long long *out) {
+  const unsigned long long l = last[0];
+  out[0] = l;
+  out[1] = (l > 0 && l <= (unsigned long long)nrows) ? (unsigned long long)ptr[l] : 0ull;
+  out[2] = vmax_bits[0];
+}
+template <class T>
+__global__ void k_weighted_sum(int64_t n, const T *__restrict__ a, unsigned long long *acc) {
+  unsigned long long v = 0;
+  for (int64_t i = (int64_t)blockIdx.x * VB + threadIdx.x; i < n; i += (int64_t)gridDim.x * VB)
+    v += (unsigned long long)a[i] * (unsigned long long)(1 + (i & 0xffff));
+  if (v) atomicAdd(acc, v);
 }
 
 struct RowPtr { int64_t s, e; float aux; };
@@ -505,7 +523,7 @@
   if ((rc = dz_scratch(ctx, "csr.absmax", (size_t)APART + 4, &pm))) return rc;
   const int nb = nblk((n + 3) / 4, APART);
   hipLaunchKernelGGL(k_absmax, dim3(nb), dim3(VB), 0, ctx->stream, n, x, pm);
-  hipLaunchKernelGGL(k_absmax_finish, dim3(1), dim3(64), 0, ctx->stream, pm, nb, pm + APART);
+  hipLaunchKernelGGL(k_absmax_finish, dim3(1), dim3(64), 0, ctx->stream, pm, nb, pm + APART, 0u);
   DZ_HIP(hipMemcpyAsync(res, pm + APART, 4, hipMemcpyDeviceToHost, ctx->stream));
   return 0;
 }
@@ -531,6 +549,8 @@
 }
 
 }
+
+static inline unsigned fbits(float x) { unsigned u; memcpy(&u, &x, 4); return u; }
 
 int dz_spmv_blocks(dazim_ctx *ctx, int64_t nrows, int64_t nx) {
   if (nx >= 0 && use_ldsx(ctx, nrows, nx)) return ctx->num_cu;
@@ -581,21 +601,40 @@
   return 0;
 }
 
-int dz_build_colblocks(dazim_ctx *ctx, dazim_csr *A, int64_t changed_from) {
-  if (A->cbptr) { dz_big_put(ctx, A->cbptr); A->cbptr = nullptr; }
-  A->ncb = (int)((A->n + CBW_MAX - 1) / CBW_MAX);
-  A->cbw = (int)(((A->n + A->ncb - 1) / A->ncb + 3) & ~3ll);
-  const int mod16 = A->n <= 65536 ? 0 : 2 * A->cbw;
-  const bool want16 = mod16 <= 65536 && A->nnz > 0 && dz_opt(ctx, "spmv.col16", 1) != 0;
-  if (A->col16 && (!want16 || A->col16_cap < A->nnz || changed_from == 0 || A->col16_mod != mod16)) {
+int dz_build_colblocks(dazim_ctx *ctx, dazim_csr *A, int64_t changed_from, int64_t rows_from, const CsrReady *ready) {
+  const ColShape cs = dz_col_shape(A->n);
+  const int mod16 = cs.mod16;
+  const bool rebuild = dz_opt(ctx, "csr.rebuild", 0) != 0;
+  const bool want16 = dz_want_col16(ctx, A->n, A->nnz);
+  const bool handed = ready && !rebuild && !A->derived;
+  bool col16_ready = false;
+  if (ready && ready->col16) {
+    if (handed && want16 && !A->col16 && ready->col16_mod == mod16 && ready->col16_cap >= A->nnz) {
+      A->col16 = ready->col16;
+      A->col16_cap = ready->col16_cap;
+      A->col16_mod = mod16;
+      col16_ready = true;
+    } else {
+      dz_big_put(ctx, ready->col16);
+    }
+  }
+  const bool append = !rebuild && !ready && A->derived && changed_from > 0 && rows_from > 0 && rows_from <= A->m &&
+                      A->ncb == cs.ncb && A->cbw == cs.cbw && A->cbptr && A->cbptr_rows >= A->m &&
+                      (A->col16 != nullptr) == want16 && (!A->col16 || (A->col16_mod == mod16 && A->col16_cap >= A->nnz));
+  const int64_t r0 = append ? rows_from : 0;
+  A->derived = false;
+  if (!append && A->cbptr) { dz_big_put(ctx, A->cbptr); A->cbptr = nullptr; A->cbptr_rows = 0; }
+  A->ncb = cs.ncb;
+  A->cbw = cs.cbw;
+  if (A->col16 && !col16_ready && (!want16 || A->col16_cap < A->nnz || changed_from == 0 || A->col16_mod != mod16)) {
     dz_big_put(ctx, A->col16);
     A->col16 = nullptr;
     A->col16_cap = 0;
   }
-  if (want16 && (!A->col16 || changed_from >= 0)) {
+  if (want16 && !col16_ready && (!A->col16 || changed_from >= 0)) {
     int64_t from = 0;
     if (!A->col16) {
-      A->col16_cap = ((A->cap_nnz > A->nnz ? A->cap_nnz : A->nnz) + 3) & ~(int64_t)3;
+      A->col16_cap = dz_col16_cap(A->nnz, A->cap_nnz);
       if (int rcp = dz_big_get(ctx, (size_t)A->col16_cap, &A->col16)) return rcp;
       A->col16_mod = mod16;
     } else {
@@ -606,34 +645,75 @@
       hipLaunchKernelGGL(k_narrow_cols, dim3(nblk((cnt + 3) / 4)), dim3(VB), 0, ctx->stream, cnt, A->col + from, A->col16 + from, mod16);
     DZ_HIP(hipGetLastError());
   }
-  const int64_t np = A->m * (A->ncb + 1);
-  if (np > 0) {
-    if (int rcp = dz_big_get(ctx, (size_t)np, &A->cbptr)) return rcp;
-    hipLaunchKernelGGL(k_colblock_ptr, dim3((unsigned)((np + VB - 1) / VB)), dim3(VB), 0, ctx->stream, A->m, A->ncb, A->cbw,
-                       A->rowptr, A->col, A->cbptr);
+  if (A->m > 0) {
+    if (!A->cbptr) {
+      A->cbptr_rows = A->cap_m > A->m ? A->cap_m : A->m;
+      if (int rcp = dz_big_get(ctx, (size_t)(A->cbptr_rows * (A->ncb + 1)), &A->cbptr)) return rcp;
+    }
+    const int64_t np = (A->m - r0) * (A->ncb + 1);
+    if (np > 0)
+      hipLaunchKernelGGL(k_colblock_ptr, dim3((unsigned)((np + VB - 1) / VB)), dim3(VB), 0, ctx->stream, r0, A->m, A->ncb, A->cbw,
+                         A->rowptr, A->col, A->cbptr);
     DZ_HIP(hipGetLastError());
   }
   int rc;
+  const unsigned old_vmax = append ? (fbits(A->vmax) & 0x7fffffffu) : 0u;
+  int64_t h_last = append ? A->last_long : 0, h_at = append ? A->last_long_at : 0;
   A->vmax = 0.0f;
+  if (A->m > 0 && A->nnz > 0) {
+    float *pm;
+    if ((rc = dz_scratch(ctx, "csr.absmax", (size_t)APART + 16, &pm))) return rc;
+    unsigned long long *d_last = reinterpret_cast<unsigned long long *>(pm + APART + 2), *d_pack = d_last + 1, *land;
+    { void *hp; if ((rc = dz_pinned(ctx, "csr.derived", 64, &hp))) return rc; land = (unsigned long long *)hp; }
+    DZ_HIP(hipMemsetAsync(d_last, 0, 8, ctx->stream));
+    if (A->m > r0)
+      hipLaunchKernelGGL(k_last_long_row, dim3(nblk(A->m - r0)), dim3(VB), 0, ctx->stream, r0, A->m, A->rowptr, SPLIT_SHORT, d_last);
+    const unsigned *vsrc = handed ? ready->vmax_bits : nullptr;
+    if (!vsrc) {
+      const int64_t from = append ? changed_from : 0, cnt = A->nnz - from;
+      const int nb = nblk((cnt + 3) / 4, APART);
+      hipLaunchKernelGGL(k_absmax, dim3(nb), dim3(VB), 0, ctx->stream, cnt, A->val + from, pm);
+      hipLaunchKernelGGL(k_absmax_finish, dim3(1), dim3(64), 0, ctx->stream, pm, nb, pm + APART, old_vmax);
+      vsrc = reinterpret_cast<const unsigned *>(pm + APART);
+    }
+    hipLaunchKernelGGL(k_pack_derived, dim3(1), dim3(1), 0, ctx->stream, d_last, A->rowptr, A->m, vsrc, d_pack);
+    DZ_HIP(hipGetLastError());
+    DZ_HIP(hipMemcpyAsync(land, d_pack, 24, hipMemcpyDeviceToHost, ctx->stream));
+    DZ_HIP(hipStreamSynchronize(ctx->stream));
+    if (land[0]) { h_last = (int64_t)land[0]; h_at = (int64_t)land[1]; }
+    const unsigned vb = (unsigned)land[2];
+    memcpy(&A->vmax, &vb, 4);
+  } else {
+    DZ_HIP(hipStreamSynchronize(ctx->stream));
+  }
+  A->last_long = h_last;
+  A->last_long_at = h_at;
   A->split_row = A->m;
   A->long_avg = A->m > 0 ? (double)A->nnz / (double)A->m : 0.0;
-  if (A->m > 0 && A->nnz > 0) {
-    float *pm;
-    if ((rc = dz_scratch(ctx, "csr.absmax", (size_t)APART + 4, &pm))) return rc;
-    unsigned long long *d_last = reinterpret_cast<unsigned long long *>(pm + APART + 2), h_last = 0;
-    DZ_HIP(hipMemsetAsync(d_last, 0, 8, ctx->stream));
-    hipLaunchKernelGGL(k_last_long_row, dim3(nblk(A->m)), dim3(VB), 0, ctx->stream, A->m, A->rowptr, SPLIT_SHORT, d_last);
-    DZ_HIP(hipMemcpyAsync(&h_last, d_last, 8, hipMemcpyDeviceToHost, ctx->stream));
-    DZ_HIP(hipStreamSynchronize(ctx->stream));
-    if ((int64_t)h_last < A->m && (int64_t)h_last > 0) {
-      int64_t at = 0;
-      DZ_HIP(hipMemcpy(&at, A->rowptr + h_last, 8, hipMemcpyDeviceToHost));
-      A->split_row = (int64_t)h_last;
-      A->long_avg = (double)at / (double)h_last;
-    }
-  }
-  if (A->nnz > 0 && (rc = absmax_to_host(ctx, A->val, A->nnz, &A->vmax))) return rc;
-  DZ_HIP(hipStreamSynchronize(ctx->stream));
+  if (h_last < A->m && h_last > 0) {
+    A->split_row = h_last;
+    A->long_avg = (double)h_at / (double)h_last;
+  }
+  A->derived = true;
+  ctx->ksec["csr.update"] = append ? 2 : (handed ? 1 : 0);
+  if (dz_opt(ctx, "csr.stats", 0) != 0) {
+    unsigned long long *acc, h[2] = {0, 0};
+    if ((rc = dz_scratch(ctx, "csr.stats", 2, &acc))) return rc;
+    DZ_HIP(hipMemsetAsync(acc, 0, 16, ctx->stream));
+    if (A->col16 && A->nnz > 0) hipLaunchKernelGGL(k_weighted_sum<unsigned short>, dim3(nblk(A->nnz)), dim3(VB), 0, ctx->stream, A->nnz, A->col16, acc);
+    if (A->cbptr && A->m > 0)
+      hipLaunchKernelGGL(k_weighted_sum<int64_t>, dim3(nblk(A->m * (A->ncb + 1))), dim3(VB), 0, ctx->stream, A->m * (A->ncb + 1), A->cbptr, acc + 1);
+    DZ_HIP(hipGetLastError());
+    DZ_HIP(hipMemcpy(h, acc, 16, hipMemcpyDeviceToHost));
+    const unsigned long long m52 = (1ull << 52) - 1;
+    ctx->ksec["csr.vmax_bits"] = (double)fbits(A->vmax);
+    ctx->ksec["csr.split_row"] = (double)A->split_row;
+    ctx->ksec["csr.long_avg"] = A->long_avg;
+    ctx->ksec["csr.col16_sum"] = A->col16 ? (double)(h[0] & m52) : -1.0;
+    ctx->ksec["csr.col16_mod"] = A->col16 ? (double)A->col16_mod : -1.0;
+    ctx->ksec["csr.cbptr_sum"] = A->cbptr ? (double)(h[1] & m52) : -1.0;
+    ctx->ksec["csr.ncb"] = A->ncb;
+  }
   return 0;
 }
 bool dz_use_scatter(dazim_ctx *ctx, const dazim_csr *A) {
@@ -839,14 +919,21 @@
 
 int dz_csr_adopt_cap(dazim_ctx *ctx, int64_t m, int64_t n, int64_t nnz, int64_t *rowptr, int *col, float *val,
                      int64_t cap_m, int64_t cap_nnz, dazim_csr **out) {
-  if (!ctx || !out || !rowptr) return DAZIM_E_BAD_ARG;
+  return dz_csr_adopt_ready(ctx, m, n, nnz, rowptr, col, val, cap_m, cap_nnz, nullptr, out);
+}
+int dz_csr_adopt_ready(dazim_ctx *ctx, int64_t m, int64_t n, int64_t nnz, int64_t *rowptr, int *col, float *val,
+                       int64_t cap_m, int64_t cap_nnz, const CsrReady *ready, dazim_csr **out) {
+  if (!ctx || !out || !rowptr) {
+    if (ctx && ready && ready->col16) dz_big_put(ctx, ready->col16);
+    return DAZIM_E_BAD_ARG;
+  }
   dazim_csr *A = new dazim_csr;
   A->m = m; A->n = n; A->nnz = nnz;
   A->rowptr = rowptr; A->col = col; A->val = val;
   if (cap_m > m) A->cap_m = cap_m;
   if (cap_nnz > nnz) A->cap_nnz = cap_nnz;
   int rc;
-  if ((rc = dz_build_colblocks(ctx, A)) || (rc = dz_invalidate_transpose(A))) {
+  if ((rc = dz_build_colblocks(ctx, A, 0, 0, ready)) || (rc = dz_invalidate_transpose(A))) {
     dazim_csr_free(ctx, A);
     return rc;
   }
@@ -904,7 +991,7 @@
   if ((rc = dazim_csr_from_coo(ctx, extra_m > 0 ? extra_m : 1, A->n, nnz2, shifted, icol_u, rw_u, &B))) return rc;
   const int64_t m2 = A->m + extra_m, nz2 = A->nnz + nnz2;
   if (A->cap_m >= m2 && A->cap_nnz >= nz2) {
-    const int64_t nnz1 = A->nnz;
+    const int64_t nnz1 = A->nnz, m1 = A->m;
     if (extra_m > 0)
       hipLaunchKernelGGL(k_offset_ptr, dim3(nblk(extra_m + 1)), dim3(VB), 0, ctx->stream, extra_m + 1, B->rowptr, A->nnz, A->rowptr + A->m);
     DZ_HIP(hipMemcpyAsync(A->col + nnz1, B->col, (size_t)nnz2 * 4, hipMemcpyDeviceToDevice, ctx->stream));
@@ -913,7 +1000,7 @@
     dazim_csr_free(ctx, B);
     A->m = m2;
     A->nnz = nz2;
-    if ((rc = dz_build_colblocks(ctx, A, nnz1 > 0 ? nnz1 : 0))) return rc;
+    if ((rc = dz_build_colblocks(ctx, A, nnz1 > 0 ? nnz1 : 0, m1))) return rc;
     if ((rc = dz_invalidate_transpose(A))) return rc;
     DZ_HIP(hipStreamSynchronize(ctx->stream));
     return 0;
diff --git a/dazimsurftomo_amd/csrc/sparse_internal.h b/dazimsurftomo_amd/csrc/sparse_internal.h
--- a/dazimsurftomo_amd/csrc/sparse_internal.h
+++ b/dazimsurftomo_amd/csrc/sparse_internal.h
@@ -16,6 +16,8 @@
   int64_t col16_cap = 0;
   int col16_mod = 0;
   int64_t cap_m = 0, cap_nnz = 0;
+  bool derived = false;
+  int64_t cbptr_rows = 0, last_long = 0, last_long_at = 0;
   dazim_csr *twin = nullptr;
 };
 
@@ -23,6 +25,26 @@
 constexpr int VB = 256;
 constexpr int NPART = 256;
 constexpr int APART = 2048;
+constexpr int CBW_MAX = 19 * 1024;
+
+struct ColShape { int ncb, cbw, mod16; };
+inline ColShape dz_col_shape(int64_t n) {
+  ColShape s;
+  s.ncb = (int)((n + CBW_MAX - 1) / CBW_MAX);
+  s.cbw = s.ncb > 0 ? (int)(((n + s.ncb - 1) / s.ncb + 3) & ~3ll) : 0;
+  s.mod16 = n <= 65536 ? 0 : 2 * s.cbw;
+  return s;
+}
+inline bool dz_want_col16(dazim_ctx *ctx, int64_t n, int64_t nnz) {
+  return dz_col_shape(n).mod16 <= 65536 && nnz > 0 && dz_opt(ctx, "spmv.col16", 1) != 0;
+}
+inline int64_t dz_col16_cap(int64_t nnz, int64_t cap_nnz) { return ((cap_nnz > nnz ? cap_nnz : nnz) + 3) & ~(int64_t)3; }
+struct CsrReady {
+  unsigned short *col16 = nullptr;
+  int64_t col16_cap = 0;
+  int col16_mod = 0;
+  const unsigned *vmax_bits = nullptr;
+};
 
 __device__ __forceinline__ float wave_sum(float v) {
 #pragma unroll
@@ -60,6 +82,8 @@
                     float beta_sign, double *sumsq, int *npart, const int *guard = nullptr);
 int dz_build_transpose(dazim_ctx *ctx, dazim_csr *A);
 int dz_invalidate_transpose(dazim_csr *A);
-int dz_build_colblocks(dazim_ctx *ctx, dazim_csr *A, int64_t changed_from = 0);
+int dz_build_colblocks(dazim_ctx *ctx, dazim_csr *A, int64_t changed_from = 0, int64_t rows_from = 0, const CsrReady *ready = nullptr);
 int dz_scale_rows(dazim_ctx *ctx, dazim_csr *A, int64_t nrows, const float *w);
+extern "C" int dz_csr_adopt_ready(dazim_ctx *ctx, int64_t m, int64_t n, int64_t nnz, int64_t *rowptr, int *col, float *val,
+                                  int64_t cap_m, int64_t cap_nnz, const CsrReady *ready, dazim_csr **out);
 #pragma GCC visibility pop
```
